# OettlM/STEDM

Hardware: AMD Instinct MI355X
Metric: U-Net denoising steps/sec (32x32x4 latent, bs=64) (higher is better)
Workload: dtype f16; 1 GPU; HER2-style DDIM-50 + CFG 1.5 (rescale 0.7) denoising step, NS32 U-Net (234.6M params, random-init PRNG weights), 32x32x4 latents + 3-ch layout concat, style vector 512; batch_per_gpu=64, global_batch=64, latent=32x32x4, cfg=cond+uncond per step, parallelism=dp1 (independent latents, no in-loop collective)

## Files before the change

include/stedm_hip.h:

```cpp
#ifndef STEDM_HIP_H
#define STEDM_HIP_H

#include <stdint.h>

#ifdef __cplusplus
extern "C" {
#endif

#define STEDM_ABI_VERSION 23

#define STEDM_F16 0
#define STEDM_BF16 1

#define STEDM_CONV_S1 0
#define STEDM_CONV_DOWN 1
#define STEDM_CONV_UP 2
#define STEDM_CONV_UP_SUBPIXEL 3
#define STEDM_CONV_S2D 4

int stedm_abi_version(void);
const char* stedm_last_error(void);
int stedm_device_cus(void);

#define STEDM_F16G_RAW 1
#define STEDM_F16G_NORM 2
#define STEDM_F16G_CONV_OUT16 4
#define STEDM_F16G_S2D 8
#define STEDM_F16G_CAST 16
#define STEDM_F16G_CONV_SRC 32
int stedm_f16_guard_set(void* flag_words);

int stedm_pack_conv_weight(const float* w_oihw, void* w_hi, void* w_lo, int cout, int cin, int ks,
                           int mm_dtype, void* stream);
int stedm_pack_conv_weight_up(const float* w_oihw, void* w_hi, void* w_lo, int cout, int cin, int mm_dtype,
                              void* stream);
int stedm_pack_conv_weight_frag(const float* w_oihw, void* out, int cout, int cin, int ks, int mm_dtype, void* stream);
int stedm_pack_conv_weight_up_frag(const float* w_oihw, void* out, int cout, int cin, int mm_dtype, void* stream);
int stedm_space_to_depth16(const float* x, int C, int B, int H, int W, void* out_hi, void* out_lo, int mm_dtype, void* stream);
int stedm_pack_conv_weight_frag16(const float* w, long sn, long sc, int flip, void* out, int cout, int cin, int ks, int mm_dtype, void* stream);
int stedm_pack_conv_weight_frag16_hl(const float* w, long sn, long sc, int flip, void* out, int cout, int cin, int mm_dtype, void* stream);
int stedm_pack_conv_weight_frag16_hl1(const float* w, long sn, long sc, int flip, void* out, int cout, int cin, int mm_dtype, void* stream);
int stedm_pack_conv_weight_up_frag16_hl(const float* w, void* out, int cout, int cin, int mm_dtype, void* stream);
int stedm_pack_conv_weight_s2d_frag16_hl(const float* w, void* out, int cout, int cin, int mm_dtype, int pad_br, void* stream);
int stedm_pack_conv_weight_s2d_frag(const float* w_oihw, void* out, int cout, int cin, int mm_dtype, int pad_br, void* stream);
int stedm_transpose_f32(const float* in, float* out, int rows, int cols, void* stream);

int stedm_gn_scale_shift(const float* x1, int c1, const float* x2, int c2, int x2_bmod,
                         const float* gamma, const float* beta, float eps, int groups, int B, int HW,
                         float* scale, float* shift, void* stream);

int stedm_gn_nslab(int C, int HW);
int stedm_gn_chan_nslab(int HW);
int stedm_gn_chan_stats(const float* x, int C, int B, int HW, int nslab, float* chan_stats, void* stream);
int stedm_gn_chan_stats16(const float* x, int C, int B, int HW, int nslab, float* chan_stats, void* out_hi, void* out_lo, int mm_dtype,
                          void* stream);
int stedm_gn_apply16c(const float* x1, int c1, const float* cs1, int nslab1, const float* x2, int c2, const float* cs2, int nslab2, int x2_bmod,
                      const float* gamma, const float* beta, float eps, int groups, int act, int B, int HW,
                      void* out_hi, void* out_lo, void* raw_hi, void* raw_lo, int mm_dtype, void* stream);
int stedm_gn_apply16c_mr(const float* x1, int c1, const float* cs1, int nslab1, const float* x2, int c2, const float* cs2, int nslab2, int x2_bmod,
                         const float* gamma, const float* beta, float eps, int groups, int act, int B, int HW,
                         void* out_hi, void* out_lo, void* raw_hi, void* raw_lo, float* mean_rstd, int mm_dtype, void* stream);
int stedm_gn_apply16c_x16(int c1, const float* cs1, int nslab1, const float* x2, int c2, const float* cs2, int nslab2, int x2_bmod,
                          const float* gamma, const float* beta, float eps, int groups, int act, int B, int HW,
                          void* out_hi, void* raw_hi, int mm_dtype, void* stream);
int stedm_gn_stats(const float* x1, int c1, const float* x2, int c2, int x2_bmod, int groups, int B, int HW,
                   double* stats, void* stream);
int stedm_gn_apply16(const float* x1, int c1, const float* x2, int c2, int x2_bmod, const float* gamma,
                     const float* beta, float eps, int groups, int act, const double* stats, int B, int HW,
                     void* out_hi, void* out_lo, int mm_dtype, void* stream);

typedef struct stedm_conv_args {
  const float* src1;
  const float* src2;
  int32_t c1, c2, src2_bmod;
  int32_t B, Hin, Win;
  int32_t mode;
  int32_t ks;
  const float* scale;
  const float* shift;
  int32_t act;
  const void* w_hi;
  const void* w_lo;
  const float* bias;
  const float* emb;
  int32_t emb_bstride;
  const float* res;
  float* out;
  int32_t cout;
  int32_t npass;
  int32_t mm_dtype;
  const void* src16_hi;
  const void* src16_lo;
  int32_t act_out;
  void* out16_hi;
  void* out16_lo;
  const void* w_frag;
  float* chan_stats;
  const void* src16b_hi;
  const void* w_frag_b;
  const float* bias_b;
  int32_t cb;
  float* ws;
  int64_t ws_floats;
  int32_t chan_nslab;
  const void* w_frag16;
  const void* w_frag_b16;
  int32_t pad_br;
  const float* gn_gamma;
  const float* gn_beta;
  float gn_eps;
  int32_t gn_groups;
  int32_t gn_act;
  void* gn_out16;
  float* gn_mr;
  int32_t gn_only;
  void* gn_out16_lo;
  void* qkv_q;
  void* qkv_k;
  void* qkv_vt;
  int32_t qkv_T, qkv_Tp, qkv_heads;
  float qkv_qscale;
  const float* ln_gamma;
  const float* ln_beta;
  const float* ln_res;
  float ln_eps;
  int32_t out16_stride;
  void* gn_coop;
  const uint32_t* gn_coop_epoch;
  uint32_t* gn_coop_tmo;
  int32_t src16_cstride;
  int32_t k_chan0;
  int32_t w_cin;
  int32_t res_bmod;
} stedm_conv_args;
int stedm_conv_igemm(const stedm_conv_args* args, void* stream);
int stedm_conv_fused_skip_ok(const stedm_conv_args* args);
int stedm_conv3x3_tiles_ok(int Hout, int Wout);
int stedm_im2col_rows16(const void* src16, void* dst16, int B, int Hs, int Ws, int C, int mode, void* stream);
int stedm_conv_rs_ok(const stedm_conv_args* args);

int stedm_conv_in(const float* x1, int c1, const float* x2, int c2, int x2_bmod, const float* w_oihw,
                  const float* bias, float* out, int B, int H, int W, int cout, float* chan_stats, void* stream);
int stedm_conv_out(const float* src, int c, const float* chan_stats, int nslab, const float* gamma, const float* beta,
                   float eps, int groups, const float* w_hwio, const float* bias, float* out, int B, int H, int W,
                   int cout, void* stream);

int stedm_time_embed(const int64_t* t, const float* freqs, const float* w0t, const float* b0,
                     const float* w2t, const float* b2, float* emb, float* ws, int B, int mc, int ted,
                     void* stream);
int stedm_time_embed_f32(const float* t, const float* freqs, const float* w0t, const float* b0,
                         const float* w2t, const float* b2, float* emb, float* ws, int B, int mc, int ted,
                         void* stream);
int stedm_emb_proj(const float* emb, const float* wt, const float* bias, float* out, int B, int k, int ntot,
                   void* stream);

int stedm_linear(const float* x, const float* wt, const float* bias, float* out, int B, int k, int n, int act_in,
                 int act_out, void* stream);

int stedm_attn_legacy(const float* qkv, float* out, int B, int T, int heads, int ch, void* stream);
int stedm_attn_legacy16(const void* qkv, int qkv_is16, void* out16, int B, int T, int heads, int ch, int mm_dtype, void* stream);

int stedm_ddim_step(const float* x, const float* e_c, const float* e_u, const float* noise,
                    const float* coefs, const int32_t* step_idx, float cfg_scale, float rescale_phi,
                    float* x_prev, float* pred_x0, int B, int C, int H, int W, void* stream);
int stedm_ddim_step_ex(const float* x, const float* e_c, const float* e_u, const float* noise, const float* coefs, const int32_t* step_idx,
                       int n_iters, float cfg_scale, float rescale_phi, int draw, float temperature, float noise_dropout, long first_id,
                       unsigned long long seed, float* x_prev, float* pred_x0, float* eps_out, float* noise_out, int B, int C, int H, int W,
                       void* stream);
int stedm_ddim_step_rows(const float* x, const float* e_c, const float* e_u, const float* noise, const float* coefs,
                         const int32_t* step_idx, int n_iters, const float* scales, float rescale_phi, int draw, long first_id,
                         unsigned long long seed, float* x_prev, float* pred_x0, int B, int C, int H, int W, void* stream);
int stedm_step_advance(int32_t* step_idx, int delta, void* stream);
int stedm_step_set_t(const int64_t* ts_table, const int32_t* step_idx, int64_t* t_buf, int B, void* stream);
int stedm_step_set_t_f32(const float* ts_table, const int32_t* step_idx, float* t_buf, int B, void* stream);

#define STEDM_DPM_NCOEF 6
int stedm_dpm_step(float* x, const float* e_c, const float* e_u, float* x0_prev, float* pred_x0, const float* coefs,
                   const int32_t* step_idx, float cfg_scale, long n, void* stream);

#define STEDM_DPMU_NCOEF 24
#define STEDM_DPMU_ALL 0
#define STEDM_DPMU_MODEL 1
#define STEDM_DPMU_COMBINE 2
int stedm_dpm_update(float* x, float* base, const float* e_c, const float* e_u, float* slots, long slot_stride, float* pred_x0,
                     const float* rows, const int32_t* step_idx, float cfg_scale, int mode, long n, void* stream);
int stedm_dpm_threshold(float* slots, long slot_stride, const float* rows, const int32_t* step_idx, float max_val, int B, long n,
                        float* q_out, void* stream);

#define STEDM_PLMS_EULER 0
#define STEDM_PLMS_HEUN 1
#define STEDM_PLMS_MULTISTEP 2
int stedm_plms_step(float* x, const float* e_c, const float* e_u, float* ring, const float* coefs, const int32_t* step_idx,
                    int n_iters, int phase, float cfg_scale, float* pred_x0, float* x_tmp, long n, void* stream);

int stedm_svit_patch_embed(const float* img, int B, int ns, int H, int W, int patch, const float* ln_w,
                           const float* ln_b, float eps, const float* wt, const float* bias, const float* pos,
                           const float* cls, float* x, int dim, void* stream);
int stedm_svit_patch_ln16(const float* img, int B, int ns, int H, int W, int patch, const float* ln_w, const float* ln_b,
                          float eps, void* out_hi, void* out_lo, int mm_dtype, void* stream);
int stedm_svit_tok_place(const float* tok, const float* pos, const float* cls, float* x, int B, int ntok, int dim, void* stream);
int stedm_ln_apply16(const float* x, const float* gamma, const float* beta, float eps, void* out_hi, void* out_lo,
                     long rows, int dim, int mm_dtype, void* stream);
int stedm_qkv_pack(const void* qkv, int qkv_is16, float qscale, void* q_hi, void* q_lo, void* k_hi, void* k_lo, void* vt_hi,
                   void* vt_lo, int B, int T, int Tp, int heads, int mm_dtype, void* stream);
int stedm_lsa_flash(const void* q_hi, const void* q_lo, const void* k_hi, const void* k_lo, const void* vt_hi,
                    const void* vt_lo, void* out_hi, void* out_lo, int B, int T, int Tp, int heads, int npass,
                    int mm_dtype, void* stream);
int stedm_qkv_pack_mx8(const void* qkv, int qkv_is16, float qscale, void* q8, void* qs, void* k8, void* ks, void* vt8, void* vs, int B, int T,
                       int Tp, int heads, int mm_dtype, void* stream);
int stedm_lsa_flash_mx8(const void* q8, const void* qs, const void* k8, const void* ks, const void* vt8, const void* vs, void* out16, int B,
                        int T, int Tp, int heads, int mm_dtype, void* stream);
int stedm_dropout_rows(const float* src, const float* res, float* out, void* out_hi, void* out_lo, long n, float p,
                       unsigned long long seed, unsigned site, int mm_dtype, void* stream);
int stedm_lsa_flash_drop(const void* q_hi, const void* q_lo, const void* k_hi, const void* k_lo, const void* vt_hi,
                         const void* vt_lo, void* out_hi, void* out_lo, int B, int T, int Tp, int heads, int npass,
                         int mm_dtype, float p, unsigned long long seed, unsigned site, void* stream);
int stedm_svit_head(const float* x, int B, int T, int dim, int pool, const float* c_old, const float* ln_w,
                    const float* ln_b, float eps, const float* wt, const float* bias, float* out, int ncls, float* ws, long ws_floats,
                    void* stream);
int stedm_geglu16(const float* g, void* out_hi, void* out_lo, long M, int I, int mm_dtype, void* stream);
int stedm_agg_reduce(const float* feats, float* out, int B, int n, int F, int mode, void* stream);
int stedm_spatial_rescale(const float* x, const float* w, float* out, int B, int cin, int cout, int H, int W,
// ... 113 lines not shown
```

stedm_amd/_lib.py:

```python
from __future__ import annotations

import ctypes as C
import os

_HERE = os.path.dirname(os.path.abspath(__file__))
LIB_PATH = os.environ.get("STEDM_HIP_LIB") or os.path.join(_HERE, "libstedm_hip.so")

ABI_VERSION = 23
F16, BF16 = 0, 1
CONV_S1, CONV_DOWN, CONV_UP, CONV_UP_SUBPIXEL, CONV_S2D = 0, 1, 2, 3, 4


class StedmHipError(RuntimeError):
    pass


class ConvArgs(C.Structure):
    _fields_ = [
        ("src1", C.c_void_p), ("src2", C.c_void_p),
        ("c1", C.c_int32), ("c2", C.c_int32), ("src2_bmod", C.c_int32),
        ("B", C.c_int32), ("Hin", C.c_int32), ("Win", C.c_int32),
        ("mode", C.c_int32), ("ks", C.c_int32),
        ("scale", C.c_void_p), ("shift", C.c_void_p),
        ("act", C.c_int32),
        ("w_hi", C.c_void_p), ("w_lo", C.c_void_p), ("bias", C.c_void_p),
        ("emb", C.c_void_p), ("emb_bstride", C.c_int32),
        ("res", C.c_void_p), ("out", C.c_void_p),
        ("cout", C.c_int32), ("npass", C.c_int32), ("mm_dtype", C.c_int32),
        ("src16_hi", C.c_void_p), ("src16_lo", C.c_void_p),
        ("act_out", C.c_int32), ("out16_hi", C.c_void_p), ("out16_lo", C.c_void_p),
        ("w_frag", C.c_void_p), ("chan_stats", C.c_void_p),
        ("src16b_hi", C.c_void_p), ("w_frag_b", C.c_void_p), ("bias_b", C.c_void_p), ("cb", C.c_int32),
        ("ws", C.c_void_p), ("ws_floats", C.c_int64), ("chan_nslab", C.c_int32), ("w_frag16", C.c_void_p), ("w_frag_b16", C.c_void_p), ("pad_br", C.c_int32),
        ("gn_gamma", C.c_void_p), ("gn_beta", C.c_void_p), ("gn_eps", C.c_float), ("gn_groups", C.c_int32), ("gn_act", C.c_int32), ("gn_out16", C.c_void_p), ("gn_mr", C.c_void_p), ("gn_only", C.c_int32),
        ("gn_out16_lo", C.c_void_p),
        ("qkv_q", C.c_void_p), ("qkv_k", C.c_void_p), ("qkv_vt", C.c_void_p),
        ("qkv_T", C.c_int32), ("qkv_Tp", C.c_int32), ("qkv_heads", C.c_int32), ("qkv_qscale", C.c_float),
        ("ln_gamma", C.c_void_p), ("ln_beta", C.c_void_p), ("ln_res", C.c_void_p), ("ln_eps", C.c_float),
        ("out16_stride", C.c_int32),
        ("gn_coop", C.c_void_p), ("gn_coop_epoch", C.c_void_p), ("gn_coop_tmo", C.c_void_p),
        ("src16_cstride", C.c_int32), ("k_chan0", C.c_int32), ("w_cin", C.c_int32), ("res_bmod", C.c_int32),
    ]


_P, _I, _F = C.c_void_p, C.c_int, C.c_float
SIGNATURES = {
    "stedm_abi_version": (_I, []),
    "stedm_last_error": (C.c_char_p, []),
    "stedm_device_cus": (_I, []),
    "stedm_f16_guard_set": (_I, [_P]),
    "stedm_pack_conv_weight": (_I, [_P, _P, _P, _I, _I, _I, _I, _P]),
    "stedm_pack_conv_weight_up": (_I, [_P, _P, _P, _I, _I, _I, _P]),
    "stedm_pack_conv_weight_frag": (_I, [_P, _P, _I, _I, _I, _I, _P]),
    "stedm_pack_conv_weight_up_frag": (_I, [_P, _P, _I, _I, _I, _P]),
    "stedm_pack_conv_weight_frag16": (_I, [_P, C.c_long, C.c_long, _I, _P, _I, _I, _I, _I, _P]),
    "stedm_pack_conv_weight_frag16_hl": (_I, [_P, C.c_long, C.c_long, _I, _P, _I, _I, _I, _P]),
    "stedm_pack_conv_weight_frag16_hl1": (_I, [_P, C.c_long, C.c_long, _I, _P, _I, _I, _I, _P]),
    "stedm_pack_conv_weight_up_frag16_hl": (_I, [_P, _P, _I, _I, _I, _P]),
    "stedm_pack_conv_weight_s2d_frag16_hl": (_I, [_P, _P, _I, _I, _I, _I, _P]),
    "stedm_pack_conv_weight_s2d_frag": (_I, [_P, _P, _I, _I, _I, _I, _P]),
    "stedm_space_to_depth16": (_I, [_P, _I, _I, _I, _I, _P, _P, _I, _P]),
    "stedm_transpose_f32": (_I, [_P, _P, _I, _I, _P]),
    "stedm_gn_scale_shift": (_I, [_P, _I, _P, _I, _I, _P, _P, _F, _I, _I, _I, _P, _P, _P]),
    "stedm_gn_nslab": (_I, [_I, _I]),
    "stedm_gn_stats": (_I, [_P, _I, _P, _I, _I, _I, _I, _I, _P, _P]),
    "stedm_gn_apply16": (_I, [_P, _I, _P, _I, _I, _P, _P, _F, _I, _I, _P, _I, _I, _P, _P, _I, _P]),
    "stedm_gn_chan_nslab": (_I, [_I]),
    "stedm_gn_chan_stats": (_I, [_P, _I, _I, _I, _I, _P, _P]),
    "stedm_gn_chan_stats16": (_I, [_P, _I, _I, _I, _I, _P, _P, _P, _I, _P]),
    "stedm_gn_apply16c": (_I, [_P, _I, _P, _I, _P, _I, _P, _I, _I, _P, _P, _F, _I, _I, _I, _I, _P, _P, _P, _P, _I, _P]),
    "stedm_gn_apply16c_mr": (_I, [_P, _I, _P, _I, _P, _I, _P, _I, _I, _P, _P, _F, _I, _I, _I, _I, _P, _P, _P, _P, _P, _I, _P]),
    "stedm_conv3x3_tiles_ok": (_I, [_I, _I]),
    "stedm_im2col_rows16": (_I, [_P, _P, _I, _I, _I, _I, _I, _P]),
    "stedm_philox_normal": (_I, [_P, _I, _I, _P, _I, C.c_ulonglong, C.c_uint, _P]),
    "stedm_ddim_mask_blend": (_I, [_P, _P, _P, C.c_long, C.c_long, _P, _P, _P, _P, _P, _I, _I, _I, C.c_long, C.c_ulonglong, _P]),
    "stedm_ddpm_step": (_I, [_P, _P, _P, _P, _I, _I, _P, _P, C.c_long, C.c_long, _P, _P, _P, _P, _I, _I, _I, C.c_long,
                            C.c_ulonglong, C.c_ulonglong, _P]),
    "stedm_ddpm_step_ex": (_I, [_P, _P, _P, _P, _P, _I, _I, _P, _P, _F, _P, _I, _P, C.c_long, C.c_long, _P, _P, _P, _P, _P, _P, _P, _P,
                               _I, _I, _I, C.c_long, C.c_ulonglong, C.c_ulonglong, _P]),
    "stedm_gn_apply16c_x16": (_I, [_I, _P, _I, _P, _I, _P, _I, _I, _P, _P, _F, _I, _I, _I, _I, _P, _P, _I, _P]),
    "stedm_conv_igemm": (_I, [C.POINTER(ConvArgs), _P]),
    "stedm_conv_fused_skip_ok": (_I, [C.POINTER(ConvArgs)]),
    "stedm_conv_rs_ok": (_I, [C.POINTER(ConvArgs)]),
    "stedm_conv_in": (_I, [_P, _I, _P, _I, _I, _P, _P, _P, _I, _I, _I, _I, _P, _P]),
    "stedm_conv_out": (_I, [_P, _I, _P, _I, _P, _P, _F, _I, _P, _P, _P, _I, _I, _I, _I, _P]),
    "stedm_time_embed": (_I, [_P, _P, _P, _P, _P, _P, _P, _P, _I, _I, _I, _P]),
    "stedm_time_embed_f32": (_I, [_P, _P, _P, _P, _P, _P, _P, _P, _I, _I, _I, _P]),
    "stedm_emb_proj": (_I, [_P, _P, _P, _P, _I, _I, _I, _P]),
    "stedm_linear": (_I, [_P, _P, _P, _P, _I, _I, _I, _I, _I, _P]),
    "stedm_attn_legacy": (_I, [_P, _P, _I, _I, _I, _I, _P]),
    "stedm_attn_legacy16": (_I, [_P, _I, _P, _I, _I, _I, _I, _I, _P]),
    "stedm_ddim_step": (_I, [_P, _P, _P, _P, _P, _P, _F, _F, _P, _P, _I, _I, _I, _I, _P]),
    "stedm_ddim_step_ex": (_I, [_P, _P, _P, _P, _P, _P, _I, _F, _F, _I, _F, _F, C.c_long, C.c_ulonglong, _P, _P, _P, _P, _I, _I, _I, _I,
                               _P]),
    "stedm_ddim_step_rows": (_I, [_P, _P, _P, _P, _P, _P, _I, _P, _F, _I, C.c_long, C.c_ulonglong, _P, _P, _I, _I, _I, _I, _P]),
    "stedm_step_advance": (_I, [_P, _I, _P]),
    "stedm_step_set_t": (_I, [_P, _P, _P, _I, _P]),
    "stedm_step_set_t_f32": (_I, [_P, _P, _P, _I, _P]),
    "stedm_dpm_step": (_I, [_P, _P, _P, _P, _P, _P, _P, _F, C.c_long, _P]),
    "stedm_dpm_update": (_I, [_P, _P, _P, _P, _P, C.c_long, _P, _P, _P, _F, _I, C.c_long, _P]),
    "stedm_dpm_threshold": (_I, [_P, C.c_long, _P, _P, _F, _I, C.c_long, _P, _P]),
    "stedm_plms_step": (_I, [_P, _P, _P, _P, _P, _P, _I, _I, _F, _P, _P, C.c_long, _P]),
    "stedm_svit_patch_embed": (_I, [_P, _I, _I, _I, _I, _I, _P, _P, _F, _P, _P, _P, _P, _P, _I, _P]),
    "stedm_svit_patch_ln16": (_I, [_P, _I, _I, _I, _I, _I, _P, _P, _F, _P, _P, _I, _P]),
    "stedm_svit_tok_place": (_I, [_P, _P, _P, _P, _I, _I, _I, _P]),
    "stedm_ln_apply16": (_I, [_P, _P, _P, _F, _P, _P, C.c_long, _I, _I, _P]),
    "stedm_qkv_pack": (_I, [_P, _I, _F, _P, _P, _P, _P, _P, _P, _I, _I, _I, _I, _I, _P]),
    "stedm_lsa_flash": (_I, [_P, _P, _P, _P, _P, _P, _P, _P, _I, _I, _I, _I, _I, _I, _P]),
    "stedm_lsa_flash_drop": (_I, [_P, _P, _P, _P, _P, _P, _P, _P, _I, _I, _I, _I, _I, _I, _F, C.c_ulonglong, C.c_uint, _P]),
    "stedm_dropout_rows": (_I, [_P, _P, _P, _P, _P, C.c_long, _F, C.c_ulonglong, C.c_uint, _I, _P]),
    "stedm_qkv_pack_mx8": (_I, [_P, _I, _F, _P, _P, _P, _P, _P, _P, _I, _I, _I, _I, _I, _P]),
    "stedm_lsa_flash_mx8": (_I, [_P, _P, _P, _P, _P, _P, _P, _I, _I, _I, _I, _I, _P]),
    "stedm_svit_head": (_I, [_P, _I, _I, _I, _I, _P, _P, _P, _F, _P, _P, _P, _I, _P, C.c_long, _P]),
    "stedm_ln_bwd_blocks": (_I, [C.c_long]),
    "stedm_ln_bwd": (_I, [_P, _P, _P, _F, _P, _P, _P, _P, _P, C.c_long, _I, _I, _P]),
    "stedm_geglu_bwd": (_I, [_P, _P, _P, C.c_long, _I, _P]),
    "stedm_geglu16": (_I, [_P, _P, _P, C.c_long, _I, _I, _P]),
    "stedm_agg_reduce": (_I, [_P, _P, _I, _I, _I, _I, _P]),
    "stedm_spatial_rescale": (_I, [_P, _P, _P, _I, _I, _I, _I, _I, _I, _P]),
    "stedm_pack_frag_multi": (_I, [_P, _I, _I, _I, _P]),
    "stedm_swin_patch16": (_I, [_P, C.c_long, C.c_long, C.c_long, C.c_long, _I, _I, _I, _P, _P, _I, _P]),
    "stedm_swin_ln": (_I, [_P, _P, _P, _F, _P, _P, _P, _P, C.c_long, _I, _I, _I, _P]),
    "stedm_swin_ln_gated": (_I, [_P, _P, _P, _F, _P, _P, _P, _P, C.c_long, _I, _I, _P, _I, _I, _P]),
    "stedm_swin_window_attn": (_I, [_P, _P, _P, _P, _P, _P, _P, _I, _I, _I, _I, _I, _I, _I, _I, _I, _P]),
    "stedm_swin_merge16": (_I, [_P, _I, _I, _I, _I, _P, _P, _I, _P]),
    "stedm_swin_rpb": (_I, [_P, _P, _P, _I, _I, _P]),
    "stedm_swin_token_mean": (_I, [_P, _P, _I, _I, _I, _P]),
    "stedm_pack_conv_weight_strided": (_I, [_P, C.c_long, C.c_long, _I, _P, _P, _P, _I, _I, _I, _I, _P]),
    "stedm_gn_fold": (_I, [_P, _I, _I, _P, _I, _I, _I, _I, _I, _F, _P, _P]),
    "stedm_gn_bwd": (_I, [_P, _I, _P, _I, _P, _P, _P, _I, _I, _P, _P, _I, _I, _P, _P, _I, _P, _I, _P, _P, _I, _P, _P, _I, _P]),
    "stedm_gn_bwd_ws_floats": (C.c_long, [_I, _I, _I, _I]),
    "stedm_im2col_t16": (_I, [_P, _P, _I, _I, _I, _I, _I, _I, C.c_long, _P]),
    "stedm_wgrad_to_oihw": (_I, [_P, _P, _I, _I, _I, _I, _I, _I, _I, _P]),
    "stedm_wgrad3x3_plan": (_I, [_I, _I, _I, _I, _I, C.POINTER(C.c_int)]),
    "stedm_wgrad3x3": (_I, [_P, _P, _P, _I, _I, _I, _I, _I, _I, _P]),
    "stedm_wgrad3x3_oihw": (_I, [_P, _P, _P, _I, _I, _I, _I, _I, _I, _P]),
    "stedm_sum_planes": (_I, [_P, _P, C.c_long, _I, _I, _P]),
    "stedm_wgrad1x1_plan": (_I, [C.c_long, _I, _I, C.POINTER(C.c_int)]),
    "stedm_wgrad1x1": (_I, [_P, _P, _P, C.c_long, _I, _I, _I, _P]),
    "stedm_chan_sum_fold": (_I, [_P, _I, _I, _I, _P, C.c_long, _P, _I, _P]),
    "stedm_chan_sum_fold2": (_I, [_P, _I, _I, _I, _P, C.c_long, _P, _I, _P, _P]),
    "stedm_sum2x2": (_I, [_P, _P, _I, _I, _I, _I, _I, _P]),
    "stedm_zero_insert16": (_I, [_P, _P, _P, _I, _I, _I, _I, _I, _P]),
    "stedm_attn_legacy_bwd_ws_floats": (C.c_long, [_I, _I, _I]),
    "stedm_attn_legacy_bwd": (_I, [_P, _P, _P, _I, _I, _I, _I, _P, _P]),
    "stedm_gemm_f32": (_I, [_P, C.c_long, _I, _P, C.c_long, _I, _P, C.c_long, _I, _I, _I, _F, _F, _P, C.c_long, _P]),
    "stedm_silu": (_I, [_P, _P, _P, C.c_long, _I, _P]),
    "stedm_q_sample": (_I, [_P, _P, _P, _P, _P, _P, _I, C.c_long, _P]),
    "stedm_l1_loss": (_I, [_P, _P, C.c_long, _F, _P, _P, _P, _P]),
    "stedm_diffusion_loss_blocks": (_I, [C.c_long]),
    "stedm_diffusion_loss": (_I, [_P, _P, _P, _P, _P, _I, C.c_long, _I, _I, C.c_double, C.c_double, C.c_double, _P, _P, _P, C.c_long, _P, _P]),
    "stedm_spatial_rescale_wgrad": (_I, [_P, _P, _P, _P, _I, _I, _I, _I, _I, _I, _I, _P]),
    "stedm_axpby_f32": (_I, [_P, _P, C.c_long, _F, _F, _P]),
    "stedm_adamw_ema": (_I, [_P, _P, _P, _I, _F, _F, _F, _F, _F, _I, _F, _F, _P]),
    "stedm_adamw_ema_pack": (_I, [_P, _I, _I, _F, _F, _F, _F, _F, _I, _F, _F, _P]),
    "stedm_adamw_ema_pack_piece": (_I, [_P, _P]),
    "stedm_adamw_ema_sched": (_I, [_P, _P, _P, _I, _F, _F, _F, _F, _P, _P, _F, _P]),
    "stedm_adamw_ema_pack_sched": (_I, [_P, _I, _I, _F, _F, _F, _F, _P, _P, _F, _P]),
    "stedm_ema_update": (_I, [_P, _P, _P, _I, _F, _P]),
    "stedm_vq_nearest": (_I, [_P, _P, _I, _I, _I, C.c_long, _P, _P, _P]),
    "stedm_ddim_quantize_x0": (_I, [_P, _P, _P, _P, _P, _P, _I, _I, _I, C.c_long, _P, _P, _P]),
    "stedm_conv1x1_nchw": (_I, [_P, _P, _P, _P, _I, _I, _I, C.c_long, _P]),
    "stedm_softmax_rows16": (_I, [_P, C.c_long, _F, _P, _P, C.c_long, _I, C.c_long, _I, _P]),
    "stedm_image_to_uint8": (_I, [_P, _P, _I, _I, _I, _I, _P]),
    "stedm_seg_merge": (_I, [_P, _P, _I, _I, _I, _I, _P]),
    "stedm_argmax_u8": (_I, [_P, _P, C.c_long, _I, _P]),
# ... 42 lines not shown
```

stedm_amd/csrc/conv_common.hpp:

```cpp
#pragma once
#include "common.hpp"

typedef float f32x16 __attribute__((ext_vector_type(16)));
typedef float f32x4 __attribute__((ext_vector_type(4)));
typedef _Float16 f16x8 __attribute__((ext_vector_type(8)));
typedef __bf16 bf16x8 __attribute__((ext_vector_type(8)));
typedef _Float16 f16x4 __attribute__((ext_vector_type(4)));
typedef __bf16 bf16x4 __attribute__((ext_vector_type(4)));

constexpr int BN = 128;

struct ConvParams {
  stedm_conv_args a;
  int M, Hout, Wout, HWout, Cin, taps;
  int cstride, w_cin;
  int whole, nsamp, trows;
  int wsplit;
  int PRs, PW, NP;
  int tiles_m, tiles_n;
  unsigned mg_hw, mg_w, mg_pw, mg_prpw;
  int ksplit;
  int stats_done;
  int gn_done;
  int gn_tile;
  int gn_coop;
  int xcd_m;
  int npers;
  unsigned* ovf;
  int dbg;
};

#ifdef STEDM_CONV_DIAG
#define STEDM_DBG(WORD, BITS) (((WORD) & (BITS)) != 0)
#else
#define STEDM_DBG(WORD, BITS) (0)
#endif

template <typename T>
struct MM;
template <>
struct MM<_Float16> {
  using V8 = f16x8;
  using V4 = f16x4;
  static __device__ __forceinline__ f32x16 mfma(V8 a, V8 b, f32x16 c) {
    return __builtin_amdgcn_mfma_f32_32x32x16_f16(a, b, c, 0, 0, 0);
  }
  static __device__ __forceinline__ f32x4 mfma16(V8 a, V8 b, f32x4 c) {
    return __builtin_amdgcn_mfma_f32_16x16x32_f16(a, b, c, 0, 0, 0);
  }
};
template <>
struct MM<__bf16> {
  using V8 = bf16x8;
  using V4 = bf16x4;
  static __device__ __forceinline__ f32x16 mfma(V8 a, V8 b, f32x16 c) {
    return __builtin_amdgcn_mfma_f32_32x32x16_bf16(a, b, c, 0, 0, 0);
  }
  static __device__ __forceinline__ f32x4 mfma16(V8 a, V8 b, f32x4 c) {
    return __builtin_amdgcn_mfma_f32_16x16x32_bf16(a, b, c, 0, 0, 0);
  }
};


#define STEDM_ZERO_PAGE_BYTES 135168

namespace stedm {
bool conv_geometry(ConvParams& p, int bm, bool allow_wsplit = false);
int conv_launch_dma(ConvParams& p, hipStream_t st, bool dry = false);
}
```

stedm_amd/csrc/conv_dma_bf16_p1.hip:

```cpp
#include "conv_igemm_dma9.inc"
#include "conv_rs.inc"
namespace stedm {
int conv_dma_pick_bf16_p1(ConvParams& p, hipStream_t st, bool dry) {
  int rc = conv_rs_pick<__bf16>(p, st, dry);
  if (rc >= 0 || dry || p.a.src16b_hi || p.a.mode == STEDM_CONV_S2D || p.a.qkv_q || p.a.ln_gamma) return rc;
  if (p.a.src16_cstride || p.a.k_chan0 || p.a.w_cin || p.a.res_bmod || p.a.out16_stride) return rc;
  rc = dma9_pick<__bf16>(p, st);
  return rc >= 0 ? rc : dma_pick<1, __bf16>(p, st);
}
}

extern "C" int stedm_debug_conv_stamps(unsigned long long* host_out, int nblocks) {
  if (!host_out || nblocks <= 0 || nblocks > 2048) { stedm::set_error("debug_conv_stamps: bad args"); return 1; }
  hipError_t e = hipMemcpyFromSymbol(host_out, HIP_SYMBOL(g_conv_stamps), (size_t)nblocks * 8 * sizeof(unsigned long long));
  if (e != hipSuccess) { stedm::set_error("debug_conv_stamps: %s", hipGetErrorString(e)); return 2; }
  return 0;
}
```

stedm_amd/csrc/conv_dma_f16_p1.hip:

```cpp
#include "conv_igemm_dma9.inc"
#include "conv_rs.inc"
namespace stedm {
int conv_dma_pick_f16_p1(ConvParams& p, hipStream_t st, bool dry) {
  int rc = conv_rs_pick<_Float16>(p, st, dry);
  if (rc >= 0 || dry || p.a.src16b_hi || p.a.mode == STEDM_CONV_S2D || p.a.qkv_q || p.a.ln_gamma) return rc;
  if (p.a.src16_cstride || p.a.k_chan0 || p.a.w_cin || p.a.res_bmod || p.a.out16_stride) return rc;
  rc = dma9_pick<_Float16>(p, st);
  return rc >= 0 ? rc : dma_pick<1, _Float16>(p, st);
}
}
```

stedm_amd/csrc/conv_igemm.hip:

```cpp
#include <stdlib.h>

#include "conv_common.hpp"
using namespace stedm;

constexpr int BM = 128, NTHREADS = 256;

template <int BKC, int NPASS, typename T>
__global__ void __launch_bounds__(NTHREADS, 2) conv_igemm_kernel(const ConvParams p) {
  using V8 = typename MM<T>::V8;
  using V4 = typename MM<T>::V4;
  constexpr int AST = BKC * 2 + 16;
  constexpr int BST = BKC * 2 + 16;
  constexpr int NPL = NPASS == 3 ? 2 : 1;
  constexpr int QC = BKC / 4;
  constexpr int POSL = NTHREADS / QC;
  constexpr int PCS = BKC / 8;
  constexpr int BPT = BN * PCS / NTHREADS;
  constexpr int KSTEPS = BKC / 16;

  extern __shared__ __attribute__((aligned(16))) unsigned char smem[];
  unsigned char* sA = smem;
  const int a_plane = p.NP * AST;
  unsigned char* sB = smem + NPL * a_plane;
  constexpr int b_plane = BN * BST;
// ... 210 lines not shown
        if (a.res) v += a.res[o];
        a.out[o] = v;
      }
    }
  }
  f16_guard_commit(p.ovf, bad_src, STEDM_F16G_CONV_SRC);
}

template <int BKC, int NPASS, typename T>
static int launch(const ConvParams& p, hipStream_t st) {
  constexpr int AST = BKC * 2 + 16, BST = BKC * 2 + 16, NPL = NPASS == 3 ? 2 : 1;
  const size_t lds = (size_t)NPL * p.NP * AST + (size_t)2 * NPL * BN * BST;
  if (lds > 160 * 1024) {
    set_error("conv_igemm: tile needs %zu B of LDS (> 160 KiB): Hin=%d Win=%d mode=%d", lds, p.a.Hin, p.a.Win, p.a.mode);
    return 1;
  }
  auto k = conv_igemm_kernel<BKC, NPASS, T>;
  if (lds > 64 * 1024) {
    hipError_t e = hipFuncSetAttribute(reinterpret_cast<const void*>(k), hipFuncAttributeMaxDynamicSharedMemorySize, (int)lds);
    if (e != hipSuccess) {
      set_error("conv_igemm: hipFuncSetAttribute(%zu) failed: %s", lds, hipGetErrorString(e));
      return 2;
    }
  }
  k<<<p.tiles_m * p.tiles_n, NTHREADS, lds, st>>>(p);
  STEDM_LAUNCH_CHECK();
  return 0;
}

bool stedm::conv_geometry(ConvParams& p, int bm, bool allow_wsplit) {
  const stedm_conv_args& a = p.a;
  p.tiles_n = (a.cout + BN - 1) / BN;
  p.tiles_m = (p.M + bm - 1) / bm;
  p.wsplit = 0;
  if (a.ks == 1) {
    p.whole = 0; p.nsamp = 1; p.trows = 0; p.PRs = 1; p.PW = bm; p.NP = bm;
    return true;
  }
  if (p.HWout <= bm) {
    if (bm % p.HWout != 0) { set_error("conv_igemm: Hout*Wout=%d must divide %d", p.HWout, bm); return false; }
    p.whole = 1; p.nsamp = bm / p.HWout; p.trows = p.Hout;
    p.tiles_m = (a.B + p.nsamp - 1) / p.nsamp;
  } else if (allow_wsplit && p.Wout > bm && p.Wout % bm == 0 && (a.mode == STEDM_CONV_S1 || a.mode == STEDM_CONV_UP_SUBPIXEL || a.mode == STEDM_CONV_S2D)) {
    p.whole = 0; p.nsamp = 1; p.trows = 1; p.wsplit = 1;
  } else {
    if (bm % p.Wout != 0 || p.HWout % bm != 0) {
      set_error("conv_igemm: unsupported spatial shape %dx%d (need Wout | %d and %d | Hout*Wout)", p.Hout, p.Wout, bm, bm);
      return false;
    }
    p.whole = 0; p.nsamp = 1; p.trows = bm / p.Wout;
  }
  if (a.mode == STEDM_CONV_S1 || a.mode == STEDM_CONV_UP_SUBPIXEL || a.mode == STEDM_CONV_S2D) p.PRs = p.trows + 2;
  else if (a.mode == STEDM_CONV_DOWN) p.PRs = 2 * p.trows + 1;
  else p.PRs = (p.trows + 1) / 2 + 2;
  p.PW = (p.wsplit ? bm : a.Win) + 2;
  p.NP = p.nsamp * p.PRs * p.PW;
  return true;
}

static int conv_dispatch(ConvParams& p, void* stream);
static int conv_setup(ConvParams& p);

extern "C" int stedm_conv3x3_tiles_ok(int Hout, int Wout) {
  if (Hout <= 0 || Wout <= 0) return 0;
  if (Wout > 256 && Wout % 256 == 0) return 1;
  for (int bm = 256; bm >= 128; bm >>= 1) {
    const int HW = Hout * Wout;
    if (HW <= bm) { if (bm % HW == 0) return 1; continue; }
    if (bm % Wout == 0 && HW % bm == 0) return 1;
  }
  return 0;
}

extern "C" int stedm_conv_fused_skip_ok(const stedm_conv_args* args) {
  if (!args || !args->src16b_hi || !args->src16_hi) return 0;
  ConvParams p;
  memset(&p, 0, sizeof(p));
  p.a = *args;
  if (conv_setup(p) != 0) return 0;
  return conv_launch_dma(p, nullptr, true) == 0 ? 1 : 0;
}

extern "C" int stedm_conv_rs_ok(const stedm_conv_args* args) {
  if (!args || !args->src16_hi || (!args->w_frag && !args->w_frag16) || (args->npass != 1 && !args->w_frag16)) return 0;
  ConvParams p;
  memset(&p, 0, sizeof(p));
  p.a = *args;
  if (conv_setup(p) != 0) return 0;
  return conv_launch_dma(p, nullptr, true) == 0 ? 1 : 0;
}

extern "C" int stedm_conv_igemm(const stedm_conv_args* args, void* stream) {
  STEDM_CHECK_ARG(args, "conv_igemm: null args");
  ConvParams p;
  memset(&p, 0, sizeof(p));
  p.a = *args;
  const stedm_conv_args& a = p.a;
  STEDM_CHECK_ARG(!a.chan_stats || a.out || (a.out16_hi && !a.out16_lo && a.npass == 1), "conv_igemm: chan_stats needs the fp32 output (or, single product, the 16-bit-only form)");
  STEDM_CHECK_ARG(a.out16_stride == 0 || (a.out16_hi && !a.out16_lo && a.npass == 1 && a.out16_stride >= a.cout && a.out16_stride % 4 == 0 && a.cout % 4 == 0 &&
                                          !a.ln_gamma && !a.qkv_q && !a.act_out),
                  "conv_igemm: out16_stride needs out16_hi alone (single product), stride >= cout, both multiples of 4, plain epilogue");
  STEDM_CHECK_ARG(!a.gn_out16 || (a.out && a.chan_stats && a.gn_gamma && a.gn_beta && a.gn_groups > 0 && a.cout % a.gn_groups == 0 &&
                                  (a.npass == 1 || a.gn_out16_lo) && a.mode == STEDM_CONV_S1 && (a.gn_act == 0 || a.gn_act == 1)),
                  "conv_igemm: gn_out16 needs out, chan_stats, gamma / beta, groups dividing cout, stride 1 and a single-product mode (or gn_out16_lo)");
  STEDM_CHECK_ARG(!a.gn_out16_lo || a.gn_out16, "conv_igemm: gn_out16_lo without gn_out16");
  int rc = conv_dispatch(p, stream);
  if (rc != 0) return rc;
  if (a.chan_stats && !p.stats_done && !a.out) {
    set_error("conv_igemm: the 16-bit-only form with chan_stats ran on a kernel without the statistics epilogue");
    return 1;
  }
  if (a.chan_stats && !p.stats_done) {
    const int up = (a.mode == STEDM_CONV_UP || a.mode == STEDM_CONV_UP_SUBPIXEL) ? 4 : 1, down = a.mode == STEDM_CONV_DOWN ? 4 : 1;
    rc = stedm_gn_chan_stats(a.out, a.cout, a.B, a.Hin * a.Win * up / down, a.chan_nslab, a.chan_stats, stream);
    if (rc != 0) return rc;
  }
  if (a.gn_out16 && !p.gn_done) {
    const int HW = a.Hin * a.Win;
    rc = stedm_gn_apply16c_mr(a.out, a.cout, a.chan_stats, a.chan_nslab > 0 ? a.chan_nslab : stedm_gn_chan_nslab(HW), nullptr, 0, nullptr, 0, 0, a.gn_gamma,
                              a.gn_beta, a.gn_eps, a.gn_groups, a.gn_act, a.B, HW, a.gn_out16, a.gn_out16_lo, nullptr, nullptr, a.gn_mr, a.mm_dtype, stream);
  }
  return rc;
}

static int conv_setup(ConvParams& p) {
  const stedm_conv_args& a = p.a;
  STEDM_CHECK_ARG((a.src1 || a.src16_hi) && (a.w_hi || (a.mode == STEDM_CONV_S2D && (a.w_frag || (a.npass == 3 && a.w_frag16)))) && (a.out || a.out16_hi || a.qkv_q),
                  "conv_igemm: null src/w_hi/out");
  STEDM_CHECK_ARG(!a.ln_gamma || (a.ln_beta && (a.out || a.out16_hi) && !a.out16_lo && !a.res && !a.emb && !a.chan_stats && !a.gn_out16 && !a.act_out && !a.qkv_q &&
                                  a.src16_hi && !a.src1 && !a.src16b_hi && a.w_frag && a.ks == 1 && a.mode == STEDM_CONV_S1 && a.npass == 1 && a.cout <= 128 &&
                                  a.cout % 4 == 0),
                  "conv_igemm: the LayerNorm epilogue needs a 1x1 GEMM with cout <= 128 (a multiple of 4), src16 + w_frag, a single-product mode and no other epilogue extra");
  STEDM_CHECK_ARG(!a.qkv_q || (a.qkv_k && a.qkv_vt && !a.out && !a.out16_hi && !a.res && !a.emb && !a.chan_stats && !a.gn_out16 && !a.act_out && a.src16_hi && !a.src1 &&
                               !a.src16b_hi && a.w_frag && a.ks == 1 && a.mode == STEDM_CONV_S1 && a.npass == 1 && a.B == 1 && a.Hin == 1 && a.qkv_heads > 0 &&
                               a.qkv_heads % 2 == 0 && a.cout == 3 * a.qkv_heads * 64 && a.qkv_T > 0 && a.qkv_T % 2 == 0 && a.qkv_Tp >= a.qkv_T &&
                               a.qkv_Tp % 2 == 0 && a.Win % a.qkv_T == 0),
                  "conv_igemm: the qkv epilogue needs a flat 1x1 GEMM (B = Hin = 1, Win = nb * T rows), cout = 3 * heads * 64 with an even head count, even T / Tp, "
                  "src16 + w_frag, a single-product mode and no other output or epilogue extra");
  STEDM_CHECK_ARG(a.pad_br == 0 || a.mode == STEDM_CONV_S2D, "conv_igemm: pad_br belongs to the space-to-depth form");
  STEDM_CHECK_ARG(a.mode != STEDM_CONV_S2D || (a.src16_hi && !a.src1 && a.ks == 3 && !a.src16b_hi &&
                                                ((a.npass == 1 && a.w_frag) || (a.npass == 3 && a.w_frag16 && a.src16_lo))),
                  "conv_igemm: the space-to-depth form needs src16 planes, ks=3 and w_frag (single product) or w_frag16 + src16_lo (3 products)");
  STEDM_CHECK_ARG((!a.act_out && !a.out16_hi) || (a.src16_hi && !a.src1), "conv_igemm: act_out/out16 need the DMA path (src16 only)");
  STEDM_CHECK_ARG(!a.src1 || (a.src2 != nullptr) == (a.c2 > 0), "conv_igemm: src2/c2 mismatch");
  STEDM_CHECK_ARG(!a.src16_hi || a.npass == 1 || a.src16_lo, "conv_igemm: npass=3 needs src16_lo");
  STEDM_CHECK_ARG(a.ks == 1 || a.ks == 3, "conv_igemm: ks must be 1 or 3");
  STEDM_CHECK_ARG(a.mode >= 0 && a.mode <= 4, "conv_igemm: bad mode %d", a.mode);
  STEDM_CHECK_ARG(a.mode != STEDM_CONV_UP_SUBPIXEL || (a.src16_hi && !a.src1 && a.ks == 3), "conv_igemm: sub-pixel upsample needs the DMA path (src16) and ks=3");
  STEDM_CHECK_ARG(a.ks == 3 || a.mode == STEDM_CONV_S1, "conv_igemm: 1x1 supports stride 1 only");
  STEDM_CHECK_ARG(a.npass == 1 || a.npass == 3, "conv_igemm: npass must be 1 or 3");
  STEDM_CHECK_ARG(a.npass == 1 || a.w_lo || (a.mode == STEDM_CONV_S2D && a.w_frag16), "conv_igemm: npass=3 needs w_lo");
  STEDM_CHECK_ARG((a.scale != nullptr) == (a.shift != nullptr), "conv_igemm: scale/shift must come together");
  STEDM_CHECK_ARG(a.B > 0 && a.Hin > 0 && a.Win > 0 && a.cout > 0, "conv_igemm: bad sizes");
  STEDM_CHECK_ARG(a.mm_dtype == STEDM_F16 || a.mm_dtype == STEDM_BF16, "conv_igemm: bad mm_dtype %d", a.mm_dtype);
  p.Cin = a.c1 + a.c2;
  p.cstride = a.src16_cstride ? a.src16_cstride : p.Cin;
  p.w_cin = a.w_cin ? a.w_cin : p.Cin;
  {
    const bool kwin = a.src16_cstride || a.k_chan0 || a.w_cin;
    const bool plain3 = a.src16_hi && !a.src1 && a.c2 == 0 && a.ks == 3 && a.mode == STEDM_CONV_S1 && a.npass == 1 && !a.src16b_hi && (a.w_frag || a.w_frag16) &&
                        !a.ln_gamma && !a.qkv_q;
    STEDM_CHECK_ARG(!kwin || (plain3 && a.k_chan0 >= 0 && a.k_chan0 % 32 == 0 && p.cstride % 32 == 0 && p.w_cin % 32 == 0 && a.c1 % 32 == 0 &&
                              a.k_chan0 + a.c1 <= p.cstride && a.k_chan0 + a.c1 <= p.w_cin),
                    "conv_igemm: a K window (src16_cstride=%d k_chan0=%d w_cin=%d) needs a plain 3x3 stride-1 single-product problem on src16 planes with "
                    "w_frag / w_frag16 and no fused skip phase; multiples of 32 with k_chan0 + c1 inside both the plane row and the pack",
                    a.src16_cstride, a.k_chan0, a.w_cin);
    STEDM_CHECK_ARG(a.res_bmod == 0 || (a.res_bmod > 0 && a.res && plain3),
                    "conv_igemm: res_bmod=%d needs res and a plain 3x3 stride-1 single-product problem on src16 planes with w_frag / w_frag16 and no fused skip phase",
                    a.res_bmod);
  }
  p.taps = (a.mode == STEDM_CONV_UP_SUBPIXEL || a.mode == STEDM_CONV_S2D) ? 4 : a.ks * a.ks;
  if (a.mode == STEDM_CONV_UP_SUBPIXEL || a.mode == STEDM_CONV_S2D) {
    p.Hout = a.Hin; p.Wout = a.Win;
  } else if (a.mode == STEDM_CONV_DOWN) {
    STEDM_CHECK_ARG(a.Hin % 2 == 0 && a.Win % 2 == 0, "conv_igemm: stride-2 needs even Hin/Win");
    p.Hout = a.Hin / 2; p.Wout = a.Win / 2;
  } else if (a.mode == STEDM_CONV_UP) {
    p.Hout = a.Hin * 2; p.Wout = a.Win * 2;
  } else {
    p.Hout = a.Hin; p.Wout = a.Win;
  }
  p.HWout = p.Hout * p.Wout;
  p.M = a.B * p.HWout;
  STEDM_CHECK_ARG(p.Cin % 32 == 0 && (a.c2 == 0 || a.c1 % 32 == 0),
                  "conv_igemm: channel counts must be multiples of 32 (c1=%d c2=%d)", a.c1, a.c2);
  STEDM_CHECK_ARG(!a.src16b_hi || (a.src16_hi && !a.src1 && ((a.w_frag && a.w_frag_b) || (a.w_frag16 && a.w_frag_b16)) && a.ks == 3 && a.mode == STEDM_CONV_S1 && a.npass == 1 && !a.res &&
                                   a.cb > 0 && a.cb % 64 == 0),
                  "conv_igemm: the fused skip phase needs the DMA path (src16 only), 3x3 stride 1, single product, w_frag + w_frag_b, cb %% 64 == 0, no res");
  return 0;
}

static int conv_dispatch(ConvParams& p, void* stream) {
  const stedm_conv_args& a = p.a;
  { const int rc = conv_setup(p); if (rc) return rc; }
  hipStream_t st = as_stream(stream);
  static const int dbg0 = getenv("STEDM_CONV_DBG") ? atoi(getenv("STEDM_CONV_DBG")) : 0;
#ifdef STEDM_CONV_DIAG
  p.dbg = dbg0;
#else
  p.dbg = 0;
  if (dbg0) { set_error("conv_igemm: STEDM_CONV_DBG=%d needs a diagnostic build (tools/conv_diag.sh, STEDM_HIP_LIB); the shipped kernels compile no ablation switch", dbg0); return 1; }
#endif
  p.ovf = a.mm_dtype == STEDM_F16 ? f16_guard_flag() : nullptr;
  if (a.src16_hi) {
    const int rc = conv_launch_dma(p, st);
    if (rc == 0 || !a.src1) return rc;
  }
  const int bkc = (a.npass == 1 && p.Cin % 64 == 0 && (a.c2 == 0 || a.c1 % 64 == 0)) ? 64 : 32;
  if (!conv_geometry(p, BM)) return 1;
  const bool f16 = a.mm_dtype == STEDM_F16;
  if (a.npass == 3) return f16 ? launch<32, 3, _Float16>(p, st) : launch<32, 3, __bf16>(p, st);
  if (bkc == 64) return f16 ? launch<64, 1, _Float16>(p, st) : launch<64, 1, __bf16>(p, st);
  return f16 ? launch<32, 1, _Float16>(p, st) : launch<32, 1, __bf16>(p, st);
}
```

stedm_amd/csrc/conv_igemm_dma.hip:

```cpp
#include "conv_common.hpp"
using namespace stedm;

namespace stedm {
int conv_dma_pick_f16_p1(ConvParams&, hipStream_t, bool dry);
int conv_dma_pick_f16_p3(ConvParams&, hipStream_t, bool dry);
int conv_dma_pick_bf16_p1(ConvParams&, hipStream_t, bool dry);
int conv_dma_pick_bf16_p3(ConvParams&, hipStream_t, bool dry);
}

int stedm::conv_launch_dma(ConvParams& p, hipStream_t st, bool dry) {
  const stedm_conv_args& a = p.a;
  if (a.src16b_hi && a.npass != 1) { set_error("conv_igemm(dma): the fused skip phase is single-product only"); return 1; }
  if (dry && a.npass != 1 && !a.w_frag16) return 1;
  if (a.src16b_hi && ((long)a.B * a.Hin * a.Win * a.cb >= (1L << 31) || a.cb * 2 + 256 > STEDM_ZERO_PAGE_BYTES)) {
    set_error("conv_igemm(dma): fused skip operand too large (cb=%d)", a.cb);
    return 1;
  }
  if ((long)a.B * a.Hin * a.Win * (p.cstride > p.Cin ? p.cstride : p.Cin) >= (1L << 31)) {
    set_error("conv_igemm(dma): activation tensor too large for 32-bit element offsets");
    return 1;
  }
  if (p.Cin * 2 + 256 > STEDM_ZERO_PAGE_BYTES) { set_error("conv_igemm(dma): Cin too large for the zero page"); return 1; }
  const bool f16 = a.mm_dtype == STEDM_F16;
  int rc = a.npass == 3 ? (f16 ? conv_dma_pick_f16_p3(p, st, dry) : conv_dma_pick_bf16_p3(p, st, dry))
                        : (f16 ? conv_dma_pick_f16_p1(p, st, dry) : conv_dma_pick_bf16_p1(p, st, dry));
  if (dry) return rc < 0 ? 1 : 0;
  if (rc < 0 && a.ln_gamma) { set_error("conv_igemm(dma): the register-streamed kernel does not run this LayerNorm-epilogue problem (see stedm_conv_rs_ok)"); return 1; }
  if (rc < 0 && a.qkv_q) { set_error("conv_igemm(dma): the register-streamed kernel does not run this qkv-epilogue problem (see stedm_conv_rs_ok)"); return 1; }
  if (rc < 0 && (a.src16_cstride || a.k_chan0 || a.w_cin || a.res_bmod || a.out16_stride)) {
    set_error("conv_igemm(dma): the register-streamed kernel does not run this problem, and no other kernel knows a K window, res_bmod or out16_stride (see stedm_conv_rs_ok)");
    return 1;
  }
  if (rc < 0 && a.src16b_hi) { set_error("conv_igemm(dma): no kernel runs this fused skip problem (see stedm_conv_fused_skip_ok)"); return 1; }
  if (rc < 0) { set_error("conv_igemm(dma): no tile configuration fits (Hin=%d Win=%d mode=%d Cin=%d)", a.Hin, a.Win, a.mode, p.Cin); return 1; }
  return rc;
}
```

stedm_amd/csrc/conv_rs.inc:

```
#pragma once
#include <type_traits>

#include "conv_igemm_dma.inc"

static __device__ unsigned long long g_conv_stamps[2048 * 8];
#define STAMP(K) if (STEDM_DBG(p.dbg, 1024) && tid == 0 && blockIdx.x < 2048) g_conv_stamps[blockIdx.x * 8 + (K)] = wall_clock64()
#define STAMPC(K) if (STEDM_DBG(p.dbg, 1024) && tid == 0 && blockIdx.x < 2048) g_conv_stamps[blockIdx.x * 8 + (K)] = __builtin_amdgcn_s_memtime()

#ifdef STEDM_CONV_DIAG
#define RS_DIAG(BIT) ((STEDM_CONV_DIAG) & (BIT))
#else
#define RS_DIAG(BIT) 0
#endif

__device__ __forceinline__ float rs_lane_xor1(float v) {
  return __builtin_bit_cast(float, __builtin_amdgcn_mov_dpp(__builtin_bit_cast(int, v), 0xB1, 0xF, 0xF, true));
}
template <typename T>
__device__ __forceinline__ unsigned rs_pack2(float lo, float hi) {
  typedef T V2T __attribute__((ext_vector_type(2)));
  V2T v; v[0] = (T)lo; v[1] = (T)hi;
  return __builtin_bit_cast(unsigned, v);
}

// ... 215 lines not shown
#define A3_AFTER(Q, WHAT)                                                                                          \
  {                                                                                                                \
    if ((Q) + 2 < 8) { WHAT(Acur, t, (Q) + 2) }                                                                    \
    else if (t + 1 < NS) { WHAT(Acur, t + 1, (Q) + 2 - 8) }                                                         \
    else { WHAT(Anext, 0, (Q) + 2 - 8) }                                                                           \
  }
#define A3_ADDR_HI(BASE, TAP, F) asm volatile("v_add_u32 %0, %1, %2" : "=v"(a_) : "s"((BASE) + tapd[TAP]), "v"(aofs[F]));
#define A3_ADDR_LO(BASE, TAP, F) asm volatile("v_add_u32 %0, %1, %2" : "=v"(a2_) : "s"((BASE) + tapd[TAP] + a_half), "v"(aofs[F]));
#define RS3_CHUNK(PAR)                                                                                             \
  _Pragma("unroll") for (int u = 0; u < NU; ++u) {                                                                 \
    const int t = u >> 1, hf = u & 1, sb = (t & 1) ^ (PAR);                                                        \
    if (u == NU - 1) __builtin_amdgcn_s_barrier();    \
    _Pragma("unroll") for (int i = 0; i < 4; ++i) {                                                                \
      const int R = hf * 4 + i;                             \
      _Pragma("unroll") for (int m = 0; m < 12; ++m) {                                                             \
        const int j = m & 3;                                                                                       \
        __builtin_amdgcn_sched_barrier(0);                                                                         \
        if (m < 4) acc[R][j] = MM<T>::mfma16(al[R & (NAR - 1)], bh[sb][j], acc[R][j]);                              \
        else if (m < 8) acc[R][j] = MM<T>::mfma16(ah[R & (NAR - 1)], bl[sb][j], acc[R][j]);                         \
        else acc[R][j] = MM<T>::mfma16(ah[R & (NAR - 1)], bh[sb][j], acc[R][j]);                                    \
        __builtin_amdgcn_sched_barrier(0);                                                                         \
        if (m == 0) { LDSR(ah[(R + 1) & (NAR - 1)], a_); }                                                          \
        else if (m == 1) { LDSR(al[(R + 1) & (NAR - 1)], a2_); }                                                    \
        if (R == 0 && m >= 4) {                                                                                    \
                        \
          if (m == 4) { int g_ = g0 + t + 1; g_ = g_ < gmax ? g_ : gmax; wcur = wq + ((size_t)(unsigned)g_ << 13) + voff; } \
          if (m < 8) bh[sb ^ 1][m - 4] = *reinterpret_cast<const V8*>(wcur + (m - 4) * 1024);                        \
          else bl[sb ^ 1][m - 8] = *reinterpret_cast<const V8*>(wcur + wlo + (m - 8) * 1024);                        \
        }                                                                                                          \
        if (m == 10) A3_AFTER(R, A3_ADDR_HI)                                                                        \
        else if (m == 11) A3_AFTER(R, A3_ADDR_LO)                                                                   \
      }                                                                                                            \
    }                                                                                                              \
  }
  const unsigned char* wcur = wq + voff;
  unsigned a_ = 0, a2_ = 0;
  LOAD_B3(0, 0)
  LOAD_B3(1, 1)
  __syncthreads();
  {
    const unsigned Afirst = A0 + abuf * a_buf;
#pragma unroll
    for (int f = 0; f < NAR; ++f) LOAD_A3(Afirst, 0, f)
    A3_ADDR_HI(Afirst, 0, 1)
    A3_ADDR_LO(Afirst, 0, 1)
  }
#define RS3_STEP(STEP, PAR)                                                                                        \
  {                                                                                                                \
    const unsigned Acur = A0 + abuf * a_buf;                                                                       \
    if (++abuf == NABUF) abuf = 0;                                                                                 \
                                       \
    const unsigned Anext = (STEP) + 1 < nchunks ? A0 + abuf * a_buf : Acur;                                        \
    const int g0 = (STEP) * NS;                                                                                    \
    RS3_CHUNK(PAR)                                                                                                 \
  }
  int step = 0;
  for (; step + 1 < nchunks; step += 2) {
    RS3_STEP(step, 0)
    RS3_STEP(step + 1, NS & 1)
  }
  if (step < nchunks) RS3_STEP(step, 0)
#undef RS3_STEP
#undef RS3_CHUNK
#undef A3_AFTER
#undef A3_ADDR_HI
#undef A3_ADDR_LO
#undef LOAD_A3
#undef LOAD_B3
#undef LDSR
}

template <typename T, int WM, int KIND, bool FUSE = false, bool P3 = false>
__global__ void __launch_bounds__((16 / WM + 2) * 64) conv_rs_kernel(const ConvParams p) {
  static_assert(!FUSE || KIND == RS_3X3 || KIND == RS_3X3M, "the fused skip phase belongs to the 3x3 kinds");
  static_assert(!P3 || ((KIND == RS_3X3M || KIND == RS_1X1M || KIND == RS_SUBM) && !FUSE), "the 3-product form exists for the plain 16x16x32 kinds");
  static_assert(KIND != RS_1X1M || (P3 && !FUSE && WM == 4), "RS_1X1M is a 3-product kind");
  static_assert(KIND != RS_SUBM || (!FUSE && WM == 4), "RS_SUBM: plain epilogues, one compute wave per SIMD");
  constexpr int NCW = 16 / WM, NT = (NCW + 2) * 64, BMT = 256;
  constexpr bool NPERS = KIND == RS_1X1N, IS1X1 = KIND == RS_1X1 || NPERS, SUBM = KIND == RS_SUBM, SUBPIX = KIND == RS_SUB || SUBM;
  constexpr bool G1 = KIND == RS_1X1M;
  constexpr bool M16 = KIND == RS_3X3M || G1 || SUBM;
  constexpr bool GEO1 = IS1X1 || G1;
  constexpr bool IS3X3 = KIND == RS_3X3 || KIND == RS_3X3M;
  constexpr int NS = IS3X3 ? 9 : (SUBM ? 4 : (SUBPIX ? 8 : (G1 ? 1 : 4)));
  constexpr int NPL = (SUBPIX || KIND == RS_3X3M) ? 2 : 1;
  constexpr int NTAB = IS3X3 ? 9 : 4;
  constexpr int BROW = IS1X1 ? 128 : (G1 ? 64 : 32);
  constexpr int CPP = BROW / 16, RPB = 16 / CPP, PPI = 64 / CPP;
  constexpr int BKC = M16 ? 32 : NS * 16 / (IS3X3 ? 9 : (SUBPIX ? 4 : 1));
  constexpr int TAPS = NTAB, NABUF = P3 ? 3 : 4;
  constexpr int SST = kStageStride;

  extern __shared__ __attribute__((aligned(16))) unsigned char smem[];
  const int nai = (p.NP + PPI - 1) / PPI;
  const int a_plane = nai * 1024;
  const int a_half = NPL * a_plane + (M16 ? 32 : 0);
  const int a_buf = P3 ? 2 * a_half : ((FUSE && NPL * a_plane < 32768) ? 32768 : a_half);
  const int pl_skew = (KIND == RS_3X3M || SUBM) ? 16 : 0;
  int* sM = reinterpret_cast<int*>(smem);
  int* sMb = sM + BMT;
  unsigned char* sA = reinterpret_cast<unsigned char*>(sMb + BMT);
  float* sStage = reinterpret_cast<float*>(sA);
  const int ring_bytes = NABUF * a_buf;
  int* sIdx = reinterpret_cast<int*>(sA + ring_bytes);

  const stedm_conv_args& a = p.a;
  const int tid = threadIdx.x;
  const int lane = tid & 63;
  const int wave = __builtin_amdgcn_readfirstlane(tid >> 6);
  const bool is_loader = wave >= NCW;
  const int ntile = p.tiles_m * p.tiles_n;
  const bool s2d = SUBPIX && a.mode == STEDM_CONV_S2D;
  const int parity = (SUBPIX && !s2d) ? (blockIdx.x / ntile) & 3 : 0;
  const bool split = (IS3X3 || SUBPIX || GEO1) && p.ksplit >= 2;
  const int kz = split ? ((SUBPIX && !s2d) ? blockIdx.x / (4 * ntile) : blockIdx.x / ntile) : 0;
  const int bid = (SUBPIX || split) ? blockIdx.x % ntile : blockIdx.x;
  const int py = parity >> 1, px = parity & 1;
  int tile_n = bid % p.tiles_n, tile_m = bid / p.tiles_n;
  if (p.xcd_m) {
    const int gm = p.xcd_m, gn = 8 / gm, x = bid & 7, j = bid >> 3, tn_x = p.tiles_n / gn;
    const int jm = j / tn_x;
    tile_n = (j - jm * tn_x) * gn + x / gm;
    tile_m = jm * gm + x % gm;
  }
  constexpr bool npers = NPERS;
  if (npers) { tile_m = bid / p.npers; tile_n = (bid % p.npers) * (p.tiles_n / p.npers); }
  if STEDM_DBG(p.dbg, 256) { tile_n = 0; tile_m = 0; }
  const int m0 = tile_m * BMT, n0 = tile_n * BN;
  const int nchunks_all = p.Cin / BKC;
  const int nchunks_w = p.w_cin / BKC;
  const int nsteps = split ? nchunks_all / p.ksplit : nchunks_all;
  const int cbeg = kz * nsteps;
  const int nsteps2_all = FUSE ? a.cb / 64 : 0;
  const int nsteps2 = split ? nsteps2_all / p.ksplit : nsteps2_all;
  const int c2beg = split ? kz * nsteps2 : 0;
  STAMP(0);

  int b0, yo0;
  if (p.whole) { b0 = tile_m * p.nsamp; yo0 = 0; }
  else { b0 = m0 / p.HWout; yo0 = (m0 - b0 * p.HWout) / p.Wout; }
  const int br = s2d ? a.pad_br : 0;
  const int x0 = p.wsplit ? (m0 - b0 * p.HWout) - yo0 * p.Wout : 0;
  const int srow0 = ((a.mode == STEDM_CONV_S1 || SUBPIX) ? yo0 - 1 : (yo0 - 1) >> 1) + br;
  static_assert(RS_3X3 == 0, "");

  auto div_hw = [&](int n) { return (int)__umulhi((unsigned)n, p.mg_hw); };
  auto div_w = [&](int n) { return (int)__umulhi((unsigned)n, p.mg_w); };
  auto div_pw = [&](int n) { return (int)__umulhi((unsigned)n, p.mg_pw); };
  auto div_prpw = [&](int n) { return (int)__umulhi((unsigned)n, p.mg_prpw); };
  const int rem0 = GEO1 ? m0 - (m0 / p.HWout) * p.HWout : 0;
  auto patch_pixel = [&](int pos) {
    int off = -1;
    if (pos < p.NP) {
      if (GEO1) { if (m0 + pos < p.M) off = m0 + pos; }
      else {
        const int s_ = div_prpw(pos), rem = pos - s_ * (p.PRs * p.PW);
        const int prow = div_pw(rem), pcol = rem - prow * p.PW;
        const int b = b0 + s_, sy = srow0 + prow, sx = x0 + pcol - 1 + br;
        if (b < a.B && sy >= 0 && sy < a.Hin && sx >= 0 && sx < a.Win) off = (b * a.Hin + sy) * a.Win + sx;
      }
    }
    return off;
  };
  constexpr int NTC = NCW * 64;
  if (!is_loader) {
  for (int ml = tid; ml < BMT; ml += NTC) {
// ... 509 lines not shown
          *reinterpret_cast<V8T*>(dstp + (((long)b * H + hd) * Tp + t) * 64 + d0) = h8;
          const uint4 hb = __builtin_bit_cast(uint4, h8);
          bad16 |= f16_over2<T>(hb.x) | f16_over2<T>(hb.y) | f16_over2<T>(hb.z) | f16_over2<T>(hb.w);
        }
      } else {
        long o[2];
#pragma unroll
        for (int hf = 0; hf < 2; ++hf) {
          const int row = 2 * (hf * 64 + lane), m = sM[row];
          o[hf] = m < 0 ? -1 : (long)sMb[row] * HD * Tp + (m - sMb[row] * Tn);
        }
        T* __restrict__ vt = reinterpret_cast<T*>(a.qkv_vt);
        for (int d = tid >> 6; d < 128; d += NT / 64) {
          const int nl = n0 - 2 * HD + d;
          const float bs = a.bias ? a.bias[n0 + d] : 0.f;
#pragma unroll
          for (int hf = 0; hf < 2; ++hf) {
            if (o[hf] < 0) continue;
            const float2 x = *reinterpret_cast<const float2*>(sStage + d * kStageStrideT + 2 * (hf * 64 + lane));
            V2T h2; h2[0] = (T)(x.x + bs); h2[1] = (T)(x.y + bs);
            *reinterpret_cast<V2T*>(vt + o[hf] + (long)nl * Tp) = h2;
            bad16 |= f16_over2<T>(__builtin_bit_cast(unsigned, h2));
          }
        }
      }
      f16_guard_commit(p.ovf, bad16, STEDM_F16G_CONV_OUT16);
      return;
    }
  }
  if (!split && !a.out && a.out16_hi && !a.out16_lo && !a.res && !a.emb && !a.chan_stats && (a.cout & 7) == 0) {
    typedef T V8T __attribute__((ext_vector_type(8)));
    const int c8 = tid & 15, n8 = n0 + c8 * 8;
    if (n8 < a.cout) {
      float b8[8];
#pragma unroll
      for (int u = 0; u < 8; ++u) b8[u] = (a.bias ? a.bias[n8 + u] : 0.f) + ((FUSE && a.bias_b) ? a.bias_b[n8 + u] : 0.f);
      const bool gelu = a.act_out == 2;
      T* __restrict__ o16 = reinterpret_cast<T*>(a.out16_hi);
      unsigned bad16 = 0u;
#pragma unroll 2
      for (int row = tid >> 4; row < BMT; row += NT / 16) {
        const int m = sM[row];
        if (m < 0) continue;
        const float4 x0 = *reinterpret_cast<const float4*>(sStage + row * SST + c8 * 8);
        const float4 x1 = *reinterpret_cast<const float4*>(sStage + row * SST + c8 * 8 + 4);
        float v[8] = {x0.x + b8[0], x0.y + b8[1], x0.z + b8[2], x0.w + b8[3], x1.x + b8[4], x1.y + b8[5], x1.z + b8[6], x1.w + b8[7]};
        V8T h8;
#pragma unroll
        for (int u = 0; u < 8; ++u) h8[u] = (T)(gelu ? gelu_erf_f(v[u]) : v[u]);
        *reinterpret_cast<V8T*>(o16 + (long)m * (a.out16_stride ? a.out16_stride : a.cout) + n8) = h8;
        const uint4 hb = __builtin_bit_cast(uint4, h8);
        bad16 |= f16_over2<T>(hb.x) | f16_over2<T>(hb.y) | f16_over2<T>(hb.z) | f16_over2<T>(hb.w);
      }
      f16_guard_commit(p.ovf, bad16, STEDM_F16G_CONV_OUT16);
    }
    return;
  }
  float* sPart = sStage + BMT * SST;
  float* sCh = sPart + (NT / 32) * 128 * 2;
  float* sGm = sCh + 128 * 2;
  const int coop = p.gn_coop;
  const bool gn_t = p.gn_tile != 0 || coop != 0;
  float* sAll = sGm + 32 * 2;
  const bool keep_out = !(gn_t && a.gn_only);
  const bool ragged = p.HWout % BMT != 0 && BMT % p.HWout != 0;
  const int rows_per = (p.HWout < BMT && !ragged) ? p.HWout : BMT;
  const int nsub = BMT / rows_per;
  unsigned bad16 = 0u, badn = 0u;
  for (int sub = 0; sub < nsub; ++sub) {
    float cs[4] = {0.f, 0.f, 0.f, 0.f}, cq[4] = {0.f, 0.f, 0.f, 0.f};
    const bool only16 = !a.out && a.out16_hi && !a.out16_lo;
    const bool fast = vec_ok && !split && (a.out ? !a.out16_hi : only16) && !a.act_out && !(ragged && a.emb);
    if (active && fast) {
      float ev[4] = {0.f, 0.f, 0.f, 0.f};
      const int rfirst = sub * rows_per;
      if (a.emb && sM[rfirst] >= 0) {
        const float* ep = a.emb + (long)sMb[rfirst] * a.emb_bstride + n;
#pragma unroll
        for (int u = 0; u < 4; ++u) ev[u] = ep[u];
      }
      const bool has_emb = a.emb != nullptr;
      const int rb_ = a.res_bmod ? __builtin_amdgcn_readfirstlane(sMb[rfirst]) : 0;
      const float* __restrict__ resp = a.res_bmod ? a.res - (long)(rb_ - rb_ % a.res_bmod) * p.HWout * a.cout : a.res;
      float* __restrict__ outp = a.out;
      typedef T V4T16 __attribute__((ext_vector_type(4)));
      T* __restrict__ o16p = only16 ? reinterpret_cast<T*>(a.out16_hi) : nullptr;
      const long ostr16 = a.out16_stride ? a.out16_stride : a.cout;
      constexpr int RB = 8;
      for (int row0 = rfirst + rg; row0 < rfirst + rows_per; row0 += RB * (NT / 32)) {
        int mm[RB];
        float4 r4[RB];
#pragma unroll
        for (int k = 0; k < RB; ++k) {
          const int row = row0 + k * (NT / 32);
          mm[k] = row < rfirst + rows_per ? sM[row] : -1;
          r4[k] = make_float4(0.f, 0.f, 0.f, 0.f);
          if (resp && mm[k] >= 0) r4[k] = *reinterpret_cast<const float4*>(resp + (long)mm[k] * a.cout + n);
        }
#pragma unroll
        for (int k = 0; k < RB; ++k) {
          const int row = row0 + k * (NT / 32), m = mm[k];
          if (m < 0) continue;
          const float4 v4 = *reinterpret_cast<const float4*>(sStage + row * SST + c4 * 4);
          const long o = (long)m * a.cout + n;
          float v[4] = {v4.x + bv[0], v4.y + bv[1], v4.z + bv[2], v4.w + bv[3]};
          if (has_emb) { v[0] += ev[0]; v[1] += ev[1]; v[2] += ev[2]; v[3] += ev[3]; }
          if (resp) { v[0] += r4[k].x; v[1] += r4[k].y; v[2] += r4[k].z; v[3] += r4[k].w; }
          if (keep_out && outp) *reinterpret_cast<float4*>(outp + o) = make_float4(v[0], v[1], v[2], v[3]);
          if (o16p) {
            V4T16 h4;
#pragma unroll
            for (int u = 0; u < 4; ++u) h4[u] = (T)v[u];
            *reinterpret_cast<V4T16*>(o16p + (long)m * ostr16 + n) = h4;
            bad16 |= f16_over_v4<T>(h4);
          }
          if (gn_t) *reinterpret_cast<float4*>(sStage + row * SST + c4 * 4) = make_float4(v[0], v[1], v[2], v[3]);
#pragma unroll
          for (int u = 0; u < 4; ++u) { cs[u] += v[u]; cq[u] += v[u] * v[u]; }
        }
      }
    } else
    if (active) {
      for (int row = sub * rows_per + rg; row < (sub + 1) * rows_per; row += NT / 32) {
        const int m = sM[row];
        if (m < 0) continue;
        const float4 v4 = *reinterpret_cast<const float4*>(sStage + row * SST + c4 * 4);
        float v[4] = {v4.x + bv[0], v4.y + bv[1], v4.z + bv[2], v4.w + bv[3]};
        const long o = (long)m * a.cout + n;
        if (split) {
          *reinterpret_cast<float4*>(a.ws + (long)kz * p.M * ((SUBPIX && !s2d) ? 4 : 1) * a.cout + o) = v4;
          continue;
        }
        if (a.emb) {
          const float* ep = a.emb + (long)sMb[row] * a.emb_bstride + n;
          for (int u = 0; u < nv; ++u) v[u] += ep[u];
        }
        if (a.res) {
          const long ro = a.res_bmod ? o - (long)(sMb[row] - sMb[row] % a.res_bmod) * p.HWout * a.cout : o;
          if (vec_ok) { const float4 r4 = *reinterpret_cast<const float4*>(a.res + ro); v[0] += r4.x; v[1] += r4.y; v[2] += r4.z; v[3] += r4.w; }
          else for (int u = 0; u < nv; ++u) v[u] += a.res[ro + u];
        }
        if (a.act_out == 2) {
#pragma unroll
          for (int u = 0; u < 4; ++u) v[u] = gelu_erf_f(v[u]);
        }
        if (a.out) {
          if (vec_ok) *reinterpret_cast<float4*>(a.out + o) = make_float4(v[0], v[1], v[2], v[3]);
          else for (int u = 0; u < nv; ++u) a.out[o + u] = v[u];
        }
        if (a.out16_hi) {
          typedef T V4T __attribute__((ext_vector_type(4)));
          if (vec_ok) {
            V4T h4, l4;
#pragma unroll
            for (int u = 0; u < 4; ++u) { h4[u] = (T)v[u]; l4[u] = (T)(v[u] - (float)h4[u]); }
            *reinterpret_cast<V4T*>(reinterpret_cast<T*>(a.out16_hi) + (a.out16_stride ? (long)m * a.out16_stride + n : o)) = h4;
            bad16 |= f16_over_v4<T>(h4);
            if (a.out16_lo) *reinterpret_cast<V4T*>(reinterpret_cast<T*>(a.out16_lo) + o) = l4;
          } else {
            for (int u = 0; u < nv; ++u) {
              const T hv = (T)v[u];
              bad16 |= f16_over2<T>((unsigned)__builtin_bit_cast(unsigned short, hv));
              reinterpret_cast<T*>(a.out16_hi)[o + u] = hv;
              if (a.out16_lo) reinterpret_cast<T*>(a.out16_lo)[o + u] = (T)(v[u] - (float)hv);
            }
          }
        }
#pragma unroll
        for (int u = 0; u < 4; ++u) { cs[u] += v[u]; cq[u] += v[u] * v[u]; }
      }
    }
    if (a.chan_stats) {
#pragma unroll
      for (int u = 0; u < 4; ++u) { sPart[(rg * 128 + c4 * 4 + u) * 2] = cs[u]; sPart[(rg * 128 + c4 * 4 + u) * 2 + 1] = cq[u]; }
      __syncthreads();
      const int row0 = sub * rows_per;
      if (tid < 128 && n0 + tid < a.cout && sM[row0] >= 0) {
        float su = 0.f, sq = 0.f;
        for (int g = 0; g < NT / 32; ++g) { su += sPart[(g * 128 + tid) * 2]; sq += sPart[(g * 128 + tid) * 2 + 1]; }
        const int b = sMb[row0];
        const int mlow = (p.whole && !GEO1) ? b * p.HWout : m0 + row0;
        const int run = (mlow - b * p.HWout) / BMT;
        const int nrun = (p.HWout + 255) / 256;
        const int nslab = (SUBPIX && !s2d) ? 4 * nrun : nrun;
        const int slab = (SUBPIX && !s2d) ? run * 4 + parity : run;
        float* d = a.chan_stats + (((long)b * nslab + slab) * a.cout + n0 + tid) * 2;
        d[0] = su; d[1] = sq;
        if (gn_t) { sCh[tid * 2] = su; sCh[tid * 2 + 1] = sq; }
        if (coop) {
          typedef __attribute__((address_space(1))) unsigned long long gu64;
          const unsigned ep = *a.gn_coop_epoch;
          gu64* G = (gu64*)(reinterpret_cast<unsigned long long*>(a.gn_coop) + (((long)b * 4 + run) * 128 + tid) * 2);
          __hip_atomic_store(G, ((unsigned long long)ep << 32) | __float_as_uint(su), __ATOMIC_RELAXED, __HIP_MEMORY_SCOPE_AGENT);
          __hip_atomic_store(G + 1, ((unsigned long long)ep << 32) | __float_as_uint(sq), __ATOMIC_RELAXED, __HIP_MEMORY_SCOPE_AGENT);
          sAll[(run * 128 + tid) * 2] = su; sAll[(run * 128 + tid) * 2 + 1] = sq;
        }
      }
      if (coop && wave == 0 && sM[sub * rows_per] >= 0) {
        typedef __attribute__((address_space(1))) unsigned long long gu64;
        const unsigned ep = *a.gn_coop_epoch;
        const int row0c = sub * rows_per;
        const int bb = sMb[row0c];
        const int runc = ((m0 + row0c) - bb * p.HWout) / BMT;
        const gu64* Gb = (const gu64*)(reinterpret_cast<const unsigned long long*>(a.gn_coop) + (long)bb * 4 * 128 * 2);
        bool done = false;
        for (unsigned spins = 0; !done; ++spins) {
          bool ok = true;
          unsigned v[3][4];
#pragma unroll
          for (int pi = 0; pi < 3; ++pi) {
            const int k = (runc + 1 + pi) % coop;
            if (pi < coop - 1) {
#pragma unroll
              for (int j = 0; j < 4; ++j) {
                const unsigned long long x = __hip_atomic_load(Gb + (k * 128 + lane + 64 * (j >> 1)) * 2 + (j & 1), __ATOMIC_RELAXED, __HIP_MEMORY_SCOPE_AGENT);
                v[pi][j] = (unsigned)x;
                ok &= (unsigned)(x >> 32) == ep;
              }
            }
          }
          done = __all(ok);
// ... 20 lines not shown
          double s_ = 0.0, q_ = 0.0;
          if (coop) {
            const int L = 256 / a.gn_groups, n_e = cpg * coop;
            for (int l = 0; l < L; ++l) {
              double su = 0.0, sq = 0.0;
              for (int e = l; e < n_e; e += L) {
                const int k = e / cpg, c = tid * cpg + (e - k * cpg);
                su += (double)sAll[(k * 128 + c) * 2]; sq += (double)sAll[(k * 128 + c) * 2 + 1];
              }
              s_ += su; q_ += sq;
            }
          } else
          for (int c = tid * cpg; c < (tid + 1) * cpg; ++c) { s_ += (double)sCh[c * 2]; q_ += (double)sCh[c * 2 + 1]; }
          const double inv_n = 1.0 / ((double)cpg * (coop ? p.HWout : rows_per));
          const double mean = s_ * inv_n;
          double var = q_ * inv_n - mean * mean;
          var = var > 0.0 ? var : 0.0;
          sGm[tid * 2] = (float)mean;
          sGm[tid * 2 + 1] = (float)(1.0 / sqrt(var + (double)a.gn_eps));
          if (a.gn_mr && sM[row0] >= 0) { float* d = a.gn_mr + ((long)sMb[row0] * a.gn_groups + n0 / cpg + tid) * 2; d[0] = sGm[tid * 2]; d[1] = sGm[tid * 2 + 1]; }
        }
        __syncthreads();
        if (active) {
          const int g = (c4 * 4) / cpg;
          const float mean = sGm[g * 2], rstd = sGm[g * 2 + 1];
          const float4 gm = *reinterpret_cast<const float4*>(a.gn_gamma + n), bt = *reinterpret_cast<const float4*>(a.gn_beta + n);
          const float4 sc = make_float4(rstd * gm.x, rstd * gm.y, rstd * gm.z, rstd * gm.w);
          typedef T V4T __attribute__((ext_vector_type(4)));
          T* __restrict__ g16 = reinterpret_cast<T*>(a.gn_out16);
          const bool silu = a.gn_act == 1;
#pragma unroll 2
          for (int row = row0 + rg; row < row0 + rows_per; row += NT / 32) {
            const int m = sM[row];
            if (m < 0) continue;
            float4 w = *reinterpret_cast<const float4*>(sStage + row * SST + c4 * 4);
            w.x = (w.x - mean) * sc.x + bt.x; w.y = (w.y - mean) * sc.y + bt.y; w.z = (w.z - mean) * sc.z + bt.z; w.w = (w.w - mean) * sc.w + bt.w;
            if (silu) { w.x = silu_f(w.x); w.y = silu_f(w.y); w.z = silu_f(w.z); w.w = silu_f(w.w); }
            V4T h4; h4[0] = (T)w.x; h4[1] = (T)w.y; h4[2] = (T)w.z; h4[3] = (T)w.w;
            *reinterpret_cast<V4T*>(g16 + (long)m * a.cout + n) = h4;
            badn |= f16_over_v4<T>(h4);
            if (a.gn_out16_lo) {
              V4T l4; l4[0] = (T)(w.x - (float)h4[0]); l4[1] = (T)(w.y - (float)h4[1]); l4[2] = (T)(w.z - (float)h4[2]); l4[3] = (T)(w.w - (float)h4[3]);
              *reinterpret_cast<V4T*>(reinterpret_cast<T*>(a.gn_out16_lo) + (long)m * a.cout + n) = l4;
            }
          }
        }
        __syncthreads();
      }
    }
  }
  f16_guard_commit(p.ovf, bad16, STEDM_F16G_CONV_OUT16);
  f16_guard_commit(p.ovf, badn, STEDM_F16G_NORM);
  STAMP(6);
  if STEDM_DBG(p.dbg, 1024) { asm volatile("s_waitcnt vmcnt(0)" ::: "memory"); STAMP(4); }
}
#undef STAMP
#undef STAMPC

template <int KSMAX, bool GN = false>
static __global__ void __launch_bounds__(256) conv_splitk_reduce_kernel(const stedm_conv_args a, const int HW, const long plane, const int ksplit,
                                                                        const int qbs ,
                                                                        unsigned* const ovf ,
                                                                        const int slab_px = 256 ) {
  __shared__ float rpart[256 * 8];
  __shared__ float gsum[GN ? 8 * 8 : 1], gmr[GN ? 16 : 1];
  const int b = blockIdx.x, slab = blockIdx.y, nslab = gridDim.y;
  const int C = a.cout, Q = C >> 2, t = threadIdx.x;
  const int qb0 = blockIdx.z * qbs, QB = min(qbs, Q - qb0);
  const int npl = 256 / QB, tq = t % QB, tp = t / QB;
  const int px0 = slab * slab_px, px1 = min(HW, px0 + slab_px);
  const int n = (qb0 + tq) * 4;
  float s[4] = {0.f, 0.f, 0.f, 0.f}, q[4] = {0.f, 0.f, 0.f, 0.f};
  unsigned bad16 = 0u, badn = 0u;
  if (tp < npl) {
    float4 add = a.bias ? *reinterpret_cast<const float4*>(a.bias + n) : make_float4(0.f, 0.f, 0.f, 0.f);
    if (a.src16b_hi && a.bias_b) {
      const float4 b4 = *reinterpret_cast<const float4*>(a.bias_b + n);
      add.x += b4.x; add.y += b4.y; add.z += b4.z; add.w += b4.w;
    }
    if (a.emb) {
      const float4 e4 = *reinterpret_cast<const float4*>(a.emb + (long)b * a.emb_bstride + n);
      add.x += e4.x; add.y += e4.y; add.z += e4.z; add.w += e4.w;
    }
#pragma unroll 2
    for (int pix = px0 + tp; pix < px1; pix += npl) {
      const long o = ((long)b * HW + pix) * C + n;
      float4 pz[KSMAX];
#pragma unroll
      for (int z = 0; z < KSMAX; ++z)
        if (KSMAX == 2 || z < ksplit) pz[z] = *reinterpret_cast<const float4*>(a.ws + z * plane + o);
      float4 v = pz[0];
#pragma unroll
      for (int z = 1; z < KSMAX; ++z)
        if (KSMAX == 2 || z < ksplit) { v.x += pz[z].x; v.y += pz[z].y; v.z += pz[z].z; v.w += pz[z].w; }
      v.x += add.x; v.y += add.y; v.z += add.z; v.w += add.w;
      if (a.res) { const float4 r4 = *reinterpret_cast<const float4*>(a.res + (a.res_bmod ? o - (long)(b - b % a.res_bmod) * HW * C : o)); v.x += r4.x; v.y += r4.y; v.z += r4.z; v.w += r4.w; }
      if (GN || a.out) *reinterpret_cast<float4*>(a.out + o) = v;
      if (a.out16_hi) {
        const long o16 = a.out16_stride ? ((long)b * HW + pix) * a.out16_stride + n : o;
        if (a.mm_dtype == STEDM_F16) {
          f16x4 h4; h4[0] = (_Float16)v.x; h4[1] = (_Float16)v.y; h4[2] = (_Float16)v.z; h4[3] = (_Float16)v.w;
          *reinterpret_cast<f16x4*>(reinterpret_cast<_Float16*>(a.out16_hi) + o16) = h4;
          bad16 |= f16_over_v4<_Float16>(h4);
        } else {
          bf16x4 h4; h4[0] = (__bf16)v.x; h4[1] = (__bf16)v.y; h4[2] = (__bf16)v.z; h4[3] = (__bf16)v.w;
          *reinterpret_cast<bf16x4*>(reinterpret_cast<__bf16*>(a.out16_hi) + o16) = h4;
        }
      }
      s[0] += v.x; s[1] += v.y; s[2] += v.z; s[3] += v.w;
      q[0] += v.x * v.x; q[1] += v.y * v.y; q[2] += v.z * v.z; q[3] += v.w * v.w;
    }
    float* d = rpart + (tp * QB + tq) * 8;
#pragma unroll
    for (int j = 0; j < 4; ++j) { d[j] = s[j]; d[4 + j] = q[j]; }
  }
  f16_guard_commit(ovf, bad16, STEDM_F16G_CONV_OUT16);
  if (!a.chan_stats) return;
  __syncthreads();
  if (t < QB) {
    float su[4] = {0.f, 0.f, 0.f, 0.f}, sq[4] = {0.f, 0.f, 0.f, 0.f};
    for (int l = 0; l < npl; ++l) {
      const float* d = rpart + (l * QB + t) * 8;
#pragma unroll
      for (int j = 0; j < 4; ++j) { su[j] += d[j]; sq[j] += d[4 + j]; }
    }
    float* dst = a.chan_stats + (((long)b * nslab + slab) * C + (qb0 + t) * 4) * 2;
#pragma unroll
    for (int j = 0; j < 4; ++j) { dst[j * 2] = su[j]; dst[j * 2 + 1] = sq[j]; }
    if (GN) {
#pragma unroll
      for (int j = 0; j < 4; ++j) { gsum[t * 8 + j] = su[j]; gsum[t * 8 + 4 + j] = sq[j]; }
    }
  }
  if (GN) {
    const int cpg = C / a.gn_groups, ng = (QB * 4) / cpg;
    __syncthreads();
    if (t < ng) {
      double s_ = 0.0, q_ = 0.0;
      for (int c = t * cpg; c < (t + 1) * cpg; ++c) { s_ += (double)gsum[(c >> 2) * 8 + (c & 3)]; q_ += (double)gsum[(c >> 2) * 8 + 4 + (c & 3)]; }
      const double inv_n = 1.0 / ((double)cpg * HW);
      const double mean = s_ * inv_n;
      double var = q_ * inv_n - mean * mean;
      var = var > 0.0 ? var : 0.0;
      gmr[t * 2] = (float)mean;
      gmr[t * 2 + 1] = (float)(1.0 / sqrt(var + (double)a.gn_eps));
      if (a.gn_mr) { float* d = a.gn_mr + ((long)b * a.gn_groups + (qb0 * 4) / cpg + t) * 2; d[0] = gmr[t * 2]; d[1] = gmr[t * 2 + 1]; }
    }
    __syncthreads();
    if (tp < npl) {
      const int g = (tq * 4) / cpg;
      const float mean = gmr[g * 2], rstd = gmr[g * 2 + 1];
      const float4 gm = *reinterpret_cast<const float4*>(a.gn_gamma + n), bt = *reinterpret_cast<const float4*>(a.gn_beta + n);
      const float4 sc = make_float4(rstd * gm.x, rstd * gm.y, rstd * gm.z, rstd * gm.w);
      for (int pix = px0 + tp; pix < px1; pix += npl) {
        const long o = ((long)b * HW + pix) * C + n;
        float4 w = *reinterpret_cast<const float4*>(a.out + o);
        w.x = (w.x - mean) * sc.x + bt.x; w.y = (w.y - mean) * sc.y + bt.y; w.z = (w.z - mean) * sc.z + bt.z; w.w = (w.w - mean) * sc.w + bt.w;
        if (a.gn_act == 1) { w.x = silu_f(w.x); w.y = silu_f(w.y); w.z = silu_f(w.z); w.w = silu_f(w.w); }
        if (a.mm_dtype == STEDM_F16) {
          f16x4 h4; h4[0] = (_Float16)w.x; h4[1] = (_Float16)w.y; h4[2] = (_Float16)w.z; h4[3] = (_Float16)w.w;
          *reinterpret_cast<f16x4*>(reinterpret_cast<_Float16*>(a.gn_out16) + o) = h4;
          badn |= f16_over_v4<_Float16>(h4);
          if (a.gn_out16_lo) {
            f16x4 l4; l4[0] = (_Float16)(w.x - (float)h4[0]); l4[1] = (_Float16)(w.y - (float)h4[1]); l4[2] = (_Float16)(w.z - (float)h4[2]); l4[3] = (_Float16)(w.w - (float)h4[3]);
            *reinterpret_cast<f16x4*>(reinterpret_cast<_Float16*>(a.gn_out16_lo) + o) = l4;
          }
        } else {
          bf16x4 h4; h4[0] = (__bf16)w.x; h4[1] = (__bf16)w.y; h4[2] = (__bf16)w.z; h4[3] = (__bf16)w.w;
          *reinterpret_cast<bf16x4*>(reinterpret_cast<__bf16*>(a.gn_out16) + o) = h4;
          if (a.gn_out16_lo) {
            bf16x4 l4; l4[0] = (__bf16)(w.x - (float)h4[0]); l4[1] = (__bf16)(w.y - (float)h4[1]); l4[2] = (__bf16)(w.z - (float)h4[2]); l4[3] = (__bf16)(w.w - (float)h4[3]);
            *reinterpret_cast<bf16x4*>(reinterpret_cast<__bf16*>(a.gn_out16_lo) + o) = l4;
          }
        }
      }
      f16_guard_commit(ovf, badn, STEDM_F16G_NORM);
    }
  }
}

template <typename T, int WM, int KIND, bool FUSE = false, bool P3 = false>
static int conv_rs_try(ConvParams& p, const ConvParams& q, hipStream_t st, bool dry = false) {
  constexpr size_t LDS_MAX = 160 * 1024;
  constexpr int BMT = 256;
  constexpr bool G1 = KIND == RS_1X1M;
  constexpr bool SUBK = KIND == RS_SUB || KIND == RS_SUBM;
  constexpr bool M16 = KIND == RS_3X3M || G1 || KIND == RS_SUBM;
  constexpr bool K1 = KIND == RS_1X1 || KIND == RS_1X1N;
  constexpr int PPI = K1 ? 8 : (G1 ? 16 : 32), NPL = (SUBK || KIND == RS_3X3M) ? 2 : 1, NTAB = (KIND == RS_3X3 || KIND == RS_3X3M) ? 9 : 4;
  if ((KIND == RS_3X3M || G1) && q.a.mode != STEDM_CONV_S1) return -1;
  const size_t nai = (q.NP + PPI - 1) / PPI;
  if ((nai + 1) / 2 > (K1 ? 16 : 13)) return -1;
  bool stats = q.a.chan_stats != nullptr;
  if (stats && (K1 || G1) && !(BMT % q.HWout == 0 || q.HWout % BMT == 0)) stats = false;
  const bool s2d = SUBK && q.a.mode == STEDM_CONV_S2D;
  const int nrun = (q.HWout + 255) / 256;
  const int HWo = (SUBK && !s2d) ? 4 * q.HWout : q.HWout;
  const bool fine_ok = q.ksplit >= 2 && q.a.chan_nslab > 0 && HWo % q.a.chan_nslab == 0 && HWo / q.a.chan_nslab >= 8 && HWo / q.a.chan_nslab <= 256;
  if (stats && q.a.chan_nslab != 0 && q.a.chan_nslab != ((SUBK && !s2d) ? 4 * nrun : nrun) && !fine_ok) stats = false;
  if (stats && SUBK && !s2d && q.a.chan_nslab == 0) stats = false;
  if (stats && q.ksplit >= 2 && !fine_ok && q.a.chan_nslab != 0 && (HWo + 255) / 256 != q.a.chan_nslab) stats = false;
  size_t a_buf = NPL * nai * 1024 + (M16 ? 32 : 0);
  if (FUSE && a_buf < 32768) a_buf = 32768;
  if (P3) a_buf *= 2;
  const size_t ring = (P3 ? 3 : 4) * a_buf;
  const size_t loop = ring + (size_t)(M16 ? 1 : NTAB) * BMT * sizeof(int);
  const size_t staging = (size_t)BMT * kStageStride * sizeof(float) + (stats ? (size_t)((16 / WM + 2) * 2) * 128 * 2 * sizeof(float) + (128 + 32) * 2 * sizeof(float) : 0);
  const size_t lds = (size_t)2 * BMT * sizeof(int) + (loop > staging ? loop : staging);
  if (lds > LDS_MAX) return -1;
  auto magic = [](int d) { return (unsigned)((0x100000000ull + (unsigned)d - 1) / (unsigned)d); };
  const bool flat = (K1 || G1) && q.a.B == 1;
  if (((K1 || G1) && q.HWout >= 65536 && !flat) || q.PRs * q.PW >= 65536 || (!(K1 || G1) && (long)q.HWout * q.Wout >= (1l << 32))) return -1;
  if (KIND == RS_1X1N &&
      !(WM == 4 && !FUSE && flat && q.ksplit < 2 && q.Cin <= 256 && q.tiles_n >= 2 && q.a.cout % 8 == 0 && (long)q.tiles_m * 4 >= (long)stedm_device_cus() * 3 &&
        !q.a.chan_stats && !q.a.emb && !q.a.gn_out16 && !q.a.out16_lo && !q.a.ln_gamma &&
        (q.a.qkv_q || (long)q.tiles_m * 256 * q.a.cout * (q.a.out ? 4 : 2) < (q.a.cout % 128 ? (1l << 31) : (1l << 32))) &&
        (!q.a.qkv_q || ((long)q.tiles_m * 256 / q.a.qkv_T + 2) * q.a.qkv_heads * 64 * q.a.qkv_Tp * 2 < (1l << 32)) &&
        ((q.a.qkv_q && q.tiles_n >= 3) || (q.a.out && !q.a.out16_hi && !q.a.act_out) || (!q.a.out && q.a.out16_hi && !q.a.res && !q.a.qkv_q)) &&
        !getenv("STEDM_CONV_NO_NPERS")))
    return -1;
  if (q.a.ln_gamma && (KIND != RS_1X1 || q.tiles_n != 1 || q.ksplit >= 2)) return -1;
  if (!q.a.out && q.a.chan_stats && !stats) return -1;
  if (q.a.out16_stride && (KIND == RS_1X1N || P3)) return -1;
  const bool kwin = q.a.src16_cstride || q.a.k_chan0 || q.a.w_cin;
  if ((kwin || q.a.res_bmod) && !((KIND == RS_3X3 || KIND == RS_3X3M) && !FUSE && !P3)) return -1;
  if (dry) return 0;
  p = q;
  p.mg_hw = flat ? 0u : magic(p.HWout); p.mg_w = magic(p.Wout); p.mg_pw = magic(p.PW); p.mg_prpw = magic(p.PRs * p.PW);
  {
    const double abytes = (double)p.M * (p.Cin + (FUSE ? p.a.cb : 0)) * 2.0 * (P3 ? 2 : 1);
    const double wbytes = (double)p.a.cout * (p.Cin * p.taps + (FUSE ? p.a.cb : 0)) * 2.0 * (P3 ? 2 : 1);
    double best = abytes * (p.tiles_n < 8 ? p.tiles_n : 8) + wbytes;
    p.xcd_m = 0;
    if (p.tiles_n > 1)
      for (int gm = 8; gm >= 2; gm >>= 1) {
        const int gn = 8 / gm;
        if (p.tiles_m % gm != 0 || p.tiles_n % gn != 0) continue;
        const double cost = abytes * gn + wbytes * gm;
        if (cost < best * 0.97) { best = cost; p.xcd_m = gm; }
      }
  }
  {
    const stedm_conv_args& a_ = p.a;
    const int cpg = (a_.gn_out16 && a_.gn_groups > 0) ? a_.cout / a_.gn_groups : 0;
    p.gn_tile = (cpg > 0 && stats && q.ksplit < 2 && (KIND == RS_3X3 || KIND == RS_3X3M) && (!P3 || a_.gn_out16_lo) && p.HWout <= BMT && BMT % p.HWout == 0 &&
                 a_.cout % 128 == 0 && cpg % 4 == 0 && 128 % cpg == 0 && a_.out && !a_.out16_hi && !a_.act_out) ? 1 : 0;
  }
  p.gn_coop = 0;
  {
    const stedm_conv_args& a_ = p.a;
    const int cpg = (a_.gn_out16 && a_.gn_groups > 0) ? a_.cout / a_.gn_groups : 0;
    const int nt = p.HWout / BMT;
    static const bool off = getenv("STEDM_NO_GN_COOP") != nullptr;
    if (!p.gn_tile && !off && cpg > 0 && stats && q.ksplit < 2 && (KIND == RS_3X3 || KIND == RS_3X3M) && !FUSE && !P3 && p.HWout % BMT == 0 && nt >= 2 && nt <= 4 &&
        a_.cout == 128 && p.tiles_n == 1 && p.xcd_m == 0 && !p.whole && cpg % 4 == 0 && 128 % cpg == 0 && 256 % a_.gn_groups == 0 && a_.out && !a_.out16_hi && !a_.act_out &&
        a_.gn_coop && a_.gn_coop_epoch && a_.gn_coop_tmo && (size_t)lds + 4 * 128 * 2 * sizeof(float) <= LDS_MAX)
      p.gn_coop = nt;
  }
  p.npers = 0;
  if (KIND == RS_1X1N) {
    const long cus = stedm_device_cus() > 0 ? stedm_device_cus() : 256;
    auto cost = [&](int s_) { return ((long)p.tiles_m * s_ + cus - 1) / cus * (2 + p.tiles_n / s_); };
    p.npers = (p.tiles_n % 2 == 0 && p.tiles_n >= 4 && cost(2) < cost(1)) ? 2 : 1;
  }
  ConvParams kp = p;
  if (!stats) kp.a.chan_stats = nullptr;
  if (q.a.k_chan0) {
    kp.a.src16_hi = reinterpret_cast<const unsigned char*>(q.a.src16_hi) + (size_t)q.a.k_chan0 * 2;
    if (q.a.w_frag) kp.a.w_frag = reinterpret_cast<const unsigned char*>(q.a.w_frag) + (size_t)q.a.k_chan0 * 9 * 256;
    if (q.a.w_frag16) kp.a.w_frag16 = reinterpret_cast<const unsigned char*>(q.a.w_frag16) + (size_t)q.a.k_chan0 * 9 * 256;
  }
  auto k = conv_rs_kernel<T, WM, KIND, FUSE, P3>;
  const size_t lds_launch = lds + (p.gn_coop ? (size_t)4 * 128 * 2 * sizeof(float) : 0);
  static size_t lds_set = 0;
  if (lds_launch > lds_set) {
    hipError_t e = hipFuncSetAttribute(reinterpret_cast<const void*>(k), hipFuncAttributeMaxDynamicSharedMemorySize, (int)lds_launch);
    if (e != hipSuccess) { set_error("conv_igemm(rs): hipFuncSetAttribute(%zu) failed: %s", lds_launch, hipGetErrorString(e)); return 2; }
    lds_set = lds_launch;
  }
  if (kp.ksplit >= 2) kp.a.chan_stats = nullptr;
  k<<<p.npers ? p.tiles_m * p.npers : p.tiles_m * p.tiles_n * ((SUBK && !s2d) ? 4 : 1) * (kp.ksplit >= 2 ? kp.ksplit : 1), (16 / WM + 2) * 64, lds_launch, st>>>(kp);
  STEDM_LAUNCH_CHECK();
  if (kp.ksplit >= 2) {
    int qbs = 64;
    while (qbs > 8 && (long)p.a.B * ((HWo + 255) / 256) * ((p.a.cout / 4 + qbs - 1) / qbs) < 256) qbs >>= 1;
    const int cpg = (p.a.gn_out16 && p.a.gn_groups > 0) ? p.a.cout / p.a.gn_groups : 0;
    const bool gn = cpg > 0 && p.a.out && HWo <= 256 && !(SUBK && !s2d) && p.a.chan_stats && stats && (p.a.chan_nslab == 0 || p.a.chan_nslab == 1) && p.a.cout % 32 == 0 &&
                    cpg % 4 == 0 && 32 % cpg == 0;
    if (gn) qbs = 8;
    int slab_px = 256;
    if (!gn) {
      if (p.a.chan_stats && stats && fine_ok) slab_px = HWo / p.a.chan_nslab;
      else if (!p.a.chan_stats || !stats)
        while (slab_px > 16 && HWo % (slab_px / 2) == 0 && (long)p.a.B * ((HWo + slab_px - 1) / slab_px) * ((p.a.cout / 4 + 7) / 8) < 512) slab_px >>= 1;
      if (slab_px < 256) {
        qbs = 256 / (slab_px < 32 ? slab_px : 32);
        if (qbs > 64) qbs = 64;
      }
    }
    dim3 grid(p.a.B, (HWo + slab_px - 1) / slab_px, (p.a.cout / 4 + qbs - 1) / qbs);
    const long plane = (long)p.a.B * HWo * p.a.cout;
    stedm_conv_args ra = p.a;
    if (!stats) ra.chan_stats = nullptr;
    if (gn) {
      if (kp.ksplit == 2) conv_splitk_reduce_kernel<2, true><<<grid, 256, 0, st>>>(ra, HWo, plane, 2, qbs, p.ovf);
      else conv_splitk_reduce_kernel<16, true><<<grid, 256, 0, st>>>(ra, HWo, plane, kp.ksplit, qbs, p.ovf);
      p.gn_done = 1;
    } else if (kp.ksplit == 2) conv_splitk_reduce_kernel<2><<<grid, 256, 0, st>>>(ra, HWo, plane, 2, qbs, p.ovf, slab_px);
    else conv_splitk_reduce_kernel<16><<<grid, 256, 0, st>>>(ra, HWo, plane, kp.ksplit, qbs, p.ovf, slab_px);
    STEDM_LAUNCH_CHECK();
    stats = ra.chan_stats != nullptr;
  }
  if (stats) p.stats_done = 1;
  if (p.gn_tile || p.gn_coop) p.gn_done = 1;
  return 0;
}

template <typename T>
static int conv_rs_pick(ConvParams& p, hipStream_t st, bool dry = false) {
  const stedm_conv_args& a = p.a;
  const bool fuse = a.src16b_hi != nullptr;
  if (fuse && (a.ks != 3 || a.mode != STEDM_CONV_S1 || !a.w_frag_b || a.cb <= 0 || a.cb % 64 != 0 || a.res)) return -1;
  if ((!a.w_frag && !a.w_frag16) || (a.act_out != 0 && a.act_out != 2) || a.npass != 1 || a.mode == STEDM_CONV_DOWN) return -1;
  const bool s2d = a.mode == STEDM_CONV_S2D;
  const bool sp = (a.mode == STEDM_CONV_UP_SUBPIXEL || s2d) && p.taps == 4 && p.Cin % 32 == 0;
  if (s2d && !sp) return -1;
  const bool k3 = a.ks == 3 && p.taps == 9 && p.Cin % 16 == 0, k1 = a.ks == 1 && p.Cin % 64 == 0;
  if (!k3 && !k1 && !sp) return -1;
  if (a.qkv_q && (!k1 || fuse || !a.w_frag)) return -1;
  if (a.ln_gamma && (!k1 || fuse || !a.w_frag || a.cout > 128)) return -1;
  static int cus = 0;
  if (cus == 0) { cus = stedm_device_cus(); if (cus <= 0) cus = 256; }
  ConvParams q = p;
  if (!conv_geometry(q, 256, true)) return -1;
  q.ksplit = 0;
  auto pick_split = [&](long tiles, int nchunks, int planes = 1, int nchunks2 = 0) {
    if (!a.ws || (!a.out && !a.out16_hi) || a.out16_lo || a.act_out || a.cout % 4 != 0 || (a.emb && a.emb_bstride % 4 != 0) || a.ln_gamma || a.qkv_q) return 0;
    const int minc = tiles * 16 <= cus ? 1 : (tiles * 8 <= cus ? 2 : 4);
    int best = 0;
    for (int ks = 2; ks <= 16; ks *= 2) {
      if (nchunks % ks != 0 || nchunks / ks < minc || a.ws_floats < (long)ks * planes * p.M * a.cout || nchunks2 % ks != 0) break;
      best = ks;
      if (tiles * ks * 4 >= (long)cus * 3) break;
    }
    return best;
  };
  const bool subm = sp && a.w_frag16 && !a.w_frag;
  if (s2d) {
    q.ksplit = (long)q.tiles_m * q.tiles_n * 4 < (long)cus * 3 ? pick_split((long)q.tiles_m * q.tiles_n, p.Cin / 32) : 0;
    if (subm) { const int rc = conv_rs_try<T, 4, RS_SUBM>(p, q, st, dry); if (rc >= 0 || !a.w_frag) return rc; }
    return a.w_frag ? conv_rs_try<T, 4, RS_SUB>(p, q, st, dry) : -1;
  }
  const bool m16 = k3 && a.mode == STEDM_CONV_S1 && a.w_frag16 && p.Cin % 32 == 0 && p.Cin >= 256 && (!fuse || a.w_frag_b16);
  if (!a.w_frag && !m16 && !subm) return -1;
  if (fuse && !m16 && !a.w_frag_b) return -1;
  if ((long)q.tiles_m * q.tiles_n * (sp ? 4 : 1) * 4 < (long)cus * 3) {
    const int ks = k3 ? pick_split((long)q.tiles_m * q.tiles_n, p.Cin / (m16 ? 32 : 16), 1, fuse ? a.cb / 64 : 0)
                 : (k1 && !fuse)      ? pick_split((long)q.tiles_m * q.tiles_n, p.Cin / 64)
                 : sp                 ? pick_split((long)q.tiles_m * q.tiles_n * 4, p.Cin / 32, 4) : 0;
    const bool half_ok = k1 && (long)q.tiles_m * q.tiles_n * 2 >= cus;
    if (ks == 0 && !half_ok) return -1;
    q.ksplit = ks;
  }
  if (fuse) {
    if (!k3) return -1;
    int rc = m16 ? conv_rs_try<T, 4, RS_3X3M, true>(p, q, st, dry) : -1;
    if (rc >= 0 || !a.w_frag || !a.w_frag_b) return rc;
    if (m16) q.ksplit = 0;
    return conv_rs_try<T, 4, RS_3X3, true>(p, q, st, dry);
  }
  if (sp) {
    if (subm) { const int rc = conv_rs_try<T, 4, RS_SUBM>(p, q, st, dry); if (rc >= 0 || !a.w_frag) return rc; }
    return a.w_frag ? conv_rs_try<T, 4, RS_SUB>(p, q, st, dry) : -1;
  }
  if (k1) {
    const int rc = conv_rs_try<T, 4, RS_1X1N>(p, q, st, dry);
    return rc >= 0 ? rc : conv_rs_try<T, 4, RS_1X1>(p, q, st, dry);
  }
  if (m16) { const int rc = conv_rs_try<T, 4, RS_3X3M>(p, q, st, dry); if (rc >= 0 || !a.w_frag) return rc; q.ksplit = 0; }
  return conv_rs_try<T, 4, RS_3X3>(p, q, st, dry);
}

template <typename T>
static int conv_rs3_pick(ConvParams& p, hipStream_t st, bool dry = false) {
  const stedm_conv_args& a = p.a;
  const bool k1 = a.ks == 1 && p.taps == 1;
  const bool s2d = a.mode == STEDM_CONV_S2D;
  const bool sp = (a.mode == STEDM_CONV_UP_SUBPIXEL || s2d) && a.ks == 3 && p.taps == 4;
  if (a.npass != 3 || !a.w_frag16 || !a.src16_lo || a.src16b_hi || !(sp || ((k1 || (a.ks == 3 && p.taps == 9)) && a.mode == STEDM_CONV_S1)) ||
      p.Cin % 32 != 0 || p.Cin < (k1 ? 64 : 128) || (a.act_out != 0 && a.act_out != 2))
    return -1;
  static int cus = 0;
  if (cus == 0) { cus = stedm_device_cus(); if (cus <= 0) cus = 256; }
  ConvParams q = p;
  if (!conv_geometry(q, 256, true)) return -1;
// ... 19 lines not shown
```

stedm_amd/ops.py:

```python
from __future__ import annotations

import ctypes as C
from dataclasses import dataclass
from typing import Optional, Tuple

import torch

from . import _lib
from ._lib import BF16, CONV_DOWN, CONV_S1, CONV_S2D, CONV_UP, CONV_UP_SUBPIXEL, F16, ConvArgs, check, lib


@dataclass(frozen=True)
class Precision:
    mm_dtype: int = F16
    npass: int = 3
    attn_fp8: bool = False

    @staticmethod
    def parse(name: str) -> "Precision":
        table = {"parity": Precision(F16, 3), "parity_bf16": Precision(BF16, 3),
                 "fast": Precision(F16, 1), "f16": Precision(F16, 1), "bf16": Precision(BF16, 1),
                 "fp8": Precision(BF16, 1, True), "bf16+fp8attn": Precision(BF16, 1, True)}
        if name not in table:
            raise ValueError(f"unknown precision {name!r}; choose from {sorted(table)}")
# ... 340 lines not shown
        return self.frag(w4, cin * ks * ks, ks * ks, False, cout, cin, ks, m16)

    def _build_table(self, idxs):
        import struct
        rec, blk = [], 0
        for i in idxs:
            (w, sn, sc, flip, cout, cin, taps, m16, out) = self.items[i]
            rec.append(struct.pack("<QQqqiiiiii", w.data_ptr(), out.data_ptr(), sn, sc, cout, cin, taps, flip, m16, blk))
            blk += ((cout + 127) // 128) * ((cin // 32) * 4 if m16 else (cin // 16) * 2)
        if not rec:
            return None, 0, 0
        return torch.frombuffer(bytearray(b"".join(rec)), dtype=torch.uint8).to(self.items[0][0].device), blk, len(rec)

    def set_fused(self, idxs) -> None:
        self._fused = frozenset(idxs)
        self._rest = None
        self._fresh = None

    def mark_fresh(self, versions) -> None:
        self._fresh = versions

    def run(self, versions=None) -> None:
        if not self.items:
            return
        fresh, self._fresh = self._fresh, None
        if self._fused and versions is not None and fresh == versions:
            if self._rest is None:
                self._rest = self._build_table([i for i in range(len(self.items)) if i not in self._fused])
            table, blocks, n = self._rest
            if n:
                check(lib().stedm_pack_frag_multi(table.data_ptr(), n, blocks, self.prec.mm_dtype, _stream()), "stedm_pack_frag_multi")
            return
        if self._table is None:
            self._table, self._blocks, _ = self._build_table(range(len(self.items)))
        check(lib().stedm_pack_frag_multi(self._table.data_ptr(), len(self.items), self._blocks, self.prec.mm_dtype, _stream()), "stedm_pack_frag_multi")


def conv3x3_tiles_ok(Hout: int, Wout: int) -> bool:
    return bool(lib().stedm_conv3x3_tiles_ok(int(Hout), int(Wout)))


_GENERIC_COLS: dict = {}


def _conv3x3_generic(src16, w_hi, w_lo, out, *, prec: Precision, mode: int, **kw):
    assert kw.get("skip") is None, "the fused skip phase belongs to the tiled kernels (stedm_conv_fused_skip_ok says so)"
    B, H, W, C = src16[0].shape
    Ho, Wo = ((H - 1) // 2 + 1, (W - 1) // 2 + 1) if mode == CONV_DOWN else ((2 * H, 2 * W) if mode == CONV_UP else (H, W))
    cols = []
    for i, pl in enumerate(src16):
        if pl is None or (i == 1 and prec.npass != 3):
            cols.append(None)
            continue
        key = (pl.device, i, B, Ho, Wo, 9 * C)
        col = _GENERIC_COLS.get(key)
        if col is None:
            if len(_GENERIC_COLS) > 16:
                _GENERIC_COLS.clear()
            col = _GENERIC_COLS[key] = torch.empty((B, Ho, Wo, 9 * C), dtype=torch.int16, device=pl.device)
        check(lib().stedm_im2col_rows16(pl.data_ptr(), col.data_ptr(), B, H, W, C, {CONV_S1: 0, CONV_DOWN: 1, CONV_UP: 2}[mode], _stream()),
              "stedm_im2col_rows16")
        cols.append(col)
    if isinstance(w_hi, LazyPlanes):
        w_hi, w_lo = w_hi.get()
    cout = w_hi.shape[0]
    assert tuple(w_hi.shape) == (cout, 9, C), (tuple(w_hi.shape), cout, C)
    for k in ("w_frag", "w_frag16", "ks", "out16_stride", "cout"):
        kw.pop(k, None)
    return conv_igemm(None, w_hi.view(cout, 1, 9 * C), None if w_lo is None else w_lo.view(cout, 1, 9 * C), out, prec=prec, ks=1, mode=CONV_S1,
                      src16=(cols[0], cols[1]), **kw)


def conv_igemm(src1: Optional[torch.Tensor], w_hi: torch.Tensor, w_lo: Optional[torch.Tensor], out: torch.Tensor, *, prec: Precision,
               ks: int = 3, mode: int = CONV_S1, src2: Optional[torch.Tensor] = None, src2_bmod: int = 0,
               scale: Optional[torch.Tensor] = None, shift: Optional[torch.Tensor] = None, act: int = 0,
               bias: Optional[torch.Tensor] = None, emb: Optional[torch.Tensor] = None, emb_offset: int = 0,
               emb_bstride: int = 0, res: Optional[torch.Tensor] = None,
               src16: Optional[Tuple[torch.Tensor, Optional[torch.Tensor]]] = None, act_out: int = 0,
               out16: Optional[Tuple[torch.Tensor, Optional[torch.Tensor]]] = None, w_frag: Optional[torch.Tensor] = None,
               chan_stats: Optional[torch.Tensor] = None,
               skip: Optional[Tuple[torch.Tensor, torch.Tensor, Optional[torch.Tensor]]] = None, query_fused: bool = False, query_rs: bool = False,
               ws: Optional[torch.Tensor] = None, pad_br: bool = False, w_frag16: Optional[torch.Tensor] = None,
               gn_next: Optional[tuple] = None, qkv_planes: Optional[tuple] = None, ln_after: Optional[tuple] = None, coop: Optional[tuple] = None,
               out16_stride: int = 0, cout: Optional[int] = None, res_bmod: int = 0):
    if src16 is not None and src1 is None and ks == 3 and mode in (CONV_S1, CONV_DOWN, CONV_UP) and not out16_stride:
        _, H_, W_, _ = src16[0].shape
        Ho_, Wo_ = ((H_ - 1) // 2 + 1, (W_ - 1) // 2 + 1) if mode == CONV_DOWN else ((2 * H_, 2 * W_) if mode == CONV_UP else (H_, W_))
        if not conv3x3_tiles_ok(Ho_, Wo_):
            if query_fused or query_rs:
                return False
            if not src16[0].is_contiguous() or res_bmod:
                raise _lib.StedmHipError("conv_igemm: a K window / res_bmod belongs to the tiled register-streamed kernel; this output grid takes the im2col form")
            return _conv3x3_generic(src16, w_hi, w_lo, out, prec=prec, mode=mode, scale=scale, shift=shift, act=act, bias=bias, emb=emb,
                                    emb_offset=emb_offset, emb_bstride=emb_bstride, res=res, act_out=act_out, out16=out16, chan_stats=chan_stats,
                                    skip=skip, ws=ws, gn_next=gn_next)
    if out is not None:
        _chk(out, name="out")
    a = ConvArgs()
    a.act_out = act_out
    if gn_next is not None:
        g_w, g_b, g_eps, g_groups, g_act, g_out = gn_next[:6]
        g_lo = None
        if isinstance(g_out, (tuple, list)):
            g_out, g_lo = g_out[0], g_out[1]
        g_mr = gn_next[6] if len(gn_next) > 6 else None
        a.gn_only = int(bool(gn_next[7])) if len(gn_next) > 7 else 0
        if g_mr is not None:
            _chk(g_mr, name="gn mean_rstd")
            assert tuple(g_mr.shape) == (out.shape[0], int(g_groups), 2)
            a.gn_mr = g_mr.data_ptr()
        _chk(g_w, name="gn gamma"); _chk(g_b, name="gn beta")
        assert g_out.dtype == torch.int16 and g_out.is_contiguous() and tuple(g_out.shape) == tuple(out.shape) and chan_stats is not None
        assert src16 is None or all(t is None or t.data_ptr() != g_out.data_ptr() for t in src16), "gn_next planes alias the convolution's input planes"
        a.gn_gamma, a.gn_beta, a.gn_eps, a.gn_groups, a.gn_act, a.gn_out16 = g_w.data_ptr(), g_b.data_ptr(), float(g_eps), int(g_groups), int(g_act), g_out.data_ptr()
        if g_lo is not None:
            assert g_lo.dtype == torch.int16 and g_lo.is_contiguous() and tuple(g_lo.shape) == tuple(out.shape)
            assert src16 is None or all(t is None or t.data_ptr() != g_lo.data_ptr() for t in src16), "gn_next lo planes alias the convolution's input planes"
            a.gn_out16_lo = g_lo.data_ptr()
        assert prec.npass == 1 or g_lo is not None, "gn_next in a 3-product mode needs the (hi, lo) planes"
        if coop is not None:
            cwd, cw = coop
            assert cwd.dtype == torch.int64 and cwd.is_contiguous() and tuple(cwd.shape) == (out.shape[0], 4, 128, 2)
            assert cw.dtype == torch.int32 and cw.numel() >= 2
            a.gn_coop, a.gn_coop_epoch, a.gn_coop_tmo = cwd.data_ptr(), cw.data_ptr(), cw.data_ptr() + 4
    a.pad_br = int(pad_br)
    a.w_frag16 = _ptr(w_frag16)
    a.w_frag = _ptr(w_frag) if prec.npass == 1 else None
    a.chan_stats = _ptr(chan_stats)
    a.chan_nslab = 0 if chan_stats is None else chan_stats.shape[1]
    if ws is not None:
        a.ws = ws.data_ptr()
        a.ws_floats = ws.numel()
    if skip is not None:
        a.src16b_hi = skip[0].data_ptr()
        a.cb = skip[0].shape[-1]
        a.w_frag_b = skip[1].data_ptr()
        a.bias_b = _ptr(skip[2])
        a.w_frag_b16 = _ptr(skip[3]) if len(skip) > 3 and prec.npass == 1 else None
    if out16 is not None:
        a.out16_hi = out16[0].data_ptr()
        a.out16_lo = _ptr(out16[1]) if prec.npass == 3 else None
        if out16_stride:
            assert cout is not None and out is None and prec.npass == 1 and out16[0].shape[-1] == out16_stride and out16[0].is_contiguous()
            a.out16_stride = int(out16_stride)
    if ln_after is not None:
        l_g, l_b, l_eps, l_res = ln_after
        _chk(l_g, name="ln gamma"); _chk(l_b, name="ln beta")
        assert res is None and prec.npass == 1 and (out is not None or out16 is not None)
        a.ln_gamma, a.ln_beta, a.ln_eps = l_g.data_ptr(), l_b.data_ptr(), float(l_eps)
        if l_res is not None:
            _chk(l_res, name="ln residual")
            a.ln_res = l_res.data_ptr()
    if qkv_planes is not None:
        qq, qk, qv, qT, qTp, qH, qs = qkv_planes
        assert out is None and out16 is None and prec.npass == 1 and src16 is not None
        nb = src16[0].shape[2] // int(qT)
        for t_, shp in ((qq, (nb * qH, qTp, 64)), (qk, (nb * qH, qTp, 64)), (qv, (nb * qH, 64, qTp))):
            assert t_.dtype == torch.int16 and t_.is_contiguous() and tuple(t_.shape) == shp, (tuple(t_.shape), shp)
        a.qkv_q, a.qkv_k, a.qkv_vt = qq.data_ptr(), qk.data_ptr(), qv.data_ptr()
        a.qkv_T, a.qkv_Tp, a.qkv_heads, a.qkv_qscale = int(qT), int(qTp), int(qH), float(qs)
        oshape = (1, 1, src16[0].shape[2], 3 * int(qH) * 64)
    else:
        oshape = out.shape if out is not None else out16[0].shape
        if cout is not None:
            oshape = tuple(oshape[:-1]) + (int(cout),)
    if src1 is not None:
        _chk(src1, name="src1")
        B, Hin, Win, c1 = src1.shape
        a.src1 = src1.data_ptr()
        a.src2 = _ptr(src2)
        c2 = 0 if src2 is None else src2.shape[-1]
    else:
        B, Hin, Win, c1 = src16[0].shape
        c2 = 0
    kwin = False
    if src16 is not None:
        s16 = src16[0]
        assert s16.dtype == torch.int16 and tuple(s16.shape) == (B, Hin, Win, c1 + c2)
        a.src16_hi = s16.data_ptr()
        a.src16_lo = _ptr(src16[1]) if prec.npass == 3 else None
        if not s16.is_contiguous():
            cs = s16.stride(2)
            base = s16._base if s16._base is not None else s16
            k0 = (s16.storage_offset() - base.storage_offset()) % cs
            assert src1 is None and tuple(s16.stride()) == (Hin * Win * cs, Win * cs, cs, 1) and k0 + c1 <= cs, \
                "src16[0] must be contiguous or a view plane[b0:b1, :, :, k0:k1] of a contiguous plane"
            assert cs % 32 == 0 and k0 % 32 == 0 and c1 % 32 == 0, "a K window is cut on 32-channel boundaries"
            kwin = True
            a.src16_hi = s16.data_ptr() - 2 * k0
            if a.src16_lo is not None:
                assert tuple(src16[1].stride()) == tuple(s16.stride()) and src16[1].storage_offset() == s16.storage_offset()
                a.src16_lo = src16[1].data_ptr() - 2 * k0
            a.src16_cstride, a.k_chan0 = cs, k0
            wplanes = w_hi._val[0] if isinstance(w_hi, LazyPlanes) and w_hi._val is not None else (None if isinstance(w_hi, LazyPlanes) else w_hi)
            a.w_cin = (w_frag.shape[-5] * 16 if w_frag is not None and prec.npass == 1 else
                       w_frag16.shape[-5] * 32 if w_frag16 is not None else wplanes.shape[-1] if wplanes is not None else cs)
            assert w_frag is None or w_frag16 is None or w_frag.shape[-5] * 16 == w_frag16.shape[-5] * 32
    a.res_bmod = int(res_bmod)
    if res_bmod:
        assert res is not None and res.is_contiguous() and res.dtype == torch.float32 and B % res_bmod == 0 and res.shape[0] >= res_bmod
    a.c1, a.c2, a.src2_bmod = c1, c2, src2_bmod
    a.B, a.Hin, a.Win = B, Hin, Win
    a.mode, a.ks = mode, ks
    a.scale, a.shift, a.act = _ptr(scale), _ptr(shift), act
    lazy = w_hi if isinstance(w_hi, LazyPlanes) else None
    if lazy is not None:
        w_hi, w_lo = lazy._val if lazy._val is not None else (w_frag if w_frag is not None else w_frag16, None)
    a.w_hi, a.w_lo = _ptr(w_hi), (_ptr(w_lo) if prec.npass == 3 else None)
    a.bias = _ptr(bias)
    a.emb = None if emb is None else emb.data_ptr() + 4 * emb_offset
    a.emb_bstride = emb_bstride
    a.res = _ptr(res)
    a.out = _ptr(out)
    a.cout = oshape[-1]
    a.npass, a.mm_dtype = prec.npass, prec.mm_dtype
    if lazy is not None and lazy._val is None:
        if src16 is None or (w_frag is None and w_frag16 is None) or prec.npass != 1 or not lib().stedm_conv_rs_ok(C.byref(a)):
            w_hi, w_lo = lazy.get()
            a.w_hi, a.w_lo = _ptr(w_hi), (_ptr(w_lo) if prec.npass == 3 else None)
    elif mode == CONV_UP_SUBPIXEL:
        assert w_hi.shape == (4 * a.cout, 4, a.c1 + a.c2), (w_hi.shape, a.cout, a.c1, a.c2)
    elif mode == CONV_S2D:
        assert w_hi is None and (w_frag is not None or w_frag16 is not None) and src1 is None, \
            "the space-to-depth form runs on the register-streamed kernel only"
    else:
        assert w_hi.shape == (a.cout, ks * ks, a.w_cin if kwin else a.c1 + a.c2), (w_hi.shape, a.cout, ks, a.c1, a.c2)
    if query_fused:
        return bool(lib().stedm_conv_fused_skip_ok(C.byref(a)))
    if query_rs:
        return bool(lib().stedm_conv_rs_ok(C.byref(a)))
    check(lib().stedm_conv_igemm(C.byref(a), _stream()), "stedm_conv_igemm")
    return out


def conv_in(x1: torch.Tensor, x2: Optional[torch.Tensor], w: torch.Tensor, bias: Optional[torch.Tensor], out: torch.Tensor,
            x2_bmod: int = 0, chan_stats: Optional[torch.Tensor] = None) -> bool:
    _chk(x1, name="x1")
    B, c1, H, W = x1.shape
    c2 = 0 if x2 is None else x2.shape[1]
    if x2 is not None:
        _chk(x2, name="x2")
    args = (x1.data_ptr(), c1, _ptr(x2), c2, x2_bmod, w.data_ptr(), _ptr(bias), out.data_ptr(), B, H, W, out.shape[-1])
    if chan_stats is not None and H % 2 == 0:
        assert tuple(chan_stats.shape) == (B, H // 2, out.shape[-1], 2) and chan_stats.dtype == torch.float32
        rc = lib().stedm_conv_in(*args, chan_stats.data_ptr(), _stream())
        if rc == 0:
            return True
        if rc != 3:
            check(rc, "stedm_conv_in")
    check(lib().stedm_conv_in(*args, None, _stream()), "stedm_conv_in")
    return False


def conv_out_weight(w_oihw: torch.Tensor) -> torch.Tensor:
    cout, c = w_oihw.shape[:2]
    cp = 4 if cout <= 4 else 8
    w = torch.zeros((3, 3, c, cp), dtype=torch.float32, device=w_oihw.device)
    w[..., :cout] = w_oihw.detach().float().permute(2, 3, 1, 0)
    return w.contiguous()


def conv_out(src: torch.Tensor, norm_weight: torch.Tensor, norm_bias: torch.Tensor, eps: float, groups: int, w: torch.Tensor,
             bias: Optional[torch.Tensor], out: torch.Tensor, chan_stats: Optional[torch.Tensor] = None) -> torch.Tensor:
    _chk(src, name="src")
    B, H, W, c = src.shape
    cout = out.shape[1]
    if w.dim() == 4 and tuple(w.shape[:3]) != (3, 3, c):
        w = conv_out_weight(w)
    assert tuple(w.shape) == (3, 3, c, 4 if cout <= 4 else 8)
    if chan_stats is None:
        chan_stats = torch.empty((B, gn_chan_nslab(H * W), c, 2), dtype=torch.float32, device=src.device)
        gn_chan_stats(src, chan_stats)
    check(lib().stedm_conv_out(src.data_ptr(), c, chan_stats.data_ptr(), chan_stats.shape[1], norm_weight.data_ptr(), norm_bias.data_ptr(), float(eps),
                               groups, w.data_ptr(), _ptr(bias), out.data_ptr(), B, H, W, out.shape[1], _stream()), "stedm_conv_out")
    return out


def time_embed(t: torch.Tensor, freqs: torch.Tensor, w0t: torch.Tensor, b0: torch.Tensor, w2t: torch.Tensor, b2: torch.Tensor,
               out: torch.Tensor, ws: Optional[torch.Tensor] = None) -> torch.Tensor:
    if t.dtype == torch.float32:
        fn, name = lib().stedm_time_embed_f32, "stedm_time_embed_f32"
    else:
        _chk(t, torch.int64, "timesteps")
        fn, name = lib().stedm_time_embed, "stedm_time_embed"
    _chk(t, t.dtype, "timesteps")
    B = t.shape[0]
    mc, ted = w0t.shape
    if ws is None:
        ws = torch.empty((B * (mc + ted),), dtype=torch.float32, device=t.device)
    assert ws.numel() >= B * (mc + ted)
    check(fn(t.data_ptr(), freqs.data_ptr(), w0t.data_ptr(), b0.data_ptr(), w2t.data_ptr(), b2.data_ptr(),
             out.data_ptr(), ws.data_ptr(), B, mc, ted, _stream()), name)
    return out


def emb_proj(emb: torch.Tensor, wt: torch.Tensor, bias: torch.Tensor, out: torch.Tensor) -> torch.Tensor:
    _chk(emb, name="emb")
    B, K = emb.shape
    assert wt.shape[0] == K and out.shape == (B, wt.shape[1])
    check(lib().stedm_emb_proj(emb.data_ptr(), wt.data_ptr(), bias.data_ptr(), out.data_ptr(), B, K, wt.shape[1], _stream()),
          "stedm_emb_proj")
    return out


def linear(x: torch.Tensor, wt: torch.Tensor, bias: Optional[torch.Tensor], out: torch.Tensor, act_in: int = 0, act_out: int = 0):
    _chk(x, name="x")
    B, K = x.shape
    check(lib().stedm_linear(x.data_ptr(), wt.data_ptr(), _ptr(bias), out.data_ptr(), B, K, wt.shape[1], act_in, act_out, _stream()),
          "stedm_linear")
    return out


def svit_patch_embed(img, ln_w, ln_b, eps, wt, bias, pos, cls, x, patch: int):
    _chk(img, name="style images")
# ... 910 lines not shown
```

stedm_amd/unet.py:

```python
from __future__ import annotations

import math
import os
from typing import Dict, List, Optional, Tuple

import torch
import torch.nn as nn

from . import ops
from ._lib import BF16, F16, CONV_S2D, CONV_DOWN, CONV_S1, CONV_UP, CONV_UP_SUBPIXEL, StedmHipError
from .ops import Precision


def zero_module(module: nn.Module) -> nn.Module:
    for p in module.parameters():
        p.detach().zero_()
    return module


class GroupNorm32(nn.GroupNorm):
    """util.py:214-216 (container; eps 1e-5, 32 groups)."""


class TimestepBlock(nn.Module):
# ... 104 lines not shown
            assert num_head_channels != -1, "Either num_heads or num_head_channels has to be set"
        if num_head_channels == -1:
            assert num_heads != -1, "Either num_heads or num_head_channels has to be set"

        self.image_size = image_size
        self.in_channels = in_channels
        self.model_channels = model_channels
        self.out_channels = out_channels
        self.num_res_blocks = num_res_blocks
        self.attention_resolutions = attention_resolutions
        self.dropout = dropout
        self.channel_mult = channel_mult
        self.conv_resample = conv_resample
        self.num_classes = num_classes
        self.use_checkpoint = use_checkpoint
        self.dtype = torch.float32
        self.num_heads = num_heads
        self.num_head_channels = num_head_channels
        self.num_heads_upsample = num_heads_upsample
        self.predict_codebook_ids = False
        self.precision = Precision.parse(precision) if isinstance(precision, str) else precision

        ted = model_channels * 4
        self.time_embed = nn.Sequential(nn.Linear(model_channels, ted), nn.SiLU(), nn.Linear(ted, ted))
        self.input_blocks = nn.ModuleList([TimestepEmbedSequential(nn.Conv2d(in_channels, model_channels, 3, padding=1))])
        input_block_chans = [model_channels]
        ch, ds = model_channels, 1
        for level, mult in enumerate(channel_mult):
            for _ in range(num_res_blocks):
                if ds in attention_resolutions:
                    raise TypeError("list.append() takes exactly one argument (0 given) "
                                    "[reference openaimodel.py:580: ds in attention_resolutions is not constructible]")
                self.input_blocks.append(TimestepEmbedSequential(ResBlock(ch, ted, dropout, out_channels=mult * model_channels)))
                ch = mult * model_channels
                input_block_chans.append(ch)
            if level != len(channel_mult) - 1:
                self.input_blocks.append(TimestepEmbedSequential(Downsample(ch, conv_resample, out_channels=ch)))
                input_block_chans.append(ch)
                ds *= 2
        if num_head_channels != -1:
            num_heads = ch // num_head_channels
        dim_head = ch // num_heads if use_spatial_transformer else num_head_channels
        if use_spatial_transformer:
            from .attention import SpatialTransformer
            mid_attn = SpatialTransformer(ch, num_heads, dim_head, depth=transformer_depth, context_dim=context_dim)
        else:
            mid_attn = AttentionBlock(ch, num_heads=num_heads, num_head_channels=dim_head)
        self.middle_block = TimestepEmbedSequential(
            ResBlock(ch, ted, dropout),
            ResBlockStyle(ch, ted, dropout),
            mid_attn,
            ResBlock(ch, ted, dropout),
        )
        self.output_blocks = nn.ModuleList([])
        for level, mult in list(enumerate(channel_mult))[::-1]:
            for i in range(num_res_blocks + 1):
                ich = input_block_chans.pop()
                layers: List[nn.Module] = [ResBlock(ch + ich, ted, dropout, out_channels=model_channels * mult)]
                ch = model_channels * mult
                if ds in attention_resolutions:
                    raise TypeError("reference output block with ds in attention_resolutions is not runnable (openaimodel.py:689-698)")
                if level and i == num_res_blocks:
                    layers.append(Upsample(ch, conv_resample, out_channels=ch))
                    ds //= 2
                self.output_blocks.append(TimestepEmbedSequential(*layers))
        self.out = nn.Sequential(GroupNorm32(32, ch), nn.SiLU(), zero_module(nn.Conv2d(model_channels, out_channels, 3, padding=1)))

        self._packed: Dict[int, _Packed] = {}
        self._pack_key = None
        self._bufs: Dict[Tuple, torch.Tensor] = {}
        self._emb_layout: List[Tuple[ResBlock, int]] = []
        self._consts: Dict[str, torch.Tensor] = {}
        self._m16 = True
        self._gn_slot = 0
        self._style_cache: Dict[Tuple, torch.Tensor] = {}
        self._cs: Dict[int, torch.Tensor] = {}
        self._raw16: Dict[int, Tuple] = {}
        self._saved16: Dict = {}
        self._saved_mr: Dict = {}
        self._mr_ctr = 0
        self._plane_ctr = 0
        self._tape: Optional[list] = None
        self.cfg_shared_skip: Optional[bool] = None

    def convert_to_fp16(self):
        pass

    def convert_to_fp32(self):
        pass

    def set_precision(self, precision) -> None:
        self.precision = Precision.parse(precision) if isinstance(precision, str) else precision
        self.invalidate()

    def invalidate(self) -> None:
        self._style_cache.clear()
        self._consts.clear()
        self._pack_key = None
        self._values_gen = getattr(self, "_values_gen", 0) + 1

    def check_f16_range(self, where: str = "UNetModel.forward") -> None:
        ops.f16_guard_check(where)

    def freshness_token(self, versions=None):
        if versions is None:
            versions = tuple(p._version for p in self.parameters())
        return (versions, getattr(self, "_values_gen", 0), ops.raw_write_epoch())

    def _buf(self, name: str, shape, dtype=torch.float32) -> torch.Tensor:
        key = (name, tuple(shape), dtype)
        t = self._bufs.get(key)
        if t is None:
            dev = next(self.parameters()).device
            t = torch.empty(tuple(shape), dtype=dtype, device=dev)
            self._bufs[key] = t
        return t

    def _timestep_blocks(self) -> List[ResBlock]:
        out = []
        for blk in list(self.input_blocks) + [self.middle_block] + list(self.output_blocks):
            for layer in blk:
                if isinstance(layer, ResBlock):
                    out.append(layer)
        return out

    def _prepare(self) -> None:
        params = list(self.parameters())
        dev = params[0].device
        if dev.type != "cuda":
            raise StedmHipError("UNetModel.forward needs its parameters on the GPU; there is no CPU fallback")
        ptrs = tuple(p.data_ptr() for p in params)
        key = (self.precision, dev, tuple(p._version for p in params), ptrs)
        if key == self._pack_key:
            return
        prec = self.precision
        if prec.mm_dtype == F16:
            ops.f16_guard_enable()
        ptr_key = (prec, dev, ptrs, self._m16)
        plan = getattr(self, "_plan", None)
        replay = plan is not None and self._plan_key == ptr_key and len(self._packed) > 0
        if not replay:
            self._packed.clear()
            plan = self._plan = ops.PackPlan(prec)
            self._plan_key = ptr_key
        self._consts.clear()
        self._style_cache.clear()

        def pack(conv):
            if replay:
                pk = self._packed[id(conv)]
                if isinstance(pk.hi, ops.LazyPlanes):
                    pk.hi.reset()
                else:
                    pk.hi, pk.lo = ops.pack_conv_weight(conv.weight.float(), prec)
                    if pk.frag16 is not None:
                        wf = conv.weight.detach().float()
                        pk.frag16 = ops.pack_conv_weight_frag16((wf.unsqueeze(-1) if wf.dim() == 3 else wf).contiguous(), prec)
                return
            hi = lo = frag = None
            w4 = conv.weight.detach().float()
            if w4.dim() == 3:
                w4 = w4.unsqueeze(-1)
            in_place = w4.is_contiguous() and w4.data_ptr() == conv.weight.data_ptr()
            if not in_place:
                self._plan_key = None
            k3 = tuple(w4.shape[2:]) == (3, 3) and conv.stride == (1, 1) and conv.in_channels % 16 == 0
# ... 207 lines not shown
        pk2 = self._packed[id(rb.out_layers[3])]
        o16 = None
        if want16:
            o16 = self._planes(B, H, W, co, "up16")
            self._raw16[out.data_ptr()] = o16
        gnn, npl, coop2 = None, None, None
        if next_norm is not None and self._tape is None and o16 is None and next_cat is None and not os.environ.get("STEDM_NO_NEXT_GN"):
            nn_, nact = next_norm
            npl = self._planes(B, H, W, co)
            gnn = (nn_.weight, nn_.bias, nn_.eps, nn_.num_groups, nact, npl if prec.npass == 3 else npl[0], None, False)
            coop2 = self._coop_for(tag + ".c2", B, H, W, co, prec)

        def filed():
            if gnn is not None:
                self._pre16[out.data_ptr()] = (id(next_norm[0]), next_norm[1], npl)
            return out
        if has_skip:
            ps = self._packed[id(rb.skip_connection)]
            h16 = h16_next if h16_next is not None else self._norm16(rb.out_layers[0], 1, h)
            fuse_key = ("fuse", id(rb), B, H, W)
            fused = self._consts.get(fuse_key)
            kw = dict(prec=prec, src16=h16, bias=pk2.bias, w_frag=pk2.frag, chan_stats=self._cs_new(out), ws=ws, out16=o16, w_frag16=pk2.frag16)
            if fused is None:
                fused = bool((pk2.frag is not None or pk2.frag16 is not None) and ps.frag is not None and
                             ops.conv_igemm(None, pk2.hi, pk2.lo, out, skip=(x16[0], ps.frag, ps.bias, ps.frag16), query_fused=True, **kw))
                self._consts[fuse_key] = fused
            if fused and next_cat is not None and o16 is None:
                keyc = ("fusecat", id(rb), B, H, W, next_cat)
                okc = self._consts.get(keyc)
                rawn = self._cat_plane(B, H, W, co, next_cat)
                kwc = dict(kw, out16=(rawn, None), out16_stride=next_cat, cout=co)
                if okc is None:
                    okc = bool(ops.conv_igemm(None, pk2.hi, pk2.lo, None, skip=(x16[0], ps.frag, ps.bias, ps.frag16), query_fused=True, **kwc))
                    self._consts[keyc] = okc
                if okc:
                    ops.conv_igemm(None, pk2.hi, pk2.lo, None, skip=(x16[0], ps.frag, ps.bias, ps.frag16), **kwc)
                    self._x16[out.data_ptr()] = (rawn, co)
                    return out
            only16 = False
            if fused and o16 is not None and self._tape is None and prec.npass == 1:
                key16 = ("fuse16", id(rb), B, H, W)
                only16 = self._consts.get(key16)
                if only16 is None:
                    only16 = bool(ops.conv_igemm(None, pk2.hi, pk2.lo, None, skip=(x16[0], ps.frag, ps.bias, ps.frag16), query_fused=True,
                                                 **dict(kw, chan_stats=None)))
                    self._consts[key16] = only16
            if only16:
                kw.update(chan_stats=None)
                self._cs.pop(out.data_ptr(), None)
                ops.conv_igemm(None, pk2.hi, pk2.lo, None, skip=(x16[0], ps.frag, ps.bias, ps.frag16), **kw)
            elif fused:
                ops.conv_igemm(None, pk2.hi, pk2.lo, out, skip=(x16[0], ps.frag, ps.bias, ps.frag16), gn_next=gnn, **kw)
                return filed()
            else:
                ops.conv_igemm(None, ps.hi, ps.lo, out, prec=prec, ks=1, src16=x16, bias=ps.bias, w_frag=ps.frag, ws=ws,
                               w_frag16=ps.frag16 if prec.npass == 3 else None)
                ops.conv_igemm(None, pk2.hi, pk2.lo, out, res=out, gn_next=gnn, **kw)
                return filed()
            return out
        assert x2 is None
        h16 = h16_next if h16_next is not None else self._norm16(rb.out_layers[0], 1, h)
        if next_cat is not None and o16 is None:
            rawn = self._cat_plane(B, H, W, co, next_cat)
            kwc = dict(prec=prec, src16=h16, bias=pk2.bias, res=x1, w_frag=pk2.frag, chan_stats=self._cs_new(out), ws=ws, w_frag16=pk2.frag16,
                       out16=(rawn, None), out16_stride=next_cat, cout=co)
            keyc = ("rescat", id(rb), B, H, W, next_cat)
            okc = self._consts.get(keyc)
            if okc is None:
                okc = bool(ops.conv_igemm(None, pk2.hi, pk2.lo, None, query_rs=True, **kwc))
                self._consts[keyc] = okc
            if okc:
                ops.conv_igemm(None, pk2.hi, pk2.lo, None, **kwc)
                self._x16[out.data_ptr()] = (rawn, co)
                return out
        ops.conv_igemm(None, pk2.hi, pk2.lo, out, prec=prec, src16=h16, bias=pk2.bias, res=x1, w_frag=pk2.frag,
                       chan_stats=self._cs_new(out), ws=ws, out16=o16, w_frag16=pk2.frag16, gn_next=gnn, coop=coop2)
        return filed()

    def _in_conv(self, tag: str, rb: ResBlock, pk, a16, c1: int, x2_bmod: int, h, kw) -> None:
        plan = self._shared_skip(rb, pk, a16, c1, x2_bmod, h, kw)
        if plan is None:
            ops.conv_igemm(None, pk.hi, pk.lo, h, src16=a16, **kw)
            return
        seam, P = plan
        Bs = P.shape[0]
        ops.conv_igemm(None, pk.hi, pk.lo, P, prec=kw["prec"], src16=(a16[0][:Bs, :, :, seam:], None), w_frag=pk.frag, w_frag16=pk.frag16, ws=kw["ws"])
        ops.conv_igemm(None, pk.hi, pk.lo, h, src16=(a16[0][:, :, :, :seam], None), res=P, res_bmod=Bs, **kw)

    def _shared_skip(self, rb: ResBlock, pk, a16, c1: int, x2_bmod: int, h, kw):
        Bd, H, W, co = h.shape
        if (self.cfg_shared_skip is False or self._tape is not None or self.precision.npass != 1 or x2_bmod <= 0 or Bd != 2 * x2_bmod or
                a16[0].shape[0] != Bd or not a16[0].is_contiguous()):
            return None
        key = ("sskip", id(rb), Bd, H, W, self.cfg_shared_skip)
        hit = self._consts.get(key)
        if hit is None:
            norm = rb.in_layers[0]
            C = a16[0].shape[-1]
            cpg = C // norm.num_groups
            seam = -(-(-(-c1 // cpg) * cpg) // 32) * 32
            if (C - seam) // 32 > 1 and ((C - seam) // 32) % 2:
                seam += 32
            hit = 0
            if 32 <= seam <= C - 32 and (pk.frag is not None or pk.frag16 is not None):
                P = self._buf(f"sskip.P.{x2_bmod}x{H}x{W}x{co}", (x2_bmod, H, W, co))
                ok = bool(ops.conv_igemm(None, pk.hi, pk.lo, P, prec=kw["prec"], src16=(a16[0][:x2_bmod, :, :, seam:], None), w_frag=pk.frag,
                                         w_frag16=pk.frag16, ws=kw["ws"], query_rs=True))
                ok = ok and bool(ops.conv_igemm(None, pk.hi, pk.lo, h, src16=(a16[0][:, :, :, :seam], None), res=P, res_bmod=x2_bmod, query_rs=True, **kw))
                if ok and (self.cfg_shared_skip or self._shared_skip_rule(Bd, H, W, co, C, seam)):
                    hit = seam
            self._consts[key] = hit
        if not hit:
            return None
        return hit, self._buf(f"sskip.P.{x2_bmod}x{H}x{W}x{co}", (x2_bmod, H, W, co))

    @staticmethod
    def _shared_skip_rule(Bd: int, H: int, W: int, co: int, C: int, seam: int) -> bool:
        cus = ops.device_cus()

        def fills(b):
            tiles_m = -(-b * H * W // 256) if H * W >= 256 else -(-b // (256 // (H * W)))
            return tiles_m * -(-co // 128) * 4 >= cus * 3
        if not fills(Bd):
            return False
        return (C - seam) // 32 >= (14 if fills(Bd // 2) else 32)

    def _attn(self, tag: str, ab: AttentionBlock, x):
        prec = self.precision
        B, H, W, Cc = x.shape
        pq = self._packed[id(ab.qkv)]
        pp = self._packed[id(ab.proj_out)]
        out = self._buf(tag + ".out", (B, H, W, Cc))
        ch = Cc // ab.num_heads
        if prec.npass == 1 and self._tape is None and ch in (16, 32, 64, 128):
            qkv16 = self._planes(B, H, W, 3 * Cc, "qkv16")
            ops.conv_igemm(None, pq.hi, pq.lo, None, prec=prec, ks=1, src16=self._norm16(ab.norm, 0, x), bias=pq.bias, w_frag=pq.frag,
                           out16=qkv16)
            a16 = self._planes(B, H, W, Cc, "attn16")
            ops.attn_legacy16(qkv16[0].view(B, H * W, 3 * Cc), a16[0], ab.num_heads, prec)
            ops.conv_igemm(None, pp.hi, pp.lo, out, prec=prec, ks=1, src16=a16, bias=pp.bias, res=x, w_frag=pp.frag,
                           chan_stats=self._cs_new(out), ws=self._splitk_ws(out.numel()))
            return out
        qkv = self._buf(tag + ".qkv", (B, H, W, 3 * Cc))
        ops.conv_igemm(None, pq.hi, pq.lo, qkv, prec=prec, ks=1, src16=self._norm16(ab.norm, 0, x), bias=pq.bias, w_frag=pq.frag,
                       w_frag16=pq.frag16 if prec.npass == 3 else None)
        a = self._buf(tag + ".a", (B, H, W, Cc))
        ops.attn_legacy(qkv.view(B, H * W, 3 * Cc), a.view(B, H * W, Cc), ab.num_heads)
        if self._tape is not None:
            self._tape.append(("attn", ab, x, qkv, a, out))
        ops.conv_igemm(None, pp.hi, pp.lo, out, prec=prec, ks=1, src16=self._norm16(None, 0, a), bias=pp.bias, res=x, w_frag=pp.frag,
                       chan_stats=self._cs_new(out), w_frag16=pp.frag16 if prec.npass == 3 else None)
        return out

    def _down(self, ltag: str, layer: Downsample, h):
        pk = self._packed[id(layer.op)]
        B, H, W, _ = h.shape
        out = self._buf(ltag + ".out", (B, H // 2, W // 2, layer.out_channels))
        if self._tape is not None:
            self._tape.append(("down", layer, h, out))
        ps2 = self._packed.get((id(layer.op), "s2d"))
        if H % 2 == 0 and W % 2 == 0 and not ops.conv3x3_tiles_ok(H // 2, W // 2):
            return ops.conv_igemm(None, pk.hi, pk.lo, out, prec=self.precision, mode=CONV_DOWN, src16=self._norm16(None, 0, h), bias=pk.bias,
                                  chan_stats=self._cs_new(out))
        elif ps2 is not None and H % 2 == 0 and W % 2 == 0 and (H // 2) * (W // 2) >= 16:
            C = h.shape[-1]
            planes = self._buf(f"s2d16.{B}x{H}x{W}x{C}", (B, H // 2, W // 2, 4 * C), torch.int16)
            planes_lo = self._buf(f"s2d16lo.{B}x{H}x{W}x{C}", (B, H // 2, W // 2, 4 * C), torch.int16) if self.precision.npass == 3 else None
            ws = self._splitk_ws(out.numel())
            kw2 = dict(prec=self.precision, mode=CONV_S2D, src16=(planes, planes_lo), bias=ps2.bias, w_frag=ps2.frag, w_frag16=ps2.frag16, ws=ws)
            if self.precision.npass == 3 and not ops.conv_igemm(None, None, None, out, query_rs=True, **kw2):
                return ops.conv_igemm(h, pk.hi, pk.lo, out, prec=self.precision, mode=CONV_DOWN, bias=pk.bias)
            else:
                ops.space_to_depth16(h, planes, planes_lo, self.precision)
                return ops.conv_igemm(None, None, None, out, chan_stats=self._cs_new(out), **kw2)
        else:
            return ops.conv_igemm(h, pk.hi, pk.lo, out, prec=self.precision, mode=CONV_DOWN, bias=pk.bias)

    def _up(self, ltag: str, layer: Upsample, h, nxt, cat_ok, next_skip_c):
        pk = self._packed[id(layer.conv)]
        B, H, W, _ = h.shape
        out = self._buf(ltag + ".out", (B, H * 2, W * 2, layer.out_channels))
        if self._tape is not None:
            self._tape.append(("up", layer, h, out))
        pu = self._packed[(id(layer.conv), "up")]
        src16 = self._raw16.get(h.data_ptr()) or self._norm16(None, 0, h)
        if not ops.conv3x3_tiles_ok(H, W):
            return ops.conv_igemm(None, pk.hi, pk.lo, out, prec=self.precision, mode=CONV_UP, src16=src16, bias=pk.bias,
                                  chan_stats=self._cs_new(out))
        ws = self._splitk_ws(out.numel()) if self.precision.npass == 1 else None
        kwu = dict(prec=self.precision, mode=CONV_UP_SUBPIXEL, src16=src16, bias=pu.bias, w_frag=pu.frag,
                   chan_stats=self._cs_new(out, 4 * ops.gn_chan_nslab(H * W)), w_frag16=pu.frag16, ws=ws)
        if cat_ok and nxt is None and ops.gn_apply16c_x16_ok(layer.out_channels, next_skip_c):
            ncat = layer.out_channels + next_skip_c
            rawn = self._cat_plane(B, 2 * H, 2 * W, layer.out_channels, ncat)
            kwc = dict(kwu, out16=(rawn, None), out16_stride=ncat, cout=layer.out_channels)
            keyc = ("upcat", id(layer), B, H, W, ncat)
            okc = self._consts.get(keyc)
            if okc is None:
                okc = bool(ops.conv_igemm(None, pu.hi, pu.lo, None, query_rs=True, **kwc))
                self._consts[keyc] = okc
            if okc:
                ops.conv_igemm(None, pu.hi, pu.lo, None, **kwc)
                self._x16[out.data_ptr()] = (rawn, layer.out_channels)
                return out
        return ops.conv_igemm(None, pu.hi, pu.lo, out, **kwu)

    @staticmethod
    def _first_norm(layer):
# ... 67 lines not shown
        c = self._consts
        key = tuple((cx.data_ptr(), cx._version, tuple(cx.shape)) for cx in contexts) + (self._pack_key is not None and id(c["style_wt"]),)
        hit = self._style_cache.get(key)
        if hit is not None:
            return hit[0]
        nrep = len(contexts)
        if nrep == 1:
            ctx_all = contexts[0].float().contiguous()
        else:
            ctx_all = torch.cat([cx.float() for cx in contexts], dim=0).contiguous()
        style_all = ops.emb_proj(ctx_all, c["style_wt"], c["style_b"],
                                 torch.empty((B * nrep, c["style_wt"].shape[1]), dtype=torch.float32, device=ctx_all.device))
        if len(self._style_cache) > 8:
            self._style_cache.clear()
        self._style_cache[key] = (style_all, tuple(contexts))
        return style_all

    def _forward_impl(self, x, c_concat, timesteps, contexts, out, uniform_t=False):
        self._prepare()
        self._cs = {}
        self._raw16 = {}
        self._x16 = {}
        self._catpp = 0
        self._pre16 = {}
        if getattr(self, "_coop_state", None) is None or self._coop_state.device != x.device:
            self._coop_bufs, self._coop_state = {}, ops.coop_words_new()
        self._coop_advanced = False
        self._saved16 = {}
        self._saved_mr = {}
        self._plane_ctr = 0
        self._mr_ctr = 0
        x = x.float().contiguous()
        B, c1, H, W = x.shape
        nrep = len(contexts)
        Bd = B * nrep

        c2 = 0
        if c_concat is not None:
            c_concat = c_concat.float().contiguous()
            c2 = c_concat.shape[1]
        assert c1 + c2 == self.in_channels, f"expected {self.in_channels} input channels, got {c1}+{c2}"
        if any(cx is None for cx in contexts):
            raise ValueError("context (style vector) is required: middle_block[1] is a ResBlockStyle (openaimodel.py:636-643)")
        if not isinstance(timesteps, torch.Tensor):
            timesteps = torch.as_tensor(timesteps)
        t_float = timesteps.is_floating_point()
        if t_float and self._tape is not None:
            raise TypeError("fractional (floating) timesteps are an inference path: the training forward takes integer timesteps")
        timesteps = timesteps.to(device=x.device, dtype=torch.float32 if t_float else torch.int64).contiguous()
        c = self._consts
        ted = self.model_channels * 4
        for cx in contexts:
            assert tuple(cx.shape) == (B, ted), f"context must be [B,{ted}] (ResBlockStyle uses it as the embedding)"
        Bt = 1 if uniform_t else B
        emb = ops.time_embed(timesteps[:Bt], c["freqs"], c["te_w0t"], c["te_b0"], c["te_w2t"], c["te_b2"], self._buf("emb", (Bt, ted)),
                             self._buf("emb_ws", (Bt * (self.model_channels + ted),)))
        emb_e = ops.emb_proj(emb, c["emb_wt"], c["emb_b"], self._buf("emb_all", (Bt, self._emb_ntot)))
        emb_stride = 0 if uniform_t else self._emb_ntot
        if nrep == 1 or uniform_t:
            emb_d = emb_e
        else:
            emb_d = self._buf("emb_all_d", (Bd, self._emb_ntot))
            emb_d.view(nrep, B, self._emb_ntot).copy_(emb_e.unsqueeze(0).expand(nrep, B, self._emb_ntot))
        style_all = self._style_proj(contexts, B, ted)

        conv0 = self.input_blocks[0][0]
        h = self._buf("in0.out", (B, H, W, self.model_channels))
        if H % 2 == 0:
            cs0 = self._cs_new(h, H // 2)
            if not ops.conv_in(x, c_concat, conv0.weight, conv0.bias, h, chan_stats=cs0):
                del self._cs[h.data_ptr()]
        else:
            ops.conv_in(x, c_concat, conv0.weight, conv0.bias, h)
        if self._tape is not None:
            self._tape.append(("conv_in", x, c_concat, h))
            self._tape_emb = (timesteps, emb, contexts[0])
        hs = [h]
        mid = list(self.middle_block)
        nblk = len(self.input_blocks)
        for i, blk in enumerate(self.input_blocks[1:], start=1):
            nl = list(self.input_blocks[i + 1])[0] if i + 1 < nblk else mid[0]
            h = self._run_block(f"in{i}", blk, h, None, emb_e, emb_stride, None, next_layer=nl)
            hs.append(h)
        h = self._run_block("mid.a", mid[:1], h, None, emb_e, emb_stride, None, next_layer=mid[1] if nrep == 1 and len(mid) > 1 else None)
        if nrep > 1:
            h2 = self._buf("mid.rep", (Bd,) + tuple(h.shape[1:]))
            cs1 = self._cs.get(h.data_ptr())
            cs2 = self._cs_new(h2, nslab=cs1.shape[1]) if cs1 is not None else None
            h2.view((nrep,) + tuple(h.shape)).copy_(h.unsqueeze(0).expand((nrep,) + tuple(h.shape)))
            if cs2 is not None:
                cs2.view((nrep,) + tuple(cs1.shape)).copy_(cs1.unsqueeze(0).expand((nrep,) + tuple(cs1.shape)))
            h = h2
        def first_takes_cat(blk):
            l0 = list(blk)[0]
            return isinstance(l0, ResBlock) and not isinstance(l0.skip_connection, nn.Identity)

        ob = list(self.output_blocks)
        h = self._run_block("mid.b", mid[1:], h, None, emb_d, emb_stride, style_all, li0=1,
                            next_skip_c=hs[-1].shape[-1] if ob and first_takes_cat(ob[0]) else None)
        bmod = B if nrep > 1 else 0
        for i, blk in enumerate(ob):
            skip = hs.pop()
            nsc = hs[-1].shape[-1] if (i + 1 < len(ob) and first_takes_cat(ob[i + 1])) else None
            h = self._run_block(f"out{i}", blk, h, skip, emb_d, emb_stride, style_all, skip_bmod=bmod, next_skip_c=nsc)
        if out is None:
            out = torch.empty((Bd, self.out_channels, H, W), dtype=torch.float32, device=x.device)
        gn = self.out[0]
        cs = self._chan_stats(h)
        ops.conv_out(h, gn.weight, gn.bias, gn.eps, gn.num_groups, c["out_w_hwio"], self.out[2].bias, out, cs)
        if self._tape is not None:
            self._tape.append(("conv_out", h, out))
        return out
```

Before: 166.8 steps/s.

## Share CFG-duplicated conv work via partials-only pass and broadcast finish

Adds a partials-only conv entry and a separate split-K finish pass that can broadcast one batch's partial sums across the replicated CFG batch (ws_bmod). The middle block's first style ResBlock now runs its first 3x3 conv once on the un-replicated batch and applies the per-branch style embedding in the finish, which avoids computing that conv twice. It also allows the shared-skip path to split its skip conv into two partial planes summed through a new res2 epilogue input. This adds kernel launches, extra workspace traffic and more dispatch conditions, and is gated by probing and heuristics.

```diff
diff --git a/include/stedm_hip.h b/include/stedm_hip.h
--- a/include/stedm_hip.h
+++ b/include/stedm_hip.h
@@ -7,7 +7,7 @@
 extern "C" {
 #endif
 
-#define STEDM_ABI_VERSION 23
+#define STEDM_ABI_VERSION 24
 
 #define STEDM_F16 0
 #define STEDM_BF16 1
@@ -132,12 +132,16 @@
   int32_t k_chan0;
   int32_t w_cin;
   int32_t res_bmod;
+  const float* res2;
+  int32_t ws_bmod;
 } stedm_conv_args;
 int stedm_conv_igemm(const stedm_conv_args* args, void* stream);
 int stedm_conv_fused_skip_ok(const stedm_conv_args* args);
 int stedm_conv3x3_tiles_ok(int Hout, int Wout);
 int stedm_im2col_rows16(const void* src16, void* dst16, int B, int Hs, int Ws, int C, int mode, void* stream);
 int stedm_conv_rs_ok(const stedm_conv_args* args);
+int stedm_conv_partials(const stedm_conv_args* args, int32_t* nshare, int dry, void* stream);
+int stedm_conv_finish(const stedm_conv_args* args, int nshare, void* stream);
 
 int stedm_conv_in(const float* x1, int c1, const float* x2, int c2, int x2_bmod, const float* w_oihw,
                   const float* bias, float* out, int B, int H, int W, int cout, float* chan_stats, void* stream);
diff --git a/stedm_amd/_lib.py b/stedm_amd/_lib.py
--- a/stedm_amd/_lib.py
+++ b/stedm_amd/_lib.py
@@ -6,7 +6,7 @@
 _HERE = os.path.dirname(os.path.abspath(__file__))
 LIB_PATH = os.environ.get("STEDM_HIP_LIB") or os.path.join(_HERE, "libstedm_hip.so")
 
-ABI_VERSION = 23
+ABI_VERSION = 24
 F16, BF16 = 0, 1
 CONV_S1, CONV_DOWN, CONV_UP, CONV_UP_SUBPIXEL, CONV_S2D = 0, 1, 2, 3, 4
 
@@ -40,6 +40,7 @@
         ("out16_stride", C.c_int32),
         ("gn_coop", C.c_void_p), ("gn_coop_epoch", C.c_void_p), ("gn_coop_tmo", C.c_void_p),
         ("src16_cstride", C.c_int32), ("k_chan0", C.c_int32), ("w_cin", C.c_int32), ("res_bmod", C.c_int32),
+        ("res2", C.c_void_p), ("ws_bmod", C.c_int32),
     ]
 
 
@@ -82,6 +83,8 @@
     "stedm_conv_igemm": (_I, [C.POINTER(ConvArgs), _P]),
     "stedm_conv_fused_skip_ok": (_I, [C.POINTER(ConvArgs)]),
     "stedm_conv_rs_ok": (_I, [C.POINTER(ConvArgs)]),
+    "stedm_conv_partials": (_I, [C.POINTER(ConvArgs), C.POINTER(C.c_int32), _I, _P]),
+    "stedm_conv_finish": (_I, [C.POINTER(ConvArgs), _I, _P]),
     "stedm_conv_in": (_I, [_P, _I, _P, _I, _I, _P, _P, _P, _I, _I, _I, _I, _P, _P]),
     "stedm_conv_out": (_I, [_P, _I, _P, _I, _P, _P, _F, _I, _P, _P, _P, _I, _I, _I, _I, _P]),
     "stedm_time_embed": (_I, [_P, _P, _P, _P, _P, _P, _P, _P, _I, _I, _I, _P]),
diff --git a/stedm_amd/csrc/conv_common.hpp b/stedm_amd/csrc/conv_common.hpp
--- a/stedm_amd/csrc/conv_common.hpp
+++ b/stedm_amd/csrc/conv_common.hpp
@@ -25,6 +25,8 @@
   int gn_tile;
   int gn_coop;
   int xcd_m;
+  int partials;
+  int nshare;
   int npers;
   unsigned* ovf;
   int dbg;
@@ -67,4 +69,5 @@
 namespace stedm {
 bool conv_geometry(ConvParams& p, int bm, bool allow_wsplit = false);
 int conv_launch_dma(ConvParams& p, hipStream_t st, bool dry = false);
+int conv_splitk_finish(ConvParams& p, int nshare, hipStream_t st);
 }
diff --git a/stedm_amd/csrc/conv_dma_bf16_p1.hip b/stedm_amd/csrc/conv_dma_bf16_p1.hip
--- a/stedm_amd/csrc/conv_dma_bf16_p1.hip
+++ b/stedm_amd/csrc/conv_dma_bf16_p1.hip
@@ -4,7 +4,7 @@
 int conv_dma_pick_bf16_p1(ConvParams& p, hipStream_t st, bool dry) {
   int rc = conv_rs_pick<__bf16>(p, st, dry);
   if (rc >= 0 || dry || p.a.src16b_hi || p.a.mode == STEDM_CONV_S2D || p.a.qkv_q || p.a.ln_gamma) return rc;
-  if (p.a.src16_cstride || p.a.k_chan0 || p.a.w_cin || p.a.res_bmod || p.a.out16_stride) return rc;
+  if (p.a.src16_cstride || p.a.k_chan0 || p.a.w_cin || p.a.res_bmod || p.a.res2 || p.partials || p.a.out16_stride) return rc;
   rc = dma9_pick<__bf16>(p, st);
   return rc >= 0 ? rc : dma_pick<1, __bf16>(p, st);
 }
diff --git a/stedm_amd/csrc/conv_dma_f16_p1.hip b/stedm_amd/csrc/conv_dma_f16_p1.hip
--- a/stedm_amd/csrc/conv_dma_f16_p1.hip
+++ b/stedm_amd/csrc/conv_dma_f16_p1.hip
@@ -4,8 +4,9 @@
 int conv_dma_pick_f16_p1(ConvParams& p, hipStream_t st, bool dry) {
   int rc = conv_rs_pick<_Float16>(p, st, dry);
   if (rc >= 0 || dry || p.a.src16b_hi || p.a.mode == STEDM_CONV_S2D || p.a.qkv_q || p.a.ln_gamma) return rc;
-  if (p.a.src16_cstride || p.a.k_chan0 || p.a.w_cin || p.a.res_bmod || p.a.out16_stride) return rc;
+  if (p.a.src16_cstride || p.a.k_chan0 || p.a.w_cin || p.a.res_bmod || p.a.res2 || p.partials || p.a.out16_stride) return rc;
   rc = dma9_pick<_Float16>(p, st);
   return rc >= 0 ? rc : dma_pick<1, _Float16>(p, st);
 }
+int conv_splitk_finish(ConvParams& p, int nshare, hipStream_t st) { return splitk_finish_impl(p, nshare, st); }
 }
diff --git a/stedm_amd/csrc/conv_igemm.hip b/stedm_amd/csrc/conv_igemm.hip
--- a/stedm_amd/csrc/conv_igemm.hip
+++ b/stedm_amd/csrc/conv_igemm.hip
@@ -316,13 +316,34 @@
 }
 
 extern "C" int stedm_conv_rs_ok(const stedm_conv_args* args) {
-  if (!args || !args->src16_hi || (!args->w_frag && !args->w_frag16) || (args->npass != 1 && !args->w_frag16)) return 0;
+  if (!args || !args->src16_hi || (!args->w_frag && !args->w_frag16) || (args->npass != 1 && !args->w_frag16) || args->ws_bmod) return 0;
   ConvParams p;
   memset(&p, 0, sizeof(p));
   p.a = *args;
   if (conv_setup(p) != 0) return 0;
   return conv_launch_dma(p, nullptr, true) == 0 ? 1 : 0;
 }
+
+static int conv_trailing(ConvParams& p, void* stream) {
+  const stedm_conv_args& a = p.a;
+  int rc = 0;
+  if (a.chan_stats && !p.stats_done && !a.out) {
+    set_error("conv_igemm: the 16-bit-only form with chan_stats ran on a kernel without the statistics epilogue");
+    return 1;
+  }
+  if (a.chan_stats && !p.stats_done) {
+    const int up = (a.mode == STEDM_CONV_UP || a.mode == STEDM_CONV_UP_SUBPIXEL) ? 4 : 1, down = a.mode == STEDM_CONV_DOWN ? 4 : 1;
+    rc = stedm_gn_chan_stats(a.out, a.cout, a.B, a.Hin * a.Win * up / down, a.chan_nslab, a.chan_stats, stream);
+    if (rc != 0) return rc;
+  }
+  if (a.gn_out16 && !p.gn_done) {
+    const int HW = a.Hin * a.Win;
+    rc = stedm_gn_apply16c_mr(a.out, a.cout, a.chan_stats, a.chan_nslab > 0 ? a.chan_nslab : stedm_gn_chan_nslab(HW), nullptr, 0, nullptr, 0, 0, a.gn_gamma,
+                              a.gn_beta, a.gn_eps, a.gn_groups, a.gn_act, a.B, HW, a.gn_out16, a.gn_out16_lo, nullptr, nullptr, a.gn_mr, a.mm_dtype, stream);
+  }
+  return rc;
+}
+
 
 extern "C" int stedm_conv_igemm(const stedm_conv_args* args, void* stream) {
   STEDM_CHECK_ARG(args, "conv_igemm: null args");
@@ -338,23 +359,64 @@
                                   (a.npass == 1 || a.gn_out16_lo) && a.mode == STEDM_CONV_S1 && (a.gn_act == 0 || a.gn_act == 1)),
                   "conv_igemm: gn_out16 needs out, chan_stats, gamma / beta, groups dividing cout, stride 1 and a single-product mode (or gn_out16_lo)");
   STEDM_CHECK_ARG(!a.gn_out16_lo || a.gn_out16, "conv_igemm: gn_out16_lo without gn_out16");
+  STEDM_CHECK_ARG(a.ws_bmod == 0, "conv_igemm: ws_bmod belongs to stedm_conv_finish");
   int rc = conv_dispatch(p, stream);
   if (rc != 0) return rc;
-  if (a.chan_stats && !p.stats_done && !a.out) {
-    set_error("conv_igemm: the 16-bit-only form with chan_stats ran on a kernel without the statistics epilogue");
-    return 1;
-  }
-  if (a.chan_stats && !p.stats_done) {
-    const int up = (a.mode == STEDM_CONV_UP || a.mode == STEDM_CONV_UP_SUBPIXEL) ? 4 : 1, down = a.mode == STEDM_CONV_DOWN ? 4 : 1;
-    rc = stedm_gn_chan_stats(a.out, a.cout, a.B, a.Hin * a.Win * up / down, a.chan_nslab, a.chan_stats, stream);
-    if (rc != 0) return rc;
-  }
-  if (a.gn_out16 && !p.gn_done) {
-    const int HW = a.Hin * a.Win;
-    rc = stedm_gn_apply16c_mr(a.out, a.cout, a.chan_stats, a.chan_nslab > 0 ? a.chan_nslab : stedm_gn_chan_nslab(HW), nullptr, 0, nullptr, 0, 0, a.gn_gamma,
-                              a.gn_beta, a.gn_eps, a.gn_groups, a.gn_act, a.B, HW, a.gn_out16, a.gn_out16_lo, nullptr, nullptr, a.gn_mr, a.mm_dtype, stream);
-  }
-  return rc;
+  return conv_trailing(p, stream);
+}
+
+extern "C" int stedm_conv_partials(const stedm_conv_args* args, int32_t* nshare, int dry, void* stream) {
+  STEDM_CHECK_ARG(args && nshare, "conv_partials: null args");
+  ConvParams p;
+  memset(&p, 0, sizeof(p));
+  p.a = *args;
+  stedm_conv_args& a = p.a;
+  STEDM_CHECK_ARG(a.ws && !a.act_out && !a.out16_lo && a.ws_bmod == 0 && a.cout > 0 && a.cout % 4 == 0 && (!a.emb || a.emb_bstride % 4 == 0),
+                  "conv_partials: needs ws, no act_out / out16_lo / ws_bmod, cout %% 4 == 0 (and emb_bstride %% 4 == 0 for the finish pass)");
+  STEDM_CHECK_ARG(a.src16_hi && !a.src1 && a.c2 == 0 && a.ks == 3 && a.mode == STEDM_CONV_S1 && a.npass == 1 && !a.src16b_hi && (a.w_frag || a.w_frag16) && !a.ln_gamma && !a.qkv_q,
+                  "conv_partials: needs a plain 3x3 stride-1 single-product problem on src16 planes with w_frag / w_frag16 and no fused skip phase");
+  STEDM_CHECK_ARG(a.ws_floats >= (int64_t)a.B * a.Hin * a.Win * a.cout, "conv_partials: ws_floats=%lld holds no partial of %d x %d x %d x %d", (long long)a.ws_floats, a.B, a.Hin, a.Win, a.cout);
+  a.out = a.ws;
+  a.bias = a.bias_b = a.emb = a.res = a.res2 = nullptr;
+  a.res_bmod = 0;
+  a.out16_hi = nullptr; a.out16_stride = 0;
+  a.chan_stats = nullptr; a.chan_nslab = 0;
+  a.gn_out16 = a.gn_out16_lo = a.gn_coop = nullptr; a.gn_mr = nullptr; a.gn_only = 0;
+  p.partials = 1;
+  int rc;
+  if (dry) {
+    rc = conv_setup(p);
+    if (rc == 0) rc = conv_launch_dma(p, nullptr, true);
+  } else rc = conv_dispatch(p, stream);
+  if (rc != 0) return rc;
+  *nshare = p.nshare;
+  return 0;
+}
+
+extern "C" int stedm_conv_finish(const stedm_conv_args* args, int nshare, void* stream) {
+  STEDM_CHECK_ARG(args, "conv_finish: null args");
+  ConvParams p;
+  memset(&p, 0, sizeof(p));
+  p.a = *args;
+  const stedm_conv_args& a = p.a;
+  STEDM_CHECK_ARG(a.B > 0 && a.Hin > 0 && a.Win > 0 && a.cout > 0 && a.cout % 4 == 0 && (a.mm_dtype == STEDM_F16 || a.mm_dtype == STEDM_BF16), "conv_finish: bad sizes / mm_dtype");
+  STEDM_CHECK_ARG(nshare >= 1 && nshare <= 16 && a.ws, "conv_finish: nshare=%d must be 1 .. 16 partial planes in ws", nshare);
+  STEDM_CHECK_ARG(a.ws_bmod >= 0 && (a.ws_bmod == 0 || a.B % a.ws_bmod == 0), "conv_finish: ws_bmod=%d must divide B=%d", a.ws_bmod, a.B);
+  STEDM_CHECK_ARG(a.ws_floats >= (int64_t)nshare * (a.ws_bmod ? a.ws_bmod : a.B) * a.Hin * a.Win * a.cout, "conv_finish: ws_floats=%lld is short of %d partial planes", (long long)a.ws_floats, nshare);
+  STEDM_CHECK_ARG((a.out || a.out16_hi) && !a.out16_lo && !a.act_out && !a.src16b_hi && !a.ln_gamma && !a.qkv_q && a.mode == STEDM_CONV_S1 && (!a.emb || a.emb_bstride % 4 == 0),
+                  "conv_finish: needs out or out16_hi, stride 1, emb_bstride %% 4 == 0 and none of out16_lo / act_out / fused skip / LayerNorm / qkv");
+  STEDM_CHECK_ARG(a.res_bmod >= 0 && (a.res_bmod == 0 || a.res) && (!a.res2 || a.res), "conv_finish: res_bmod / res2 need res");
+  STEDM_CHECK_ARG(!a.chan_stats || a.out || a.out16_hi, "conv_finish: chan_stats needs an output");
+  STEDM_CHECK_ARG(a.out16_stride == 0 || (a.out16_hi && a.out16_stride >= a.cout && a.out16_stride % 4 == 0), "conv_finish: out16_stride needs out16_hi, stride >= cout, a multiple of 4");
+  STEDM_CHECK_ARG(!a.gn_out16 || (a.out && a.chan_stats && a.gn_gamma && a.gn_beta && a.gn_groups > 0 && a.cout % a.gn_groups == 0 && (a.npass == 1 || a.gn_out16_lo) &&
+                                  (a.gn_act == 0 || a.gn_act == 1)),
+                  "conv_finish: gn_out16 needs out, chan_stats, gamma / beta, groups dividing cout and a single-product mode (or gn_out16_lo)");
+  STEDM_CHECK_ARG(!a.gn_out16_lo || a.gn_out16, "conv_finish: gn_out16_lo without gn_out16");
+  p.HWout = a.Hin * a.Win;
+  p.ovf = a.mm_dtype == STEDM_F16 ? f16_guard_flag() : nullptr;
+  const int rc = conv_splitk_finish(p, nshare, as_stream(stream));
+  if (rc != 0) return rc;
+  return conv_trailing(p, stream);
 }
 
 static int conv_setup(ConvParams& p) {
@@ -402,6 +464,8 @@
     STEDM_CHECK_ARG(a.res_bmod == 0 || (a.res_bmod > 0 && a.res && plain3),
                     "conv_igemm: res_bmod=%d needs res and a plain 3x3 stride-1 single-product problem on src16 planes with w_frag / w_frag16 and no fused skip phase",
                     a.res_bmod);
+    STEDM_CHECK_ARG(!a.res2 || (a.res && plain3 && a.cout % 4 == 0),
+                    "conv_igemm: res2 needs res, cout %% 4 == 0 and a plain 3x3 stride-1 single-product problem on src16 planes with w_frag / w_frag16 and no fused skip phase");
   }
   p.taps = (a.mode == STEDM_CONV_UP_SUBPIXEL || a.mode == STEDM_CONV_S2D) ? 4 : a.ks * a.ks;
   if (a.mode == STEDM_CONV_UP_SUBPIXEL || a.mode == STEDM_CONV_S2D) {
diff --git a/stedm_amd/csrc/conv_igemm_dma.hip b/stedm_amd/csrc/conv_igemm_dma.hip
--- a/stedm_amd/csrc/conv_igemm_dma.hip
+++ b/stedm_amd/csrc/conv_igemm_dma.hip
@@ -27,8 +27,8 @@
   if (dry) return rc < 0 ? 1 : 0;
   if (rc < 0 && a.ln_gamma) { set_error("conv_igemm(dma): the register-streamed kernel does not run this LayerNorm-epilogue problem (see stedm_conv_rs_ok)"); return 1; }
   if (rc < 0 && a.qkv_q) { set_error("conv_igemm(dma): the register-streamed kernel does not run this qkv-epilogue problem (see stedm_conv_rs_ok)"); return 1; }
-  if (rc < 0 && (a.src16_cstride || a.k_chan0 || a.w_cin || a.res_bmod || a.out16_stride)) {
-    set_error("conv_igemm(dma): the register-streamed kernel does not run this problem, and no other kernel knows a K window, res_bmod or out16_stride (see stedm_conv_rs_ok)");
+  if (rc < 0 && (a.src16_cstride || a.k_chan0 || a.w_cin || a.res_bmod || a.res2 || p.partials || a.out16_stride)) {
+    set_error("conv_igemm(dma): the register-streamed kernel does not run this problem, and no other kernel knows a K window, res_bmod / res2, the partials-only form or out16_stride (see stedm_conv_rs_ok)");
     return 1;
   }
   if (rc < 0 && a.src16b_hi) { set_error("conv_igemm(dma): no kernel runs this fused skip problem (see stedm_conv_fused_skip_ok)"); return 1; }
diff --git a/stedm_amd/csrc/conv_rs.inc b/stedm_amd/csrc/conv_rs.inc
--- a/stedm_amd/csrc/conv_rs.inc
+++ b/stedm_amd/csrc/conv_rs.inc
@@ -321,6 +321,7 @@
   constexpr bool M16 = KIND == RS_3X3M || G1 || SUBM;
   constexpr bool GEO1 = IS1X1 || G1;
   constexpr bool IS3X3 = KIND == RS_3X3 || KIND == RS_3X3M;
+  constexpr bool RES2 = IS3X3 && !FUSE && !P3;
   constexpr int NS = IS3X3 ? 9 : (SUBM ? 4 : (SUBPIX ? 8 : (G1 ? 1 : 4)));
   constexpr int NPL = (SUBPIX || KIND == RS_3X3M) ? 2 : 1;
   constexpr int NTAB = IS3X3 ? 9 : 4;
@@ -996,6 +997,7 @@
       const bool has_emb = a.emb != nullptr;
       const int rb_ = a.res_bmod ? __builtin_amdgcn_readfirstlane(sMb[rfirst]) : 0;
       const float* __restrict__ resp = a.res_bmod ? a.res - (long)(rb_ - rb_ % a.res_bmod) * p.HWout * a.cout : a.res;
+      const float* __restrict__ resp2 = (RES2 && a.res2) ? a.res2 + (resp - a.res) : nullptr;
       float* __restrict__ outp = a.out;
       typedef T V4T16 __attribute__((ext_vector_type(4)));
       T* __restrict__ o16p = only16 ? reinterpret_cast<T*>(a.out16_hi) : nullptr;
@@ -1010,6 +1012,14 @@
           mm[k] = row < rfirst + rows_per ? sM[row] : -1;
           r4[k] = make_float4(0.f, 0.f, 0.f, 0.f);
           if (resp && mm[k] >= 0) r4[k] = *reinterpret_cast<const float4*>(resp + (long)mm[k] * a.cout + n);
+        }
+        if (RES2 && resp2) {
+#pragma unroll
+          for (int k = 0; k < RB; ++k)
+            if (mm[k] >= 0) {
+              const float4 s4 = *reinterpret_cast<const float4*>(resp2 + (long)mm[k] * a.cout + n);
+              r4[k].x += s4.x; r4[k].y += s4.y; r4[k].z += s4.z; r4[k].w += s4.w;
+            }
         }
 #pragma unroll
         for (int k = 0; k < RB; ++k) {
@@ -1051,6 +1061,10 @@
         }
         if (a.res) {
           const long ro = a.res_bmod ? o - (long)(sMb[row] - sMb[row] % a.res_bmod) * p.HWout * a.cout : o;
+          if (RES2 && a.res2) {
+            const float4 r4 = *reinterpret_cast<const float4*>(a.res + ro), s4 = *reinterpret_cast<const float4*>(a.res2 + ro);
+            v[0] += r4.x + s4.x; v[1] += r4.y + s4.y; v[2] += r4.z + s4.z; v[3] += r4.w + s4.w;
+          } else
           if (vec_ok) { const float4 r4 = *reinterpret_cast<const float4*>(a.res + ro); v[0] += r4.x; v[1] += r4.y; v[2] += r4.z; v[3] += r4.w; }
           else for (int u = 0; u < nv; ++u) v[u] += a.res[ro + u];
         }
@@ -1237,19 +1251,25 @@
       const float4 e4 = *reinterpret_cast<const float4*>(a.emb + (long)b * a.emb_bstride + n);
       add.x += e4.x; add.y += e4.y; add.z += e4.z; add.w += e4.w;
     }
+    const long wshift = a.ws_bmod ? (long)(b - b % a.ws_bmod) * HW * C : 0;
+    const long rshift = a.res_bmod ? (long)(b - b % a.res_bmod) * HW * C : 0;
 #pragma unroll 2
     for (int pix = px0 + tp; pix < px1; pix += npl) {
       const long o = ((long)b * HW + pix) * C + n;
       float4 pz[KSMAX];
 #pragma unroll
       for (int z = 0; z < KSMAX; ++z)
-        if (KSMAX == 2 || z < ksplit) pz[z] = *reinterpret_cast<const float4*>(a.ws + z * plane + o);
+        if (KSMAX == 2 || z < ksplit) pz[z] = *reinterpret_cast<const float4*>(a.ws + z * plane + (o - wshift));
       float4 v = pz[0];
 #pragma unroll
       for (int z = 1; z < KSMAX; ++z)
         if (KSMAX == 2 || z < ksplit) { v.x += pz[z].x; v.y += pz[z].y; v.z += pz[z].z; v.w += pz[z].w; }
       v.x += add.x; v.y += add.y; v.z += add.z; v.w += add.w;
-      if (a.res) { const float4 r4 = *reinterpret_cast<const float4*>(a.res + (a.res_bmod ? o - (long)(b - b % a.res_bmod) * HW * C : o)); v.x += r4.x; v.y += r4.y; v.z += r4.z; v.w += r4.w; }
+      if (a.res) {
+        float4 r4 = *reinterpret_cast<const float4*>(a.res + (o - rshift));
+        if (a.res2) { const float4 s4 = *reinterpret_cast<const float4*>(a.res2 + (o - rshift)); r4.x += s4.x; r4.y += s4.y; r4.z += s4.z; r4.w += s4.w; }
+        v.x += r4.x; v.y += r4.y; v.z += r4.z; v.w += r4.w;
+      }
       if (GN || a.out) *reinterpret_cast<float4*>(a.out + o) = v;
       if (a.out16_hi) {
         const long o16 = a.out16_stride ? ((long)b * HW + pix) * a.out16_stride + n : o;
@@ -1332,6 +1352,48 @@
       f16_guard_commit(ovf, badn, STEDM_F16G_NORM);
     }
   }
+}
+
+static bool splitk_reduce_launch(ConvParams& p, const int HWo, const long plane, const int ksplit, bool stats, const bool fine_ok, const bool gn_ok, hipStream_t st) {
+  int qbs = 64;
+  while (qbs > 8 && (long)p.a.B * ((HWo + 255) / 256) * ((p.a.cout / 4 + qbs - 1) / qbs) < 256) qbs >>= 1;
+  const int cpg = (p.a.gn_out16 && p.a.gn_groups > 0) ? p.a.cout / p.a.gn_groups : 0;
+  const bool gn = cpg > 0 && p.a.out && HWo <= 256 && gn_ok && p.a.chan_stats && stats && (p.a.chan_nslab == 0 || p.a.chan_nslab == 1) && p.a.cout % 32 == 0 &&
+                  cpg % 4 == 0 && 32 % cpg == 0;
+  if (gn) qbs = 8;
+  int slab_px = 256;
+  if (!gn) {
+    if (p.a.chan_stats && stats && fine_ok) slab_px = HWo / p.a.chan_nslab;
+    else if (!p.a.chan_stats || !stats)
+      while (slab_px > 16 && HWo % (slab_px / 2) == 0 && (long)p.a.B * ((HWo + slab_px - 1) / slab_px) * ((p.a.cout / 4 + 7) / 8) < 512) slab_px >>= 1;
+    if (slab_px < 256) {
+      qbs = 256 / (slab_px < 32 ? slab_px : 32);
+      if (qbs > 64) qbs = 64;
+    }
+  }
+  dim3 grid(p.a.B, (HWo + slab_px - 1) / slab_px, (p.a.cout / 4 + qbs - 1) / qbs);
+  stedm_conv_args ra = p.a;
+  if (!stats) ra.chan_stats = nullptr;
+  if (gn) {
+    if (ksplit == 2) conv_splitk_reduce_kernel<2, true><<<grid, 256, 0, st>>>(ra, HWo, plane, 2, qbs, p.ovf);
+    else conv_splitk_reduce_kernel<16, true><<<grid, 256, 0, st>>>(ra, HWo, plane, ksplit, qbs, p.ovf);
+    p.gn_done = 1;
+  } else if (ksplit == 2) conv_splitk_reduce_kernel<2><<<grid, 256, 0, st>>>(ra, HWo, plane, 2, qbs, p.ovf, slab_px);
+  else conv_splitk_reduce_kernel<16><<<grid, 256, 0, st>>>(ra, HWo, plane, ksplit, qbs, p.ovf, slab_px);
+  return ra.chan_stats != nullptr;
+}
+
+static int splitk_finish_impl(ConvParams& p, const int nshare, hipStream_t st) {
+  const stedm_conv_args& a = p.a;
+  const int HW = a.Hin * a.Win, nrun = (HW + 255) / 256;
+  const bool fine_ok = a.chan_nslab > 0 && HW % a.chan_nslab == 0 && HW / a.chan_nslab >= 8 && HW / a.chan_nslab <= 256;
+  const bool stats = a.chan_stats && (a.chan_nslab == 0 || a.chan_nslab == nrun || fine_ok);
+  const long plane = (long)(a.ws_bmod ? a.ws_bmod : a.B) * HW * a.cout;
+  p.gn_done = 0;
+  const bool wrote = splitk_reduce_launch(p, HW, plane, nshare, stats, fine_ok, true, st);
+  STEDM_LAUNCH_CHECK();
+  p.stats_done = wrote ? 1 : 0;
+  return 0;
 }
 
 template <typename T, int WM, int KIND, bool FUSE = false, bool P3 = false>
@@ -1378,8 +1440,9 @@
   if (!q.a.out && q.a.chan_stats && !stats) return -1;
   if (q.a.out16_stride && (KIND == RS_1X1N || P3)) return -1;
   const bool kwin = q.a.src16_cstride || q.a.k_chan0 || q.a.w_cin;
-  if ((kwin || q.a.res_bmod) && !((KIND == RS_3X3 || KIND == RS_3X3M) && !FUSE && !P3)) return -1;
-  if (dry) return 0;
+  if ((kwin || q.a.res_bmod || q.a.res2 || q.partials) && !((KIND == RS_3X3 || KIND == RS_3X3M) && !FUSE && !P3)) return -1;
+  if (q.a.res2 && q.a.cout % 4 != 0) return -1;
+  if (dry) { p.nshare = q.ksplit >= 2 ? q.ksplit : 1; return 0; }
   p = q;
   p.mg_hw = flat ? 0u : magic(p.HWout); p.mg_w = magic(p.Wout); p.mg_pw = magic(p.PW); p.mg_prpw = magic(p.PRs * p.PW);
   {
@@ -1436,36 +1499,12 @@
   if (kp.ksplit >= 2) kp.a.chan_stats = nullptr;
   k<<<p.npers ? p.tiles_m * p.npers : p.tiles_m * p.tiles_n * ((SUBK && !s2d) ? 4 : 1) * (kp.ksplit >= 2 ? kp.ksplit : 1), (16 / WM + 2) * 64, lds_launch, st>>>(kp);
   STEDM_LAUNCH_CHECK();
-  if (kp.ksplit >= 2) {
-    int qbs = 64;
-    while (qbs > 8 && (long)p.a.B * ((HWo + 255) / 256) * ((p.a.cout / 4 + qbs - 1) / qbs) < 256) qbs >>= 1;
-    const int cpg = (p.a.gn_out16 && p.a.gn_groups > 0) ? p.a.cout / p.a.gn_groups : 0;
-    const bool gn = cpg > 0 && p.a.out && HWo <= 256 && !(SUBK && !s2d) && p.a.chan_stats && stats && (p.a.chan_nslab == 0 || p.a.chan_nslab == 1) && p.a.cout % 32 == 0 &&
-                    cpg % 4 == 0 && 32 % cpg == 0;
-    if (gn) qbs = 8;
-    int slab_px = 256;
-    if (!gn) {
-      if (p.a.chan_stats && stats && fine_ok) slab_px = HWo / p.a.chan_nslab;
-      else if (!p.a.chan_stats || !stats)
-        while (slab_px > 16 && HWo % (slab_px / 2) == 0 && (long)p.a.B * ((HWo + slab_px - 1) / slab_px) * ((p.a.cout / 4 + 7) / 8) < 512) slab_px >>= 1;
-      if (slab_px < 256) {
-        qbs = 256 / (slab_px < 32 ? slab_px : 32);
-        if (qbs > 64) qbs = 64;
-      }
-    }
-    dim3 grid(p.a.B, (HWo + slab_px - 1) / slab_px, (p.a.cout / 4 + qbs - 1) / qbs);
-    const long plane = (long)p.a.B * HWo * p.a.cout;
-    stedm_conv_args ra = p.a;
-    if (!stats) ra.chan_stats = nullptr;
-    if (gn) {
-      if (kp.ksplit == 2) conv_splitk_reduce_kernel<2, true><<<grid, 256, 0, st>>>(ra, HWo, plane, 2, qbs, p.ovf);
-      else conv_splitk_reduce_kernel<16, true><<<grid, 256, 0, st>>>(ra, HWo, plane, kp.ksplit, qbs, p.ovf);
-      p.gn_done = 1;
-    } else if (kp.ksplit == 2) conv_splitk_reduce_kernel<2><<<grid, 256, 0, st>>>(ra, HWo, plane, 2, qbs, p.ovf, slab_px);
-    else conv_splitk_reduce_kernel<16><<<grid, 256, 0, st>>>(ra, HWo, plane, kp.ksplit, qbs, p.ovf, slab_px);
+  p.nshare = kp.ksplit >= 2 ? kp.ksplit : 1;
+  if (kp.ksplit >= 2 && !p.partials) {
+    stats = splitk_reduce_launch(p, HWo, (long)p.a.B * HWo * p.a.cout, kp.ksplit, stats, fine_ok, !(SUBK && !s2d), st);
     STEDM_LAUNCH_CHECK();
-    stats = ra.chan_stats != nullptr;
-  }
+  }
+  if (p.partials) return 0;
   if (stats) p.stats_done = 1;
   if (p.gn_tile || p.gn_coop) p.gn_done = 1;
   return 0;
diff --git a/stedm_amd/ops.py b/stedm_amd/ops.py
--- a/stedm_amd/ops.py
+++ b/stedm_amd/ops.py
@@ -446,14 +446,14 @@
                skip: Optional[Tuple[torch.Tensor, torch.Tensor, Optional[torch.Tensor]]] = None, query_fused: bool = False, query_rs: bool = False,
                ws: Optional[torch.Tensor] = None, pad_br: bool = False, w_frag16: Optional[torch.Tensor] = None,
                gn_next: Optional[tuple] = None, qkv_planes: Optional[tuple] = None, ln_after: Optional[tuple] = None, coop: Optional[tuple] = None,
-               out16_stride: int = 0, cout: Optional[int] = None, res_bmod: int = 0):
+               out16_stride: int = 0, cout: Optional[int] = None, res_bmod: int = 0, res2: Optional[torch.Tensor] = None, partials: bool = False):
     if src16 is not None and src1 is None and ks == 3 and mode in (CONV_S1, CONV_DOWN, CONV_UP) and not out16_stride:
         _, H_, W_, _ = src16[0].shape
         Ho_, Wo_ = ((H_ - 1) // 2 + 1, (W_ - 1) // 2 + 1) if mode == CONV_DOWN else ((2 * H_, 2 * W_) if mode == CONV_UP else (H_, W_))
         if not conv3x3_tiles_ok(Ho_, Wo_):
             if query_fused or query_rs:
                 return False
-            if not src16[0].is_contiguous() or res_bmod:
+            if not src16[0].is_contiguous() or res_bmod or res2 is not None or partials:
                 raise _lib.StedmHipError("conv_igemm: a K window / res_bmod belongs to the tiled register-streamed kernel; this output grid takes the im2col form")
             return _conv3x3_generic(src16, w_hi, w_lo, out, prec=prec, mode=mode, scale=scale, shift=shift, act=act, bias=bias, emb=emb,
                                     emb_offset=emb_offset, emb_bstride=emb_bstride, res=res, act_out=act_out, out16=out16, chan_stats=chan_stats,
@@ -563,6 +563,9 @@
     a.res_bmod = int(res_bmod)
     if res_bmod:
         assert res is not None and res.is_contiguous() and res.dtype == torch.float32 and B % res_bmod == 0 and res.shape[0] >= res_bmod
+    if res2 is not None:
+        assert res is not None and res2.is_contiguous() and res2.dtype == torch.float32 and tuple(res2.shape) == tuple(res.shape)
+        a.res2 = res2.data_ptr()
     a.c1, a.c2, a.src2_bmod = c1, c2, src2_bmod
     a.B, a.Hin, a.Win = B, Hin, Win
     a.mode, a.ks = mode, ks
@@ -589,11 +592,74 @@
             "the space-to-depth form runs on the register-streamed kernel only"
     else:
         assert w_hi.shape == (a.cout, ks * ks, a.w_cin if kwin else a.c1 + a.c2), (w_hi.shape, a.cout, ks, a.c1, a.c2)
+    if partials:
+        assert ws is not None and not query_fused
+        n = C.c_int32(0)
+        rc = lib().stedm_conv_partials(C.byref(a), C.byref(n), int(bool(query_rs)), _stream())
+        if query_rs:
+            return int(n.value) if rc == 0 else 0
+        check(rc, "stedm_conv_partials")
+        return int(n.value)
     if query_fused:
         return bool(lib().stedm_conv_fused_skip_ok(C.byref(a)))
     if query_rs:
         return bool(lib().stedm_conv_rs_ok(C.byref(a)))
     check(lib().stedm_conv_igemm(C.byref(a), _stream()), "stedm_conv_igemm")
+    return out
+
+
+def conv_finish(ws: torch.Tensor, nshare: int, out: Optional[torch.Tensor], *, prec: Precision, ws_bmod: int = 0, bias: Optional[torch.Tensor] = None,
+                emb: Optional[torch.Tensor] = None, emb_offset: int = 0, emb_bstride: int = 0, res: Optional[torch.Tensor] = None,
+                res2: Optional[torch.Tensor] = None, res_bmod: int = 0, chan_stats: Optional[torch.Tensor] = None,
+                out16: Optional[Tuple[torch.Tensor, Optional[torch.Tensor]]] = None, out16_stride: int = 0, cout: Optional[int] = None,
+                gn_next: Optional[tuple] = None):
+    shape = tuple(out.shape) if out is not None else tuple(out16[0].shape[:-1]) + (int(cout),)
+    B, H, W, co = shape
+    a = ConvArgs()
+    _chk(ws, name="ws")
+    a.ws, a.ws_floats, a.ws_bmod = ws.data_ptr(), ws.numel(), int(ws_bmod)
+    a.B, a.Hin, a.Win, a.cout = B, H, W, co
+    a.mode, a.ks, a.npass, a.mm_dtype = CONV_S1, 3, prec.npass, prec.mm_dtype
+    if out is not None:
+        _chk(out, name="out")
+        a.out = out.data_ptr()
+    a.bias = _ptr(bias)
+    if bias is not None:
+        assert bias.numel() == co
+    if emb is not None:
+        assert emb.dtype == torch.float32 and emb.numel() >= emb_offset + (B - 1) * emb_bstride + co
+        a.emb = emb.data_ptr() + 4 * emb_offset
+    a.emb_bstride = int(emb_bstride)
+    for r in (res, res2):
+        if r is not None:
+            _chk(r, name="res")
+            assert tuple(r.shape[1:]) == (H, W, co) and r.shape[0] >= (res_bmod or B)
+    assert res2 is None or res is not None
+    a.res, a.res2, a.res_bmod = _ptr(res), _ptr(res2), int(res_bmod)
+    if chan_stats is not None:
+        _chk(chan_stats, name="chan_stats")
+        assert chan_stats.shape[0] == B and tuple(chan_stats.shape[2:]) == (co, 2)
+        a.chan_stats, a.chan_nslab = chan_stats.data_ptr(), chan_stats.shape[1]
+    if out16 is not None:
+        assert out16[0].dtype == torch.int16 and out16[0].is_contiguous() and tuple(out16[0].shape) == (B, H, W, out16_stride or co)
+        a.out16_hi, a.out16_stride = out16[0].data_ptr(), int(out16_stride)
+    if gn_next is not None:
+        g_w, g_b, g_eps, g_groups, g_act, g_out = gn_next[:6]
+        g_lo = None
+        if isinstance(g_out, (tuple, list)):
+            g_out, g_lo = g_out[0], g_out[1]
+        g_mr = gn_next[6] if len(gn_next) > 6 else None
+        _chk(g_w, name="gn gamma"); _chk(g_b, name="gn beta")
+        assert out is not None and chan_stats is not None and g_out.dtype == torch.int16 and g_out.is_contiguous() and tuple(g_out.shape) == shape
+        a.gn_gamma, a.gn_beta, a.gn_eps, a.gn_groups, a.gn_act, a.gn_out16 = g_w.data_ptr(), g_b.data_ptr(), float(g_eps), int(g_groups), int(g_act), g_out.data_ptr()
+        if g_lo is not None:
+            assert g_lo.dtype == torch.int16 and g_lo.is_contiguous() and tuple(g_lo.shape) == shape
+            a.gn_out16_lo = g_lo.data_ptr()
+        if g_mr is not None:
+            _chk(g_mr, name="gn mean_rstd")
+            assert tuple(g_mr.shape) == (B, int(g_groups), 2)
+            a.gn_mr = g_mr.data_ptr()
+    check(lib().stedm_conv_finish(C.byref(a), int(nshare), _stream()), "stedm_conv_finish")
     return out
 
 
diff --git a/stedm_amd/unet.py b/stedm_amd/unet.py
--- a/stedm_amd/unet.py
+++ b/stedm_amd/unet.py
@@ -210,6 +210,8 @@
         self._plane_ctr = 0
         self._tape: Optional[list] = None
         self.cfg_shared_skip: Optional[bool] = None
+        self.cfg_shared_front: Optional[bool] = None
+        self.cfg_skip_partials: Optional[bool] = None
 
     def convert_to_fp16(self):
         pass
@@ -583,8 +585,14 @@
         if plan is None:
             ops.conv_igemm(None, pk.hi, pk.lo, h, src16=a16, **kw)
             return
-        seam, P = plan
+        seam, P, P2 = plan
         Bs = P.shape[0]
+        if P2 is not None:
+            n = ops.conv_igemm(None, pk.hi, pk.lo, P, prec=kw["prec"], src16=(a16[0][:Bs, :, :, seam:], None), w_frag=pk.frag, w_frag16=pk.frag16,
+                               ws=P2.view(-1), partials=True)
+            assert n == 2, n
+            ops.conv_igemm(None, pk.hi, pk.lo, h, src16=(a16[0][:, :, :, :seam], None), res=P2[0], res2=P2[1], res_bmod=Bs, **kw)
+            return
         ops.conv_igemm(None, pk.hi, pk.lo, P, prec=kw["prec"], src16=(a16[0][:Bs, :, :, seam:], None), w_frag=pk.frag, w_frag16=pk.frag16, ws=kw["ws"])
         ops.conv_igemm(None, pk.hi, pk.lo, h, src16=(a16[0][:, :, :, :seam], None), res=P, res_bmod=Bs, **kw)
 
@@ -593,7 +601,7 @@
         if (self.cfg_shared_skip is False or self._tape is not None or self.precision.npass != 1 or x2_bmod <= 0 or Bd != 2 * x2_bmod or
                 a16[0].shape[0] != Bd or not a16[0].is_contiguous()):
             return None
-        key = ("sskip", id(rb), Bd, H, W, self.cfg_shared_skip)
+        key = ("sskip", id(rb), Bd, H, W, self.cfg_shared_skip, self.cfg_skip_partials)
         hit = self._consts.get(key)
         if hit is None:
             norm = rb.in_layers[0]
@@ -610,10 +618,20 @@
                 ok = ok and bool(ops.conv_igemm(None, pk.hi, pk.lo, h, src16=(a16[0][:, :, :, :seam], None), res=P, res_bmod=x2_bmod, query_rs=True, **kw))
                 if ok and (self.cfg_shared_skip or self._shared_skip_rule(Bd, H, W, co, C, seam)):
                     hit = seam
+                    two = self.cfg_skip_partials is True and kw["ws"] is not None and ops.conv_igemm(None, pk.hi, pk.lo, P, prec=kw["prec"], src16=(a16[0][:x2_bmod, :, :, seam:], None), w_frag=pk.frag,
+                                                                  w_frag16=pk.frag16, ws=kw["ws"], partials=True, query_rs=True) == 2
+                    if two:
+                        P2 = self._buf(f"sskip.P2.{x2_bmod}x{H}x{W}x{co}", (2, x2_bmod, H, W, co))
+                        two = (ops.conv_igemm(None, pk.hi, pk.lo, P, prec=kw["prec"], src16=(a16[0][:x2_bmod, :, :, seam:], None), w_frag=pk.frag,
+                                              w_frag16=pk.frag16, ws=P2.view(-1), partials=True, query_rs=True) == 2 and
+                               bool(ops.conv_igemm(None, pk.hi, pk.lo, h, src16=(a16[0][:, :, :, :seam], None), res=P2[0], res2=P2[1], res_bmod=x2_bmod,
+                                                   query_rs=True, **kw)))
+                    self._consts[("sskip2",) + key[1:]] = bool(two)
             self._consts[key] = hit
         if not hit:
             return None
-        return hit, self._buf(f"sskip.P.{x2_bmod}x{H}x{W}x{co}", (x2_bmod, H, W, co))
+        P2 = self._buf(f"sskip.P2.{x2_bmod}x{H}x{W}x{co}", (2, x2_bmod, H, W, co)) if self._consts.get(("sskip2",) + key[1:]) else None
+        return hit, self._buf(f"sskip.P.{x2_bmod}x{H}x{W}x{co}", (x2_bmod, H, W, co)), P2
 
     @staticmethod
     def _shared_skip_rule(Bd: int, H: int, W: int, co: int, C: int, seam: int) -> bool:
@@ -625,6 +643,75 @@
         if not fills(Bd):
             return False
         return (C - seam) // 32 >= (14 if fills(Bd // 2) else 32)
+
+    def _replicate(self, h, nrep: int):
+        h2 = self._buf("mid.rep", (nrep * h.shape[0],) + tuple(h.shape[1:]))
+        cs1 = self._cs.get(h.data_ptr())
+        cs2 = self._cs_new(h2, nslab=cs1.shape[1]) if cs1 is not None else None
+        h2.view((nrep,) + tuple(h.shape)).copy_(h.unsqueeze(0).expand((nrep,) + tuple(h.shape)))
+        if cs2 is not None:
+            cs2.view((nrep,) + tuple(cs1.shape)).copy_(cs1.unsqueeze(0).expand((nrep,) + tuple(cs1.shape)))
+        return h2
+
+    def _front_ws(self, nel: int) -> torch.Tensor:
+        return self._buf("sfront.ws", ((16 if nel <= (1 << 20) else (4 if nel <= (1 << 22) else (2 if nel <= (1 << 23) else 1))) * nel,))
+
+    def _front_kw(self, tag: str, rb: ResBlock, x1, next_norm):
+        prec = self.precision
+        B, H, W, _ = x1.shape
+        Bd, co = 2 * B, rb.out_channels
+        pk, pk2 = self._packed[id(rb.in_layers[2])], self._packed[id(rb.out_layers[3])]
+        h = self._buf(f"h.{Bd}x{H}x{W}x{co}", (Bd, H, W, co))
+        out = self._buf(tag + ".out", (Bd, H, W, co))
+        gn2 = rb.out_layers[0]
+        h16 = self._planes(Bd, H, W, co, "g16")
+        gnn = npl = coop2 = None
+        if next_norm is not None and not os.environ.get("STEDM_NO_NEXT_GN"):
+            nn_, nact = next_norm
+            npl = self._planes(Bd, H, W, co)
+            gnn = (nn_.weight, nn_.bias, nn_.eps, nn_.num_groups, nact, npl[0], None, False)
+            coop2 = self._coop_for(tag + ".c2", Bd, H, W, co, prec)
+        part = dict(prec=prec, w_frag=pk.frag, w_frag16=pk.frag16, ws=self._front_ws(B * H * W * co), partials=True)
+        fin = dict(prec=prec, ws_bmod=B, bias=pk.bias, gn_next=(gn2.weight, gn2.bias, gn2.eps, gn2.num_groups, 1, h16[0], None, True))
+        tail = dict(prec=prec, src16=h16, bias=pk2.bias, res=x1, res_bmod=B, w_frag=pk2.frag, ws=self._splitk_ws_res(Bd * H * W * co), w_frag16=pk2.frag16,
+                    gn_next=gnn, coop=coop2)
+        return pk, pk2, h, out, npl, part, fin, tail
+
+    def _shared_front(self, tag: str, rb: ResBlock, x1shape, next_norm) -> bool:
+        B, H, W, C = x1shape
+        if (self.cfg_shared_front is False or self._tape is not None or self.precision.npass != 1 or not isinstance(rb.skip_connection, nn.Identity) or
+                rb.out_channels != C):
+            return False
+        key = ("sfront", id(rb), 2 * B, H, W, self.cfg_shared_front)
+        hit = self._consts.get(key)
+        if hit is None:
+            hit = 0
+            pk, pk2, h, out, npl, part, fin, tail = self._front_kw(tag, rb, self._buf("mid.a.0.out", x1shape), next_norm)
+            if (pk.frag is not None or pk.frag16 is not None) and C % 4 == 0 and (self.cfg_shared_front or self._shared_front_rule(2 * B, H, W, C)):
+                a16 = self._planes(B, H, W, C)
+                n = ops.conv_igemm(None, pk.hi, pk.lo, self._buf(f"h.{B}x{H}x{W}x{C}", (B, H, W, C)), src16=a16, query_rs=True, **part)
+                if n and ops.conv_igemm(None, pk2.hi, pk2.lo, out, chan_stats=self._cs_new(out), query_rs=True, **tail):
+                    hit = int(n)
+            self._consts[key] = hit
+        return bool(hit)
+
+    @staticmethod
+    def _shared_front_rule(Bd: int, H: int, W: int, co: int) -> bool:
+        cus = ops.device_cus()
+        tiles_m = -(-Bd * H * W // 256) if H * W >= 256 else -(-Bd // (256 // (H * W)))
+        return tiles_m * -(-co // 128) * 2 >= cus
+
+    def _res_front(self, tag: str, rb: ResBlock, x1, style_all, next_norm):
+        B, H, W, C = x1.shape
+        pk, pk2, h, out, npl, part, fin, tail = self._front_kw(tag, rb, x1, next_norm)
+        a16 = self._norm16(rb.in_layers[0], 1, x1)
+        n = ops.conv_igemm(None, pk.hi, pk.lo, self._buf(f"h.{B}x{H}x{W}x{C}", (B, H, W, C)), src16=a16, **part)
+        self._last_h = h
+        ops.conv_finish(part["ws"], n, h, emb=style_all, emb_bstride=style_all.shape[1], chan_stats=self._cs_new(h), **fin)
+        ops.conv_igemm(None, pk2.hi, pk2.lo, out, chan_stats=self._cs_new(out), **tail)
+        if npl is not None:
+            self._pre16[out.data_ptr()] = (id(next_norm[0]), next_norm[1], npl)
+        return out
 
     def _attn(self, tag: str, ab: AttentionBlock, x):
         prec = self.precision
@@ -858,21 +945,20 @@
             nl = list(self.input_blocks[i + 1])[0] if i + 1 < nblk else mid[0]
             h = self._run_block(f"in{i}", blk, h, None, emb_e, emb_stride, None, next_layer=nl)
             hs.append(h)
-        h = self._run_block("mid.a", mid[:1], h, None, emb_e, emb_stride, None, next_layer=mid[1] if nrep == 1 and len(mid) > 1 else None)
-        if nrep > 1:
-            h2 = self._buf("mid.rep", (Bd,) + tuple(h.shape[1:]))
-            cs1 = self._cs.get(h.data_ptr())
-            cs2 = self._cs_new(h2, nslab=cs1.shape[1]) if cs1 is not None else None
-            h2.view((nrep,) + tuple(h.shape)).copy_(h.unsqueeze(0).expand((nrep,) + tuple(h.shape)))
-            if cs2 is not None:
-                cs2.view((nrep,) + tuple(cs1.shape)).copy_(cs1.unsqueeze(0).expand((nrep,) + tuple(cs1.shape)))
-            h = h2
+        front = (nrep == 2 and len(mid) > 2 and isinstance(mid[1], ResBlockStyle) and
+                 self._shared_front("mid.b.1", mid[1].block, tuple(h.shape), self._first_norm(mid[2])))
+        h = self._run_block("mid.a", mid[:1], h, None, emb_e, emb_stride, None, next_layer=mid[1] if (nrep == 1 or front) and len(mid) > 1 else None)
+        if front:
+            h = self._res_front("mid.b.1", mid[1].block, h, style_all, self._first_norm(mid[2]))
+        elif nrep > 1:
+            h = self._replicate(h, nrep)
+
         def first_takes_cat(blk):
             l0 = list(blk)[0]
             return isinstance(l0, ResBlock) and not isinstance(l0.skip_connection, nn.Identity)
 
         ob = list(self.output_blocks)
-        h = self._run_block("mid.b", mid[1:], h, None, emb_d, emb_stride, style_all, li0=1,
+        h = self._run_block("mid.b", mid[2:] if front else mid[1:], h, None, emb_d, emb_stride, style_all, li0=2 if front else 1,
                             next_skip_c=hs[-1].shape[-1] if ob and first_takes_cat(ob[0]) else None)
         bmod = B if nrep > 1 else 0
         for i, blk in enumerate(ob):
```

Measured after the change: 168.8 steps/s (median of 6 runs). +1.2%, better.
